# evergreen-ci/evergreen

Measured on NVIDIA H100. Metric: tasks scheduled/sec over N distros; host-allocator decisions/sec at 1/2/4/8 GPU, higher is better.
Workload: dtype int64

## Files before the change

### evergreen_b200/_lib.py

```python
from __future__ import annotations

import ctypes as C
import os

import numpy as np

_HERE = os.path.dirname(os.path.abspath(__file__))
LIB_PATH = os.path.join(_HERE, "libevgsched.so")

EVG_TIME_ZERO = -(2 ** 63)

EVG_OK = 0
EVG_ERR_INVALID, EVG_ERR_CUDA, EVG_ERR_NOMEM, EVG_ERR_STATE = -1, -2, -3, -4
EVG_ALLOC_OK, EVG_ALLOC_ERR_FUTURE_FRACTION, EVG_ALLOC_ERR_POOL_SIZE, EVG_ALLOC_ERR_PARENT_MISSING = 0, 1, 2, 3

EVG_TF_REQ_OTHER, EVG_TF_REQ_PATCH, EVG_TF_REQ_MERGE_QUEUE = 0, 1, 2
EVG_TF_GENERATE, EVG_TF_STEPBACK, EVG_TF_DEPS_MET, EVG_TF_OTHER_DISTRO = 0x4, 0x8, 0x10, 0x20
EVG_HF_RUNNING, EVG_HF_TEARDOWN, EVG_HF_RT_FOUND = 0x1, 0x2, 0x4
EVG_HG_NONE, EVG_HG_UNQUEUED = -1, -2
EVG_PROVIDER_STATIC, EVG_PROVIDER_EPHEMERAL, EVG_PROVIDER_DOCKER = 0, 1, 2
EVG_OPT_BREAKDOWN = 0x1
EVG_BD_N = 13
(EVG_BD_TASK_GROUP_LENGTH, EVG_BD_TOTAL_VALUE, EVG_BD_P_INITIAL, EVG_BD_P_TASK_GROUP, EVG_BD_P_GENERATOR,
 EVG_BD_P_COMMIT_QUEUE, EVG_BD_R_COMMIT_QUEUE, EVG_BD_R_NUM_DEPENDENTS, EVG_BD_R_ESTIMATED_RUNTIME,
# ... 66 lines not shown
class PlanOutStruct(C.Structure):
    _fields_ = [("order", C.c_void_p), ("total_value", C.c_void_p), ("breakdown", C.c_void_p),
                ("info", C.c_void_p), ("group_info", C.c_void_p)]


class HostSoAStruct(C.Structure):
    _fields_ = [("n_hosts", C.c_int64), ("flags", C.c_void_p), ("group_id", C.c_void_p),
                ("expected_ns", C.c_void_p), ("std_ns", C.c_void_p), ("start_ns", C.c_void_p)]


class DepsInStruct(C.Structure):
    _fields_ = [("n_tasks", C.c_int64), ("n_deps", C.c_int64), ("dep_off", C.c_void_p), ("dep_kind", C.c_void_p),
                ("dep_ref", C.c_void_p), ("dep_want", C.c_void_p), ("task_state", C.c_void_p), ("task_pre", C.c_void_p),
                ("ext_state", C.c_void_p), ("n_ext", C.c_int64)]


EVG_DEP_IN_QUEUE, EVG_DEP_EXTERNAL, EVG_DEP_MISSING = 0, 1, 2
EVG_WANT_SUCCESS, EVG_WANT_FAILED, EVG_WANT_ANY, EVG_WANT_OTHER = 0, 1, 2, 3
EVG_TS_BLOCKED = 0x4
EVG_TP_OVERRIDE, EVG_TP_MET_TIME = 0x1, 0x2


class RunnableInStruct(C.Structure):
    _fields_ = [("n_tasks", C.c_int64), ("n_distros", C.c_int32), ("n_projects", C.c_int32), ("task_off", C.c_void_p),
                ("sched", C.c_void_p), ("project", C.c_void_p), ("project_flags", C.c_void_p), ("valid_off", C.c_void_p),
                ("valid_idx", C.c_void_p), ("finder", C.c_void_p), ("deps", C.POINTER(DepsInStruct))]


class AliasInStruct(C.Structure):
    _fields_ = [("tasks", TaskSoAStruct), ("n_groups", C.c_int32), ("n_versions", C.c_int32), ("group_max_hosts", C.c_void_p),
                ("sched", C.c_void_p), ("task_group_max_hosts", C.c_void_p), ("primary", C.c_void_p),
                ("secondary_off", C.c_void_p), ("secondary_idx", C.c_void_p), ("n_names", C.c_int32), ("_reserved", C.c_int32),
                ("dest_off", C.c_void_p), ("dest_idx", C.c_void_p), ("deps", C.POINTER(DepsInStruct)),
                ("dep_finished_ns", C.c_void_p)]


class AliasOutStruct(C.Structure):
    _fields_ = [("task_off", C.c_void_p), ("group_off", C.c_void_p), ("n_versions", C.c_void_p)]


EVG_SQ_ACTIVATED, EVG_SQ_UNDISPATCHED, EVG_SQ_PRIORITY_OK, EVG_SQ_HOST_PLATFORM = 0x01, 0x02, 0x04, 0x08
EVG_SQ_UNATTAINABLE, EVG_SQ_OVERRIDE_DEPS, EVG_SQ_GITHUB_PR, EVG_SQ_PATCH_REQUEST = 0x10, 0x20, 0x40, 0x80
EVG_PF_ENABLED, EVG_PF_HIDDEN, EVG_PF_DISPATCHING_DISABLED, EVG_PF_PATCHING_DISABLED = 0x1, 0x2, 0x4, 0x8
EVG_FINDER_NO_DEPS, EVG_FINDER_LEGACY, EVG_FINDER_ALTERNATE = 0, 1, 2
EVG_FINDER_PIPELINE, EVG_FINDER_PIPELINE_NO_DEPS = 3, 4
EVG_STATUS_SUCCESS, EVG_STATUS_FAILED, EVG_STATUS_ANY = 0, 1, 2
EVG_PR_ENABLED, EVG_PR_DISPATCHING_DISABLED, EVG_PR_PATCHING_FALSE = 0x1, 0x2, 0x4


class PipelineInStruct(C.Structure):
    _fields_ = [("n_status", C.c_int32), ("_reserved", C.c_int32), ("dep_status", C.c_void_p), ("task_status", C.c_void_p),
                ("ext_status", C.c_void_p), ("task_unattainable", C.c_void_p), ("ext_unattainable", C.c_void_p),
                ("project_raw", C.c_void_p)]


class DurationRowsStruct(C.Structure):
    _fields_ = [("n_rows", C.c_int64), ("n_keys", C.c_int32), ("_reserved", C.c_int32), ("key", C.c_void_p),
                ("time_taken_ns", C.c_void_p), ("start_ns", C.c_void_p), ("finish_ns", C.c_void_p), ("flags", C.c_void_p),
                ("window_start_ns", C.c_int64), ("window_end_ns", C.c_int64)]


EVG_DR_COMPLETED, EVG_DR_TIMED_OUT = 0x1, 0x2
DURATION_STAT_DTYPE = np.dtype([("count", np.int64), ("mean_ns", np.float64), ("stddev_ns", np.float64)])
EVG_DK_NONE = -1


def EVG_DK_PAIR(p: int) -> int:
    return -2 - p


EVG_DS_FRESH, EVG_DS_BACKFILL, EVG_DS_HISTORY, EVG_DS_PREVIOUS, EVG_DS_DEFAULT = 0, 1, 2, 3, 4
DURATION_CACHE_COLUMNS = ("value_ns", "std_ns", "ttl_ns", "collected_ns", "expected_ns", "expected_std_ns")


class DurationCacheStruct(C.Structure):
    _fields_ = [("n_rows", C.c_int64), ("rows", C.c_void_p), ("value_ns", C.c_void_p), ("std_ns", C.c_void_p),
                ("ttl_ns", C.c_void_p), ("collected_ns", C.c_void_p), ("expected_ns", C.c_void_p),
                ("expected_std_ns", C.c_void_p), ("key", C.c_void_p)]


class DurationInStruct(C.Structure):
    _fields_ = [("history", C.POINTER(DurationRowsStruct)), ("n_pairs", C.c_int32), ("_reserved", C.c_int32),
                ("pair_key_off", C.c_void_p), ("tasks", C.POINTER(DurationCacheStruct)),
                ("hosts", C.POINTER(DurationCacheStruct))]


DURATION_OUT_FIELDS = ("avg_ns", "std_ns", "value_ns", "pred_std_ns", "collected_ns", "source")


class DurationOutStruct(C.Structure):
    _fields_ = [(f, C.c_void_p) for f in DURATION_OUT_FIELDS]


class LegacySoAStruct(C.Structure):
    _fields_ = [("n_tasks", C.c_int64), ("priority", C.c_void_p), ("ingest_ns", C.c_void_p), ("expected_ns", C.c_void_p),
                ("num_dependents", C.c_void_p), ("revision_order", C.c_void_p), ("project_id", C.c_void_p),
                ("tg_rank", C.c_void_p), ("tg_pair_id", C.c_void_p), ("task_group_order", C.c_void_p),
                ("presort_rank", C.c_void_p), ("flags", C.c_void_p)]


EVG_LF_REQ_SYSTEM, EVG_LF_REQ_PATCH, EVG_LF_REQ_OTHER, EVG_LF_GENERATE, EVG_LF_MERGE_QUEUE_VERSION = 0, 1, 2, 0x4, 0x8
EVG_LEGACY_MODE_INGEST, EVG_LEGACY_MODE_REVISION, EVG_LEGACY_MODE_LITERAL = 0, 1, 2
EVG_LEGACY_OK, EVG_LEGACY_NOT_DECOMPOSABLE = 0, 1


class DagInStruct(C.Structure):
    _fields_ = [("n_items", C.c_int64), ("n_deps", C.c_int64), ("dep_off", C.c_void_p), ("dep_item", C.c_void_p),
                ("group_id", C.c_void_p), ("group_index", C.c_void_p)]


DISPATCH_OUT_FIELDS = ("item_off", "sorted", "n_sorted", "n_cycles", "group_off", "group_slot", "unit_items", "unit_off")


class DispatchOutStruct(C.Structure):
    _fields_ = [(f, C.c_void_p) for f in DISPATCH_OUT_FIELDS]


class AllocOutStruct(C.Structure):
    _fields_ = [("result", C.c_void_p), ("status", C.c_void_p)]


class EvgError(RuntimeError):
    def __init__(self, code: int, msg: str):
        super().__init__(f"libevgsched error {code}: {msg}")
        self.code = code


_P = C.c_void_p
SYMBOLS = {
    "evg_init": (C.c_int, [C.c_int, _P, C.POINTER(_P)]),
    "evg_shutdown": (None, [_P]),
    "evg_last_error": (C.c_char_p, []),
    "evg_abi_version": (C.c_int, []),
    "evg_host_alloc": (_P, [C.c_uint64]),
    "evg_host_free": (None, [_P]),
    "evg_plan_batch": (C.c_int, [_P, _P, _P, C.c_int64, C.c_uint32, _P]),
    "evg_alloc_batch": (C.c_int, [_P, _P, _P, _P, _P, _P, _P, C.c_int32, C.c_int64, _P]),
    "evg_plan_and_alloc_batch": (C.c_int, [_P, _P, _P, _P, _P, _P, C.c_int64, C.c_uint32, _P, _P]),
    "evg_upload": (C.c_int, [_P, _P, _P, _P, _P, _P]),
    "evg_upload_device": (C.c_int, [_P, _P, _P, _P, _P, _P]),
    "evg_update_tasks": (C.c_int, [_P, C.c_int64, _P, _P]),
    "evg_edit_tasks": (C.c_int, [_P, _P, _P, _P, _P, _P]),
    "evg_plan_from_finder": (C.c_int, [_P, _P, _P, _P, _P, _P, _P, _P, C.c_int64, _P, _P]),
    "evg_plan_from_finder_ex": (C.c_int, [_P, _P, _P, _P, _P, _P, _P, _P, _P, C.c_int64, _P, _P]),
    "evg_plan_aliases": (C.c_int, [_P, _P, _P, C.c_int32, C.c_int64, _P]),
    "evg_download_alias_map": (C.c_int, [_P, _P, _P]),
    "evg_intern_columns": (C.c_int, [_P, _P, C.c_int32]),
    "evg_run_resident": (C.c_int, [_P, C.c_int64, C.c_uint32]),
    "evg_download": (C.c_int, [_P, _P, _P]),
    "evg_download_queue": (C.c_int, [_P, C.c_int32, _P, _P, C.c_int64]),
    "evg_device_result_ptr": (_P, [_P]),
    "evg_bind_result_buffer": (C.c_int, [_P, _P, C.c_int64]),
    "evg_last_launch_count": (C.c_int64, [_P]),
    "evg_last_timing_ms": (C.c_int, [_P, C.POINTER(C.c_float), C.POINTER(C.c_float)]),
    "evg_kernel_timing_ms": (C.c_int, [_P, C.POINTER(C.c_float), C.c_int32]),
    "evg_general_timing_ms": (C.c_int, [_P, C.POINTER(C.c_float), C.POINTER(C.c_float)]),
    "evg_deps_met_batch": (C.c_int, [_P, _P, _P]),
    "evg_upload_with_deps": (C.c_int, [_P, _P, _P, _P, _P, _P, _P, _P, C.c_int64]),
    "evg_download_deps": (C.c_int, [_P, _P, _P]),
    "evg_find_runnable_batch": (C.c_int, [_P, _P, _P, _P]),
    "evg_find_runnable_ex": (C.c_int, [_P, _P, _P, _P, _P]),
    "evg_expected_durations_batch": (C.c_int, [_P, _P, _P]),
    "evg_resolve_durations": (C.c_int, [_P, _P, C.c_int64]),
    "evg_download_durations": (C.c_int, [_P, _P, _P]),
    "evg_prioritize_legacy_batch": (C.c_int, [_P, _P, _P, _P, C.c_int32, _P, _P, _P]),
    "evg_dag_rebuild_batch": (C.c_int, [_P, _P, _P, _P, C.c_int32, _P, _P, _P, _P, _P]),
    "evg_rebuild_dispatchers": (C.c_int, [_P, C.c_int32, C.c_int64, C.c_int64, _P]),
    "evg_plan_distro": (C.c_int, [_P, _P, _P, C.c_int32, _P, C.c_int64, C.c_uint32, _P]),
    "evg_alloc_distro": (C.c_int, [_P, _P, _P, _P, _P, C.c_int32, C.c_int64, _P, _P]),
}

_lib = None


def load() -> C.CDLL:
    global _lib
    if _lib is not None:
        return _lib
    if not os.path.exists(LIB_PATH):
        raise ImportError(
            f"{LIB_PATH} is missing: build it with `python -c 'import __graft_entry__ as g; g.build()'` "
            "(nvcc, sm_90a). evergreen_b200 has no CPU fallback.")
    lib = C.CDLL(LIB_PATH)
    for name, (res, args) in SYMBOLS.items():
        fn = getattr(lib, name)
        fn.restype = res
        fn.argtypes = args
    if lib.evg_abi_version() != 1:
        raise ImportError("libevgsched.so ABI version mismatch")
    _lib = lib
    return lib


def last_error() -> str:
    return (load().evg_last_error() or b"").decode("utf-8", "replace")


def check(rc: int) -> None:
    if rc != EVG_OK:
        raise EvgError(rc, last_error())


def ptr(a) -> int:
    if a is None:
        return None
    assert a.flags["C_CONTIGUOUS"], "columns must be C-contiguous"
    return a.ctypes.data
```

### evergreen_b200/csrc/evg_plan_general.cuh

```cuda
#pragma once

#ifndef EVG_OCC_GLINK
#define EVG_OCC_GLINK 4
#endif
#ifndef EVG_OCC_GALLOC
#define EVG_OCC_GALLOC 4
#endif
#ifndef EVG_OCC_GFILL
#define EVG_OCC_GFILL 4
#endif
#ifndef EVG_OCC_GUNIT
#define EVG_OCC_GUNIT 4
#endif
#ifndef EVG_OCC_GBEST
#define EVG_OCC_GBEST 4
#endif
#ifndef EVG_GTASK_OCC
#define EVG_GTASK_OCC 2
#endif
constexpr int kGTile = 2048;

struct DGen {
  int64_t n_tiles;
  int64_t tile0;
  const int32_t* tile_distro;
  const int64_t* tile_start;
  const int64_t* dtile_off;
  unsigned long long* vmm;
  uint32_t* key_lo[2];
  uint32_t* key_hi[2];
  uint32_t* idx[2];
  uint32_t* e;
  uint32_t* tile_sum;
  uint32_t* tile_hist;
  uint4* wl;
  struct URec* pay;
  unsigned int* ccount;
  uint4* tie;
  int32_t* maxpass;
  uint32_t* run;
  uint32_t* pown;
  uint32_t* pver;
  uint32_t* pedge;
  uint32_t* sedge;
  uint32_t* rank;
  unsigned int* rcount;
  uint2* blist;
  unsigned int* bcount;
  uint4* usum;
  uint2* hlist;
  unsigned int* hcount;
  int64_t* tv;
};

__device__ __forceinline__ int gen_bits(const DGen& G, int d) {
  const unsigned long long r = G.vmm[2 * d] - G.vmm[2 * d + 1];
  return r == 0 ? 0 : 64 - __clzll((long long)r);
}
__device__ __forceinline__ int gen_npass(int bits) { return (bits + 7) >> 3; }

struct __align__(16) URec {
  int32_t prio, nd;
  int64_t exp_ns, qb;
  int32_t tgo;
  uint32_t lif;
};
static_assert(sizeof(URec) == 32, "one L2 sector per member");
constexpr uint32_t kRecGrouped = 1u << 22, kRecWaitOver = 1u << 23;
constexpr uint32_t kRunOwn = 1u << 31, kRunEntry = kRunOwn - 1u;
__device__ __forceinline__ uint32_t rec_li(const URec& r) { return r.lif & 0x1FFFFFu; }
__device__ __forceinline__ URec rec_load(const URec* p) {
  const uint4 a = reinterpret_cast<const uint4*>(p)[0], b = reinterpret_cast<const uint4*>(p)[1];
  URec r;
  r.prio = int32_t(a.x); r.nd = int32_t(a.y); r.exp_ns = int64_t((unsigned long long)a.z | ((unsigned long long)a.w << 32));
  r.qb = int64_t((unsigned long long)b.x | ((unsigned long long)b.y << 32)); r.tgo = int32_t(b.z); r.lif = b.w;
  return r;
}
__device__ __forceinline__ void rec_store(URec* p, const URec& r) {
  reinterpret_cast<uint4*>(p)[0] = make_uint4(uint32_t(r.prio), uint32_t(r.nd), uint32_t(uint64_t(r.exp_ns)), uint32_t(uint64_t(r.exp_ns) >> 32));
  reinterpret_cast<uint4*>(p)[1] = make_uint4(uint32_t(uint64_t(r.qb)), uint32_t(uint64_t(r.qb) >> 32), uint32_t(r.tgo), r.lif);
}

__global__ void k_ginit(DGen G, const int32_t* __restrict__ general_list, int n) {
  const int k = blockIdx.x * blockDim.x + threadIdx.x;
  if (k == 0) { *G.ccount = 0u; *G.maxpass = 0; *G.rcount = 0u; *G.hcount = 0u; *G.bcount = 0u; }
  if (k >= n) return;
  const int d = general_list[k];
  G.vmm[2 * d] = 0ull;
  G.vmm[2 * d + 1] = ~0ull;
}

__global__ void __launch_bounds__(256) k_gmark(DTasks T, DDistros D, DWork W, DGen G) {
  if (*W.err) return;
  const int tile = int(blockIdx.x + G.tile0);
  const int d = G.tile_distro[tile];
  const int64_t base = D.task_off[d], end = D.task_off[d + 1];
  const int64_t lo = max(G.tile_start[tile], base), hi = min(G.tile_start[tile] + kGTile, end);
  for (int64_t t = lo + threadIdx.x; t < hi; t += 256)
    for (int64_t e = T.dep_off[t]; e < T.dep_off[t + 1]; e++) W.has_dep[base + T.dep_idx[e]] = 1;
}

struct TileFold {
  unsigned int c[10];
  unsigned long long s[4];
  unsigned long long vmax, vmin;
};

__global__ void __launch_bounds__(256, EVG_GTASK_OCC) k_gtask(DTasks T, DDistros D, DWork W, DGen G, int64_t now, int any_complex) {
  if (*W.err) return;
  __shared__ TileFold F;
  __shared__ evg_distro_cfg s_cfg;
  __shared__ uint32_t s_nd[kNdTable];
  const int tile = int(blockIdx.x + G.tile0);
  const int d = G.tile_distro[tile];
  const int tid = threadIdx.x, lane = tid & 31;
  const unsigned full = 0xffffffffu;
  if (tid == 0) {
    for (int k = 0; k < 10; k++) F.c[k] = 0;
    for (int k = 0; k < 4; k++) F.s[k] = 0;
    F.vmax = 0ull; F.vmin = ~0ull;
    s_cfg = D.cfg[d];
  }
  __syncthreads();
  const evg_distro_cfg& cfg = s_cfg;
  const int64_t base = D.task_off[d], end = D.task_off[d + 1];
  const int64_t ts = G.tile_start[tile];
  const uint32_t ng = uint32_t(D.group_off[d + 1] - D.group_off[d]);
  const uint32_t ub = uint32_t(D.unit_base[d]);
  const bool gv = cfg.group_versions != 0;
  const int64_t threshold = cfg.target_time_ns;
  const PlannerFactors pf = clamp_factors(cfg);
  const Factors32 f32 = factors32(pf, now);
  const bool sane_clock = threshold >= 0 && now >= threshold;
  const int64_t wait_cutoff = wsub(now, threshold);
  const bool fast_clock = now >= 0 && pf.nd_int != 0;
  const bool incl = cfg.includes_dependencies != 0;
  if (tid < kNdTable) {
    const int64_t e = nd_table_entry(pf, tid);
    s_nd[tid] = (e >= 0 && e < int64_t(kNdTermLimit)) ? uint32_t(e) : 0xFFFFFFFFu;
  }
  __syncthreads();
  const bool dcomplex = any_complex && (ng > 0 || gv || (T.n_edges > 0 && T.dep_off[end] > T.dep_off[base]));

  unsigned int c_dm = 0, c_mq = 0, c_over = 0, c_wait = 0, c_sec = 0, c_ung = 0, c_ucnt = 0, c_uover = 0, c_uwait = 0, c_umq = 0;
  int64_t s_exp = 0, s_over = 0, s_uexp = 0, s_uover = 0;
  unsigned long long kmax = 0ull, kmin = ~0ull;

#pragma unroll 1
  for (int u = 0; u < 2; u++) {
    const int64_t t4 = ts + 4 * int64_t(u * 256 + tid);
    const bool live = t4 < end;
    int4 prio4 = make_int4(0, 0, 0, 0), nd4 = prio4, gid4 = make_int4(-1, -1, -1, -1), tgo4 = prio4, vid4 = prio4;
    uint4 fl4 = make_uint4(0, 0, 0, 0);
    uint32_t cmask = 0, womask = 0;
    if (live && dcomplex) {
      tgo4 = *reinterpret_cast<const int4*>(T.tgo + t4);
      if (gv) vid4 = *reinterpret_cast<const int4*>(T.vid + t4);
    }
    longlong2 ex01 = make_longlong2(0, 0), ex23 = ex01, qb01 = ex01, qb23 = ex01, wb01 = ex01, wb23 = ex01;
    if (live) {
      prio4 = *reinterpret_cast<const int4*>(T.priority + t4);
      nd4 = *reinterpret_cast<const int4*>(T.numdep + t4);
      gid4 = *reinterpret_cast<const int4*>(T.gid + t4);
      fl4 = *reinterpret_cast<const uint4*>(T.flags + t4);
      ex01 = *reinterpret_cast<const longlong2*>(T.expected + t4); ex23 = *reinterpret_cast<const longlong2*>(T.expected + t4 + 2);
      qb01 = *reinterpret_cast<const longlong2*>(T.qbasis + t4); qb23 = *reinterpret_cast<const longlong2*>(T.qbasis + t4 + 2);
      wb01 = *reinterpret_cast<const longlong2*>(T.wbasis + t4); wb23 = *reinterpret_cast<const longlong2*>(T.wbasis + t4 + 2);
    }
    int64_t doff[5] = {0, 0, 0, 0, 0};
    uint32_t hd4 = 0;
    if (live && dcomplex) {
      if (T.n_edges > 0) {
        const longlong2 d01 = *reinterpret_cast<const longlong2*>(T.dep_off + t4), d23 = *reinterpret_cast<const longlong2*>(T.dep_off + t4 + 2);
        doff[0] = d01.x; doff[1] = d01.y; doff[2] = d23.x; doff[3] = d23.y; doff[4] = T.dep_off[t4 + 4];
      }
      hd4 = *reinterpret_cast<const uint32_t*>(W.has_dep + t4);
    }
    const int32_t prio_[4] = {prio4.x, prio4.y, prio4.z, prio4.w}, nd_[4] = {nd4.x, nd4.y, nd4.z, nd4.w};
    const int32_t gid_[4] = {gid4.x, gid4.y, gid4.z, gid4.w};
    const uint32_t fl_[4] = {fl4.x, fl4.y, fl4.z, fl4.w};
    const int64_t ex_[4] = {ex01.x, ex01.y, ex23.x, ex23.y}, qb_[4] = {qb01.x, qb01.y, qb23.x, qb23.y};
    const int64_t wb_[4] = {wb01.x, wb01.y, wb23.x, wb23.y};
    int64_t vout[4];
    uint32_t eout[4], nd_term[4];
    bool wr_v[4], solo[4];
    bool dom = true;
#pragma unroll
    for (int m = 0; m < 4; m++) {
      const int64_t t = t4 + m;
      const bool valid = live & (t >= base) & (t < end);
      const int32_t prio = prio_[m], nd = nd_[m], gid = gid_[m];
      const uint32_t fl = fl_[m];
      const int64_t exp_ns = ex_[m], qb = qb_[m], wb = wb_[m];
      const bool dm = valid & ((fl & EVG_TF_DEPS_MET) != 0);
      const bool counted = valid & (!incl | dm);
      const bool over = counted & (exp_ns > threshold);
      const bool waited = sane_clock ? (wb < wait_cutoff) : (since(now, wb) > threshold);
      const bool wait_over = counted & dm & waited;
      const bool mq_dm = dm & ((fl & EVG_TF_REQ_MASK) == EVG_TF_REQ_MERGE_QUEUE);
      const bool ung = valid & (gid < 0);
      c_dm += dm; c_mq += mq_dm; c_over += over; c_wait += wait_over; c_sec += valid & ((fl & EVG_TF_OTHER_DISTRO) != 0);
      s_exp += counted ? exp_ns : 0;
      s_over += over ? exp_ns : 0;
      c_ung += ung; c_ucnt += ung & counted; c_uover += ung & over; c_uwait += ung & wait_over; c_umq += ung & mq_dm;
      s_uexp += (ung & counted) ? exp_ns : 0;
      s_uover += (ung & over) ? exp_ns : 0;
      const bool own_complex = valid & dcomplex & ((gid >= 0) | gv | (((hd4 >> (8 * m)) & 0xFFu) != 0));
      const bool complex_task = own_complex | (valid & dcomplex & (doff[m + 1] > doff[m]));
      const bool scores = valid & !own_complex;
      const uint32_t ndc = uint32_t(nd > 0 ? nd : 0);
      const uint32_t tab = s_nd[ndc < uint32_t(kNdTable) ? ndc : 0u];
      const uint32_t mul = (f32.ok & (ndc < kTask32Limit)) ? f32.nd * ndc : 0xFFFFFFFFu;
      nd_term[m] = ndc < uint32_t(kNdTable) ? tab : mul;
      dom = dom & (!scores | (score32_bad(now, prio, exp_ns, qb, nd_term[m]) == 0u));
      wr_v[m] = scores;
      solo[m] = scores & !complex_task;
      eout[m] = (valid & !complex_task) ? 1u : 0u;
      cmask |= (complex_task ? 1u : 0u) << m;
      womask |= (wait_over ? 1u : 0u) << m;
    }
    if (f32.ok_base && __all_sync(full, dom)) {
#pragma unroll
      for (int m = 0; m < 4; m++) vout[m] = int64_t(single_task_value32_nd(f32, now, prio_[m], ex_[m], qb_[m], nd_term[m], fl_[m]));
    } else {
#pragma unroll
      for (int m = 0; m < 4; m++) vout[m] = int64_t(score_slow(pf, fast_clock, wr_v[m], now, prio_[m], ex_[m], qb_[m], nd_[m], fl_[m]));
    }
#pragma unroll
    for (int m = 0; m < 4; m++) {
      const unsigned long long k = ord_i64(vout[m]);
      kmax = solo[m] ? max(kmax, k) : kmax;
      kmin = solo[m] ? min(kmin, k) : kmin;
    }
    if (!live) {
    } else if (t4 >= base && t4 + 3 < end) {
      *reinterpret_cast<longlong2*>(G.tv + t4) = make_longlong2(vout[0], vout[1]);
      *reinterpret_cast<longlong2*>(G.tv + t4 + 2) = make_longlong2(vout[2], vout[3]);
    } else {
#pragma unroll
      for (int m = 0; m < 4; m++)
        if (wr_v[m]) G.tv[t4 + m] = vout[m];
    }
    if (dcomplex && live) {
      if (t4 >= base && t4 + 3 < end) *reinterpret_cast<uint4*>(G.e + t4) = make_uint4(eout[0], eout[1], eout[2], eout[3]);
      else {
#pragma unroll
        for (int m = 0; m < 4; m++)
          if (t4 + m >= base && t4 + m < end) G.e[t4 + m] = eout[m];
      }
    }
    if (dcomplex) {
      __shared__ uint32_t s_wsum[8];
      __shared__ uint32_t s_lbase;
      const uint32_t mine = __popc(cmask);
      uint32_t inc = mine;
#pragma unroll
      for (int o = 1; o < 32; o <<= 1) { const uint32_t x = __shfl_up_sync(full, inc, o); if (lane >= o) inc += x; }
      if (lane == 31) s_wsum[tid >> 5] = inc;
      __syncthreads();
      uint32_t before = 0, total = 0;
#pragma unroll
      for (int w = 0; w < 8; w++) { const uint32_t x = s_wsum[w]; before += w < (tid >> 5) ? x : 0u; total += x; }
      if (total) {
        if (tid == 0) s_lbase = atomicAdd(G.ccount, total);
        __syncthreads();
        uint32_t pos = s_lbase + before + inc - mine;
        const int32_t vid_[4] = {vid4.x, vid4.y, vid4.z, vid4.w}, tgo_[4] = {tgo4.x, tgo4.y, tgo4.z, tgo4.w};
#pragma unroll
        for (int m = 0; m < 4; m++) {
          if (!((cmask >> m) & 1u)) continue;
          const uint32_t t = uint32_t(t4 + m), li = uint32_t(t4 + m - base);
          const int32_t gid = gid_[m], vid = vid_[m];
          const bool own_complex = (gid >= 0) | gv | (((hd4 >> (8 * m)) & 0xFFu) != 0);
          const uint32_t s_own = own_complex ? ub + own_slot_local(gid, vid, li, ng, gv) : kInactive;
          const uint32_t s_ver = (gid >= 0 && gv) ? ub + ng + uint32_t(vid) : kInactive;
          G.wl[pos] = make_uint4(t, uint32_t(d), s_own, s_ver);
          URec r;
          r.prio = prio_[m]; r.nd = nd_[m]; r.exp_ns = ex_[m]; r.qb = qb_[m]; r.tgo = tgo_[m];
          r.lif = li | (gid >= 0 ? kRecGrouped : 0u) | (((womask >> m) & 1u) ? kRecWaitOver : 0u) | ((fl_[m] & 0x3Fu) << 24);
          rec_store(G.pay + pos, r);
          pos++;
        }
      }
      __syncthreads();
    }
  }
  {
    unsigned int cs[10] = {c_dm, c_mq, c_over, c_wait, c_sec, c_ung, c_ucnt, c_uover, c_uwait, c_umq};
#pragma unroll
    for (int k = 0; k < 10; k++) cs[k] = __reduce_add_sync(full, cs[k]);
    int64_t ss[4] = {s_exp, s_over, s_uexp, s_uover};
#pragma unroll
    for (int k = 0; k < 4; k++) ss[k] = warp_sum64(ss[k]);
#pragma unroll
    for (int o = 16; o > 0; o >>= 1) {
      kmax = max(kmax, __shfl_xor_sync(full, kmax, o));
      kmin = min(kmin, __shfl_xor_sync(full, kmin, o));
    }
    if (lane == 0) {
#pragma unroll
      for (int k = 0; k < 10; k++) if (cs[k]) atomicAdd(&F.c[k], cs[k]);
#pragma unroll
      for (int k = 0; k < 4; k++) if (ss[k]) atomicAdd(&F.s[k], (unsigned long long)ss[k]);
      atomicMax(&F.vmax, kmax); atomicMin(&F.vmin, kmin);
    }
  }
  __syncthreads();
  if (tid < 16) {
    evg_queue_info* q = W.qinfo + d;
    switch (tid) {
      case 0: atomic_add64(&q->length_with_dependencies_met, F.c[0]); break;
      case 1: atomic_add64(&q->count_dep_filled_merge_queue_tasks, F.c[1]); break;
      case 2: atomic_add64(&q->count_duration_over_threshold, F.c[2]); break;
      case 3: atomic_add64(&q->count_wait_over_threshold, F.c[3]); break;
      case 4: atomic_add64(&q->secondary_queue, F.c[4]); break;
      case 5: atomic_add64(&q->has_ungrouped, F.c[5]); break;
      case 6: atomic_add64(&q->ungrouped.count, F.c[6]); break;
      case 7: atomic_add64(&q->ungrouped.count_duration_over_threshold, F.c[7]); break;
      case 8: atomic_add64(&q->ungrouped.count_wait_over_threshold, F.c[8]); break;
      case 9: atomic_add64(&q->ungrouped.count_dep_filled_merge_queue_tasks, F.c[9]); break;
      case 10: atomic_add64(&q->expected_duration, int64_t(F.s[0])); break;
      case 11: atomic_add64(&q->duration_over_threshold, int64_t(F.s[1])); break;
      case 12: atomic_add64(&q->ungrouped.expected_duration, int64_t(F.s[2])); break;
      case 13: atomic_add64(&q->ungrouped.duration_over_threshold, int64_t(F.s[3])); break;
      case 14: if (F.vmax > __ldcg(G.vmm + 2 * d)) atomicMax(G.vmm + 2 * d, F.vmax); break;
      case 15: if (F.vmin < __ldcg(G.vmm + 2 * d + 1)) atomicMin(G.vmm + 2 * d + 1, F.vmin); break;
    }
  }
}


struct WlTask {
  uint32_t t; int d; int64_t base; uint32_t li; bool own_complex; uint32_t s_own, s_ver;
};
__device__ __forceinline__ WlTask wl_task(const DDistros& D, const DGen& G, unsigned int k) {
  const uint4 e = G.wl[k];
  WlTask x;
  x.t = e.x; x.d = int(e.y); x.s_own = e.z; x.s_ver = e.w;
  x.base = D.task_off[x.d];
  x.li = uint32_t(int64_t(x.t) - x.base);
  x.own_complex = x.s_own != kInactive;
  return x;
}
template <typename F>
__device__ __forceinline__ void wl_pairs(const DTasks& T, const DGen& G, const WlTask& x, unsigned int k, F&& f) {
  if (x.own_complex) f(G.pown + k, x.s_own, true);
  if (x.s_ver != kInactive) f(G.pver + k, x.s_ver, false);
  if (T.n_edges > 0)
    for (int64_t e = T.dep_off[x.t]; e < T.dep_off[x.t + 1]; e++) {
      const uint32_t sl = G.sedge[e];
      if (sl != kInactive) f(G.pedge + e, sl, false);
    }
}

__global__ void __launch_bounds__(256, EVG_OCC_GLINK) k_glink(DTasks T, DDistros D, DWork W, DGen G, int64_t now) {
  if (*W.err) return;
  const unsigned int n = *G.ccount;
  for (unsigned int k = blockIdx.x * blockDim.x + threadIdx.x; k < n; k += gridDim.x * blockDim.x) {
    const WlTask x = wl_task(D, G, k);
    const uint32_t t = x.t;
    const int d = x.d;
    const uint32_t ub = uint32_t(D.unit_base[d]), ng = uint32_t(D.group_off[d + 1] - D.group_off[d]);
    if (x.own_complex && x.s_own - ub < ng) {
      const URec me = rec_load(G.pay + k);
      const evg_distro_cfg* cf = D.cfg + d;
      const uint32_t fl = (me.lif >> 24) & 0x3Fu;
      const int64_t exp_ns = me.exp_ns, threshold = cf->target_time_ns;
      const bool dm = (fl & EVG_TF_DEPS_MET) != 0;
      const bool counted = !cf->includes_dependencies || dm;
      const bool over = counted && exp_ns > threshold;
      const bool wait_over = (me.lif & kRecWaitOver) != 0;
      const bool mq_dm = dm && (fl & EVG_TF_REQ_MASK) == EVG_TF_REQ_MERGE_QUEUE;
      evg_group_info* g = W.ginfo + D.group_off[d] + (x.s_own - ub);
      atomic_add64(&g->count, counted);
      atomic_add64(&g->expected_duration, counted ? exp_ns : 0);
      atomic_add64(&g->count_duration_over_threshold, over);
      atomic_add64(&g->duration_over_threshold, over ? exp_ns : 0);
      atomic_add64(&g->count_wait_over_threshold, wait_over);
      atomic_add64(&g->count_dep_filled_merge_queue_tasks, mq_dm);
    }
    if (x.own_complex) G.pown[k] = atomicAdd(W.unit_n + x.s_own, 1u);
    if (x.s_ver != kInactive) G.pver[k] = atomicAdd(W.unit_n + x.s_ver, 1u);
    if (T.n_edges > 0) {
      const bool gv = D.cfg[d].group_versions != 0;
      const int64_t e0 = T.dep_off[t], e1 = T.dep_off[t + 1];
      for (int64_t e = e0; e < e1; e++) {
        const uint32_t dl = uint32_t(T.dep_idx[e]);
        const uint32_t sl = ub + own_slot_local(T.gid[x.base + dl], T.vid[x.base + dl], dl, ng, gv);
        bool dup = (sl == x.s_own) || (sl == x.s_ver);
        for (int64_t f = e0; f < e && !dup; f++) {
          const uint32_t fl2 = uint32_t(T.dep_idx[f]);
          dup = ub + own_slot_local(T.gid[x.base + fl2], T.vid[x.base + fl2], fl2, ng, gv) == sl;
        }
        G.sedge[e] = dup ? kInactive : sl;
        if (!dup) G.pedge[e] = atomicAdd(W.unit_n + sl, 1u);
      }
    }
  }
}

__global__ void __launch_bounds__(256, EVG_OCC_GALLOC) k_galloc(DTasks T, DDistros D, DWork W, DGen G) {
  if (*W.err) return;
  __shared__ uint32_t s_wsum[8], s_wcnt[8];
  __shared__ uint32_t s_base, s_hbase;
  const unsigned int n = *G.ccount;
  const int lane = threadIdx.x & 31, warp = threadIdx.x >> 5;
  for (unsigned int k0 = blockIdx.x * blockDim.x; k0 < n; k0 += gridDim.x * blockDim.x) {
    const unsigned int k = k0 + threadIdx.x;
    WlTask x;
    uint32_t need = 0, heads = 0;
    if (k < n) {
      x = wl_task(D, G, k);
      wl_pairs(T, G, x, k, [&](const uint32_t* place, uint32_t slot, bool) { if (*place == 0u) { need += W.unit_n[slot]; heads++; } });
    }
    uint32_t inc = need, hinc = heads;
#pragma unroll
    for (int o = 1; o < 32; o <<= 1) {
      const uint32_t y = __shfl_up_sync(0xffffffffu, inc, o), z = __shfl_up_sync(0xffffffffu, hinc, o);
      if (lane >= o) { inc += y; hinc += z; }
    }
    if (lane == 31) { s_wsum[warp] = inc; s_wcnt[warp] = hinc; }
    __syncthreads();
    uint32_t before = 0, total = 0, hbefore = 0, htotal = 0;
#pragma unroll
    for (int w = 0; w < 8; w++) {
      const uint32_t y = s_wsum[w], z = s_wcnt[w];
      before += w < warp ? y : 0u; total += y; hbefore += w < warp ? z : 0u; htotal += z;
    }
    if (threadIdx.x == 0 && htotal) { s_base = atomicAdd(G.rcount, total); s_hbase = atomicAdd(G.hcount, htotal); }
    __syncthreads();
    if (heads) {
      uint32_t pos = s_base + before + inc - need, hp = s_hbase + hbefore + hinc - heads;
      wl_pairs(T, G, x, k, [&](const uint32_t* place, uint32_t slot, bool) {
        if (*place == 0u) { W.head[slot] = pos; pos += W.unit_n[slot]; G.hlist[hp++] = make_uint2(slot, uint32_t(x.d)); }
      });
    }
    __syncthreads();
  }
}

__global__ void __launch_bounds__(256, EVG_OCC_GFILL) k_gfill(DTasks T, DDistros D, DWork W, DGen G) {
  if (*W.err) return;
  const unsigned int n = *G.ccount;
  for (unsigned int k = blockIdx.x * blockDim.x + threadIdx.x; k < n; k += gridDim.x * blockDim.x) {
    const WlTask x = wl_task(D, G, k);
    wl_pairs(T, G, x, k, [&](const uint32_t* place, uint32_t slot, bool own) {
      G.run[W.head[slot] + *place] = k | (own ? kRunOwn : 0u);
    });
  }
}

__device__ __forceinline__ void rec_acc(UnitAcc& a, int64_t now, const URec& r) {
  acc_add(a, now, r.prio, r.exp_ns, r.qb, r.nd, (r.lif & kRecGrouped) ? 0 : -1, (r.lif >> 24) & 0x3Fu);
}
__device__ __forceinline__ bool rec_less(const URec& x, const URec& y) {
  return in_unit_less(x.tgo, x.nd, x.prio, x.exp_ns, rec_li(x), y.tgo, y.nd, y.prio, y.exp_ns, rec_li(y));
}
constexpr uint32_t kRankOne = 8;
constexpr int kRankKey = 6;

__global__ void __launch_bounds__(256, EVG_OCC_GUNIT) k_gunit(DDistros D, DWork W, DGen G, int64_t now) {
  if (*W.err) return;
  const unsigned int n = *G.hcount;
  __shared__ uint32_t s_key[kRankOne * kRankKey][256];
  for (unsigned int k = blockIdx.x * blockDim.x + threadIdx.x; k < n; k += gridDim.x * blockDim.x) {
    const uint2 u = G.hlist[k];
    const uint32_t cnt = W.unit_n[u.x], h = W.head[u.x];
    const uint32_t* run = G.run + h;
    UnitAcc a;
    acc_init(a);
    uint32_t anchor = kNoAnchor;
    const bool small = cnt <= kRankOne;
    for (uint32_t i = 0; i < cnt; i++) {
      const uint32_t q = run[i];
      const URec r = rec_load(G.pay + (q & kRunEntry));
      rec_acc(a, now, r);
      if (q & kRunOwn) anchor = min(anchor, rec_li(r));
      if (small) {
        uint32_t* kx = &s_key[i * kRankKey][threadIdx.x];
        kx[0] = uint32_t(r.tgo); kx[256] = uint32_t(r.nd); kx[512] = uint32_t(r.prio);
        kx[768] = uint32_t(uint64_t(r.exp_ns)); kx[1024] = uint32_t(uint64_t(r.exp_ns) >> 32); kx[1280] = rec_li(r);
      }
    }
    const unsigned long long v = (unsigned long long)unit_value(a, D.cfg[u.y], nullptr);
    G.usum[u.x] = make_uint4(uint32_t(v), uint32_t(v >> 32), anchor, cnt);
    W.unit_mask[u.x] = 0ull;
    if (small) {
      auto key = [&](uint32_t i, URec& r) {
        const uint32_t* kx = &s_key[i * kRankKey][threadIdx.x];
        r.tgo = int32_t(kx[0]); r.nd = int32_t(kx[256]); r.prio = int32_t(kx[512]);
        r.exp_ns = int64_t((unsigned long long)kx[768] | ((unsigned long long)kx[1024] << 32)); r.lif = kx[1280];
      };
      for (uint32_t i = 0; i < cnt; i++) {
        URec me, o;
        key(i, me);
        uint32_t rk = 0;
        for (uint32_t j = 0; j < cnt; j++) { key(j, o); rk += rec_less(o, me) ? 1u : 0u; }
        G.rank[h + i] = rk;
      }
    } else {
      const uint32_t nch = (cnt + 31) >> 5;
      const uint32_t b = atomicAdd(G.bcount, nch);
      for (uint32_t c = 0; c < nch; c++) G.blist[b + c] = make_uint2(u.x, c);
    }
  }
}

__global__ void __launch_bounds__(256, EVG_OCC_GUNIT) k_grank(DWork W, DGen G) {
  if (*W.err) return;
  const unsigned int n = *G.bcount;
  const unsigned full = 0xffffffffu;
  const int lane = threadIdx.x & 31;
  const unsigned int nw = gridDim.x * (blockDim.x >> 5);
  for (unsigned int c = blockIdx.x * (blockDim.x >> 5) + (threadIdx.x >> 5); c < n; c += nw) {
    const uint2 ch = G.blist[c];
    const uint32_t cnt = W.unit_n[ch.x], h = W.head[ch.x];
    const uint32_t* run = G.run + h;
    const uint32_t i = ch.y * 32u + uint32_t(lane);
    URec me;
    me.tgo = 0; me.nd = 0; me.prio = 0; me.exp_ns = 0; me.lif = 0;
    if (i < cnt) me = rec_load(G.pay + (run[i] & kRunEntry));
    uint32_t rk = 0;
    for (uint32_t j0 = 0; j0 < cnt; j0 += 32) {
      URec o;
      o.tgo = 0; o.nd = 0; o.prio = 0; o.exp_ns = 0; o.lif = 0;
      if (j0 + lane < cnt) o = rec_load(G.pay + (run[j0 + lane] & kRunEntry));
      const uint32_t m = min(32u, cnt - j0);
      for (uint32_t q = 0; q < m; q++) {
        URec y;
        y.tgo = __shfl_sync(full, o.tgo, q); y.nd = __shfl_sync(full, o.nd, q); y.prio = __shfl_sync(full, o.prio, q);
        y.exp_ns = __shfl_sync(full, o.exp_ns, q); y.lif = __shfl_sync(full, o.lif, q);
        rk += (i < cnt && rec_less(y, me)) ? 1u : 0u;
      }
    }
    if (i < cnt) G.rank[h + i] = rk;
  }
}

__global__ void __launch_bounds__(256, EVG_OCC_GBEST) k_gbest(DTasks T, DDistros D, DWork W, DGen G, int want_best_pair) {
  if (*W.err) return;
  const unsigned int n = *G.ccount;
  const unsigned full = 0xffffffffu;
  const int lane = threadIdx.x & 31;
  for (unsigned int kw = blockIdx.x * blockDim.x + (threadIdx.x & ~31u); kw < n; kw += gridDim.x * blockDim.x) {
    const unsigned int k = kw + lane;
    int d = -1;
    unsigned long long kk = 0ull;
    if (k < n) {
      const WlTask x = wl_task(D, G, k);
      const uint32_t t = x.t, li = x.li;
      d = x.d;
      bool have = false;
      int64_t bv = 0;
      uint32_t ba = 0, brk = 0, bslot = kInactive, bn = 1, bkx = 0;
      if (!x.own_complex) { have = true; bv = G.tv[t]; ba = li; }
      wl_pairs(T, G, x, k, [&](const uint32_t* place, uint32_t slot, bool) {
        const uint4 u = G.usum[slot];
        const uint32_t kx = *place;
        const uint32_t a = u.z;
        if (a == kNoAnchor) return;
        const int64_t v = int64_t((unsigned long long)u.x | ((unsigned long long)u.y << 32));
        if (!have || v > bv || (v == bv && a < ba)) { have = true; bv = v; ba = a; bslot = slot; bn = u.w; bkx = kx; }
      });
      if (bslot != kInactive) {
        brk = G.rank[W.head[bslot] + bkx];
        if (bn <= 64) atomicOr(&W.unit_mask[bslot], 1ull << brk);
      }
      G.tv[t] = bv;
      G.tie[k] = make_uint4(ba, brk, bslot, 0u);
      if (want_best_pair) W.best_pair[t] = bslot;
      const bool displaced = !(ba == li && brk == 0);
      if (displaced) W.has_dep[t] |= 2;
      atomicAdd(G.e + x.base + ba, 1u);
      kk = ord_i64(bv);
    }
    const int d0 = __shfl_sync(full, d, 0);
    if (__all_sync(full, d < 0 || d == d0)) {
      unsigned long long hi = d < 0 ? 0ull : kk, lo = d < 0 ? ~0ull : kk;
#pragma unroll
      for (int o = 16; o > 0; o >>= 1) {
        hi = max(hi, __shfl_xor_sync(full, hi, o));
        lo = min(lo, __shfl_xor_sync(full, lo, o));
      }
      if (lane == 0) {
        if (hi > __ldcg(G.vmm + 2 * d0)) atomicMax(G.vmm + 2 * d0, hi);
        if (lo < __ldcg(G.vmm + 2 * d0 + 1)) atomicMin(G.vmm + 2 * d0 + 1, lo);
      }
    } else if (d >= 0) {
      if (kk > __ldcg(G.vmm + 2 * d)) atomicMax(G.vmm + 2 * d, kk);
      if (kk < __ldcg(G.vmm + 2 * d + 1)) atomicMin(G.vmm + 2 * d + 1, kk);
    }
  }
}

__global__ void k_gsched(DGen G, const int32_t* __restrict__ general_list, int n) {
  const int k = blockIdx.x * blockDim.x + threadIdx.x;
  if (k >= n) return;
  const int np = gen_npass(gen_bits(G, general_list[k]));
  if (np > 0) atomicMax(G.maxpass, np);
}

__global__ void __launch_bounds__(256) k_gsum(DDistros D, DGen G) {
  const int tile = int(blockIdx.x + G.tile0);
  const int d = G.tile_distro[tile];
  const int64_t base = D.task_off[d], end = D.task_off[d + 1];
  const int64_t lo = max(G.tile_start[tile], base), hi = min(G.tile_start[tile] + kGTile, end);
  uint32_t sum = 0;
  for (int64_t t = lo + threadIdx.x; t < hi; t += 256) sum += G.e[t];
  sum = __reduce_add_sync(0xffffffffu, sum);
  __shared__ uint32_t sw[8];
  if ((threadIdx.x & 31) == 0) sw[threadIdx.x >> 5] = sum;
  __syncthreads();
  if (threadIdx.x == 0) G.tile_sum[tile] = sw[0] + sw[1] + sw[2] + sw[3] + sw[4] + sw[5] + sw[6] + sw[7];
}

__global__ void __launch_bounds__(1024) k_gscan(DGen G, const int32_t* __restrict__ general_list) {
  const int d = general_list[blockIdx.x];
  const int64_t t0 = G.dtile_off[d], nt = G.dtile_off[d + 1] - t0;
  __shared__ uint32_t sw[32];
  __shared__ uint32_t carry;
  const int lane = threadIdx.x & 31, warp = threadIdx.x >> 5;
  if (threadIdx.x == 0) carry = 0;
  __syncthreads();
  for (int64_t c0 = 0; c0 < nt; c0 += 1024) {
    const int64_t i = c0 + threadIdx.x;
    const uint32_t v = i < nt ? G.tile_sum[t0 + i] : 0u;
    uint32_t inc = v;
#pragma unroll
    for (int o = 1; o < 32; o <<= 1) { const uint32_t x = __shfl_up_sync(0xffffffffu, inc, o); if (lane >= o) inc += x; }
    if (lane == 31) sw[warp] = inc;
    __syncthreads();
    if (warp == 0) {
      const uint32_t w = sw[lane];
      uint32_t winc = w;
#pragma unroll
      for (int o = 1; o < 32; o <<= 1) { const uint32_t x = __shfl_up_sync(0xffffffffu, winc, o); if (lane >= o) winc += x; }
      sw[lane] = winc - w;
    }
    __syncthreads();
    const uint32_t ex = carry + sw[warp] + inc - v;
    if (i < nt) G.tile_sum[t0 + i] = ex;
    __syncthreads();
    if (threadIdx.x == 1023) carry = ex + v;
    __syncthreads();
  }
}

__device__ __forceinline__ void gen_put(const DGen& G, int64_t base, uint32_t pos, unsigned long long vmax_ord, bool wide,
                                        int64_t v, uint32_t li) {
  const unsigned long long key = vmax_ord - ord_i64(v);
  G.key_lo[0][base + pos] = uint32_t(key);
  if (wide) G.key_hi[0][base + pos] = uint32_t(key >> 32);
  G.idx[0][base + pos] = li;
}

__global__ void __launch_bounds__(256) k_gplace(DDistros D, DWork W, DGen G, int use_e) {
  const int tile = int(blockIdx.x + G.tile0);
  const int d = G.tile_distro[tile];
  const int64_t base = D.task_off[d], end = D.task_off[d + 1];
  const int64_t ts = G.tile_start[tile];
  const unsigned long long vmax_ord = G.vmm[2 * d];
  const bool wide = gen_bits(G, d) > 32;
  const int tid = threadIdx.x, lane = tid & 31, warp = tid >> 5;
  const int64_t t8 = ts + 8 * int64_t(tid);
  const bool interior = t8 >= base && t8 + 7 < end;
  uint32_t ev[8];
  uint32_t sum = 0;
  if (use_e) {
    if (interior) {
      const uint4 a = *reinterpret_cast<const uint4*>(G.e + t8), b = *reinterpret_cast<const uint4*>(G.e + t8 + 4);
      ev[0] = a.x; ev[1] = a.y; ev[2] = a.z; ev[3] = a.w; ev[4] = b.x; ev[5] = b.y; ev[6] = b.z; ev[7] = b.w;
    } else {
#pragma unroll
      for (int m = 0; m < 8; m++) { const int64_t t = t8 + m; ev[m] = (t >= base && t < end) ? G.e[t] : 0u; }
    }
#pragma unroll
    for (int m = 0; m < 8; m++) sum += ev[m];
  }
  uint32_t run = 0;
  if (use_e) {
    __shared__ uint32_t sw[8];
    uint32_t inc = sum;
#pragma unroll
    for (int o = 1; o < 32; o <<= 1) { const uint32_t x = __shfl_up_sync(0xffffffffu, inc, o); if (lane >= o) inc += x; }
    if (lane == 31) sw[warp] = inc;
    __syncthreads();
    uint32_t before = 0;
#pragma unroll
    for (int w = 0; w < 8; w++) if (w < warp) before += sw[w];
    run = G.tile_sum[tile] + before + inc - sum;
  }
  int64_t vv[8];
  uint32_t dsp = 0;
  if (interior) {
#pragma unroll
    for (int m = 0; m < 8; m += 2) {
      const longlong2 x = *reinterpret_cast<const longlong2*>(G.tv + t8 + m);
      vv[m] = x.x; vv[m + 1] = x.y;
    }
    if (use_e) {
      const uint32_t h0 = *reinterpret_cast<const uint32_t*>(W.has_dep + t8), h1 = *reinterpret_cast<const uint32_t*>(W.has_dep + t8 + 4);
#pragma unroll
      for (int m = 0; m < 4; m++) dsp |= (((h0 >> (8 * m + 1)) & 1u) << m) | (((h1 >> (8 * m + 1)) & 1u) << (m + 4));
    }
  } else {
#pragma unroll
    for (int m = 0; m < 8; m++) {
      const int64_t t = t8 + m;
      const bool in = t >= base && t < end;
      vv[m] = in ? G.tv[t] : 0;
      if (use_e && in && (W.has_dep[t] & 2)) dsp |= 1u << m;
    }
  }
  if (use_e) {
    constexpr int kStage = 3072;
    __shared__ uint32_t st_lo[kStage], st_ix[kStage], st_hi[kStage];
    __shared__ uint32_t s_total;
    const uint32_t p_tile = G.tile_sum[tile];
    if (tid == 255) s_total = run + sum - p_tile;
    uint32_t ps[8];
#pragma unroll
    for (int m = 0; m < 8; m++) { ps[m] = run; run += ev[m]; }
    if (interior) {
      *reinterpret_cast<uint4*>(G.e + t8) = make_uint4(ps[0], ps[1], ps[2], ps[3]);
      *reinterpret_cast<uint4*>(G.e + t8 + 4) = make_uint4(ps[4], ps[5], ps[6], ps[7]);
    } else {
#pragma unroll
      for (int m = 0; m < 8; m++) { const int64_t t = t8 + m; if (t >= base && t < end) G.e[t] = ps[m]; }
    }
    __syncthreads();
    const uint32_t total = s_total;
    const bool staged = total <= uint32_t(kStage);
#pragma unroll
    for (int m = 0; m < 8; m++) {
      const int64_t t = t8 + m;
      if (t >= base && t < end && !((dsp >> m) & 1u)) {
        if (staged) {
          const unsigned long long key = vmax_ord - ord_i64(vv[m]);
          const uint32_t q = ps[m] - p_tile;
          st_lo[q] = uint32_t(key); st_ix[q] = uint32_t(t - base);
          if (wide) st_hi[q] = uint32_t(key >> 32);
        } else {
          gen_put(G, base, ps[m], vmax_ord, wide, vv[m], uint32_t(t - base));
        }
      }
    }
    if (staged) {
      __syncthreads();
      uint32_t* dlo = G.key_lo[0] + base + p_tile;
      uint32_t* dix = G.idx[0] + base + p_tile;
      uint32_t* dhi = G.key_hi[0] + base + p_tile;
      for (uint32_t q = tid; q < total; q += 256) {
        dlo[q] = st_lo[q]; dix[q] = st_ix[q];
        if (wide) dhi[q] = st_hi[q];
      }
    }
  } else if (interior) {
    uint32_t kl[8], kh[8];
#pragma unroll
    for (int m = 0; m < 8; m++) {
      const unsigned long long key = vmax_ord - ord_i64(vv[m]);
      kl[m] = uint32_t(key); kh[m] = uint32_t(key >> 32);
    }
    const uint32_t p0 = uint32_t(t8 - base);
    *reinterpret_cast<uint4*>(G.key_lo[0] + t8) = make_uint4(kl[0], kl[1], kl[2], kl[3]);
    *reinterpret_cast<uint4*>(G.key_lo[0] + t8 + 4) = make_uint4(kl[4], kl[5], kl[6], kl[7]);
    *reinterpret_cast<uint4*>(G.idx[0] + t8) = make_uint4(p0, p0 + 1, p0 + 2, p0 + 3);
    *reinterpret_cast<uint4*>(G.idx[0] + t8 + 4) = make_uint4(p0 + 4, p0 + 5, p0 + 6, p0 + 7);
    if (wide) {
      *reinterpret_cast<uint4*>(G.key_hi[0] + t8) = make_uint4(kh[0], kh[1], kh[2], kh[3]);
      *reinterpret_cast<uint4*>(G.key_hi[0] + t8 + 4) = make_uint4(kh[4], kh[5], kh[6], kh[7]);
    }
  } else {
#pragma unroll
    for (int m = 0; m < 8; m++) {
      const int64_t t = t8 + m;
      if (t >= base && t < end) gen_put(G, base, uint32_t(t - base), vmax_ord, wide, vv[m], uint32_t(t - base));
    }
  }
}

__global__ void __launch_bounds__(256) k_gplace_disp(DTasks T, DDistros D, DWork W, DGen G) {
  const unsigned int n = *G.ccount;
  for (unsigned int k = blockIdx.x * blockDim.x + threadIdx.x; k < n; k += gridDim.x * blockDim.x) {
  const uint4 ent = G.wl[k];
  const uint32_t t = ent.x;
  if (!(W.has_dep[t] & 2)) continue;
  const int d = int(ent.y);
  const int64_t base = D.task_off[d];
  const uint4 tie = G.tie[k];
  const uint32_t a = tie.x, myrk = tie.y, slot = tie.z;
  uint32_t pos = G.e[base + a];
  const uint32_t cnt = W.unit_n[slot];
  if (cnt <= 64) {
    pos += __popcll(W.unit_mask[slot] & ((1ull << myrk) - 1ull));
  } else {
    const uint32_t* run = G.run + W.head[slot];
    for (uint32_t i = 0; i < cnt; i++) {
      const uint4 tq = G.tie[run[i] & kRunEntry];
      if (tq.z == slot && tq.y < myrk) pos++;
    }
  }
  gen_put(G, base, pos, G.vmm[2 * d], gen_bits(G, d) > 32, G.tv[t], uint32_t(int64_t(t) - base));
  }
}

__device__ __forceinline__ bool gen_tile(const DDistros& D, const DGen& G, int tile, int j, int* d_out, int64_t* seg, int64_t* lo,
                                         int* cnt, bool* wide) {
  const int d = G.tile_distro[tile];
  const int bits = gen_bits(G, d);
  if (j >= gen_npass(bits)) return false;
  const int64_t base = D.task_off[d], end = D.task_off[d + 1];
  const int64_t a = max(G.tile_start[tile], base), b = min(G.tile_start[tile] + kGTile, end);
  *d_out = d; *seg = base; *lo = a; *cnt = int(b - a); *wide = bits > 32;
  return true;
}

__global__ void __launch_bounds__(256) k_ghist(int j, DDistros D, DGen G) {
  if (j >= *G.maxpass) return;
  int d, cnt; int64_t seg, lo; bool wide;
  const int tile = int(blockIdx.x + G.tile0);
  if (!gen_tile(D, G, tile, j, &d, &seg, &lo, &cnt, &wide)) return;
  const uint32_t* src = (j < 4 ? G.key_lo[j & 1] : G.key_hi[j & 1]) + lo;
  const int shift = 8 * (j & 3);
  __shared__ uint32_t h[256];
  h[threadIdx.x] = 0;
  __syncthreads();
  for (int i = threadIdx.x; i < cnt; i += 256) atomicAdd(&h[(src[i] >> shift) & 255u], 1u);
  __syncthreads();
  G.tile_hist[int64_t(tile) * 256 + threadIdx.x] = h[threadIdx.x];
}

__global__ void __launch_bounds__(1024) k_gdscan(int j, const int32_t* __restrict__ general_list, DGen G) {
  if (j >= *G.maxpass) return;
  const int d = general_list[blockIdx.x];
  if (j >= gen_npass(gen_bits(G, d))) return;
  const int dg = threadIdx.x & 255, grp = threadIdx.x >> 8;
  const int64_t t0 = G.dtile_off[d], nt = G.dtile_off[d + 1] - t0;
  const int64_t per = (nt + 3) / 4;
  const int64_t a = t0 + (grp * per < nt ? grp * per : nt), b = t0 + ((grp + 1) * per < nt ? (grp + 1) * per : nt);
  uint32_t* h = G.tile_hist + dg;
  uint32_t sum = 0;
  int64_t tile = a;
  for (; tile + 8 <= b; tile += 8) {
    uint32_t x[8];
#pragma unroll
    for (int k = 0; k < 8; k++) x[k] = h[(tile + k) * 256];
#pragma unroll
    for (int k = 0; k < 8; k++) sum += x[k];
  }
  for (; tile < b; tile++) sum += h[tile * 256];
  __shared__ uint32_t part[4][256];
  __shared__ uint32_t s[256];
  part[grp][dg] = sum;
  __syncthreads();
  const uint32_t total = part[0][dg] + part[1][dg] + part[2][dg] + part[3][dg];
  if (grp == 0) s[dg] = total;
  __syncthreads();
  for (int o = 1; o < 256; o <<= 1) {
    uint32_t v = 0;
    if (grp == 0 && dg >= o) v = s[dg - o];
    __syncthreads();
    if (grp == 0) s[dg] += v;
    __syncthreads();
  }
  uint32_t run = s[dg] - total;
  for (int g = 0; g < grp; g++) run += part[g][dg];
  tile = a;
  for (; tile + 8 <= b; tile += 8) {
    uint32_t x[8];
#pragma unroll
    for (int k = 0; k < 8; k++) x[k] = h[(tile + k) * 256];
#pragma unroll
    for (int k = 0; k < 8; k++) { h[(tile + k) * 256] = run; run += x[k]; }
  }
  for (; tile < b; tile++) { const uint32_t x = h[tile * 256]; h[tile * 256] = run; run += x; }
}

template <bool WIDE>
__device__ __forceinline__ void gscatter_tile(int j, const DGen& G, int tile, int64_t seg, int64_t lo, int cnt, uint32_t (*wcnt)[256],
                                              uint32_t* s_lo, uint32_t* s_ix, uint32_t* s_hi, int32_t* s_delta, uint32_t* s_wsum) {
  constexpr bool wide = WIDE;
  const int sb = j & 1, db = sb ^ 1;
  const int tid = threadIdx.x, warp = tid >> 5, lane = tid & 31;
#pragma unroll
  for (int w = 0; w < 8; w++) wcnt[w][tid] = 0u;
  __syncthreads();
  const unsigned lt = (1u << lane) - 1u;
  const int shift = 8 * (j & 3);
  const bool use_hi = j >= 4;
  const uint32_t* src_lo = G.key_lo[sb] + lo;
  const uint32_t* src_hi = G.key_hi[sb] + lo;
  const uint32_t* src_ix = G.idx[sb] + lo;
  uint32_t kl[8], kh[8], ix[8], dg[8], rk[8];
#pragma unroll
  for (int k = 0; k < 8; k++) {
    const int i = (warp * 8 + k) * 32 + lane;
    const bool ok = i < cnt;
    kl[k] = ok ? src_lo[i] : 0u;
    kh[k] = (ok && wide) ? src_hi[i] : 0u;
    ix[k] = ok ? src_ix[i] : 0u;
  }
  unsigned peers[8];
#pragma unroll
  for (int k = 0; k < 8; k++) {
    const int i = (warp * 8 + k) * 32 + lane;
    dg[k] = i < cnt ? (((use_hi ? kh[k] : kl[k]) >> shift) & 255u) : 256u;
    peers[k] = __match_any_sync(0xffffffffu, dg[k]);
  }
#pragma unroll
  for (int k = 0; k < 8; k++) {
    rk[k] = 0;
    if (dg[k] < 256u && (peers[k] & lt) == 0u) rk[k] = atomicAdd(&wcnt[warp][dg[k]], uint32_t(__popc(peers[k])));
  }
#pragma unroll
  for (int k = 0; k < 8; k++) rk[k] = __shfl_sync(0xffffffffu, rk[k], __ffs(peers[k]) - 1) + uint32_t(__popc(peers[k] & lt));
  __syncthreads();
  {
    uint32_t x[8], tot = 0;
#pragma unroll
    for (int w = 0; w < 8; w++) { x[w] = wcnt[w][tid]; tot += x[w]; }
    uint32_t inc = tot;
#pragma unroll
    for (int o = 1; o < 32; o <<= 1) { const uint32_t y = __shfl_up_sync(0xffffffffu, inc, o); if (lane >= o) inc += y; }
    if (lane == 31) s_wsum[warp] = inc;
    __syncthreads();
    uint32_t before = 0;
#pragma unroll
    for (int w = 0; w < 8; w++) before += w < warp ? s_wsum[w] : 0u;
    const uint32_t lbase = before + inc - tot;
    s_delta[tid] = int32_t(G.tile_hist[int64_t(tile) * 256 + tid]) - int32_t(lbase);
    uint32_t run = lbase;
#pragma unroll
    for (int w = 0; w < 8; w++) { wcnt[w][tid] = run; run += x[w]; }
  }
  __syncthreads();
#pragma unroll
  for (int k = 0; k < 8; k++) {
    if (dg[k] < 256u) {
      const uint32_t lp = wcnt[warp][dg[k]] + rk[k];
// ... 49 lines not shown
```

### evergreen_b200/csrc/evg_sched.cu

```cuda
#include <cuda_runtime.h>
#include <stdarg.h>
#include <stdint.h>
#include <stdio.h>
#include <string.h>

#include <algorithm>
#include <type_traits>
#include <cstdlib>
#include <future>
#include <mutex>
#include <string>
#include <vector>

#include "evg_score.cuh"
#include "evg_intern.h"

using namespace evg;

namespace {

thread_local std::string g_err;

int fail(int code, const char* fmt, ...) {
  char buf[512];
// ... 962 lines not shown
  }
  int32_t st = EVG_ALLOC_OK;
  int64_t n_new = 0, n_free_out = n_free_all;
  if (c.provider != EVG_PROVIDER_DOCKER && n_existing >= c.maximum_hosts) {
    n_new = 0;
  } else if (c.disabled) {
    n_new = int64_t(c.minimum_hosts) - n_existing;
    if (n_new < 0) n_new = 0;
  } else {
    int64_t required = 0, free_approx = 0;
    if (qi.has_ungrouped || u_hosts > 0) {
      int64_t n, f;
      st = eval_group(c, qi.ungrouped, threshold, c.maximum_hosts, u_hosts, u_free, u_soon, &n, &f);
      required += n;
      free_approx += f;
    }
    if (st == EVG_ALLOC_OK) {
      if (required + n_free_all > qi.length_with_dependencies_met) required = qi.length_with_dependencies_met - n_free_all;
      if (required < 0) required = 0;
      int64_t topup = 0;
      if (n_existing + required < c.minimum_hosts) topup = c.minimum_hosts - (n_existing + required);
      n_new = required + topup;
      n_free_out = free_approx;
    } else {
      n_new = 0;
      n_free_out = n_free_all;
    }
  }
  int64_t deficit = wsub(qi.expected_duration, wmul(n_free_out, threshold));
  if (deficit < 0) deficit = 0;
  result[d].new_hosts = int32_t(n_new);
  result[d].free_hosts = int32_t(n_free_out);
  result[d].deficit_ns = deficit;
  status[d] = st;
}

struct TaskCols {
  DevBuf prio, nd, tgo, gid, vid, flags, exp, qb, wb;
  int stage(const evg_task_soa* t, int64_t n, cudaStream_t s) {
    UP(s, prio, t->priority, n, int32_t);
    UP(s, nd, t->num_dependents, n, int32_t);
    UP(s, tgo, t->task_group_order, n, int32_t);
    UP(s, gid, t->group_id, n, int32_t);
    UP(s, vid, t->version_id, n, int32_t);
    UP(s, flags, t->flags, n, uint32_t);
    UP(s, exp, t->expected_ns, n, int64_t);
    UP(s, qb, t->queue_basis_ns, n, int64_t);
    UP(s, wb, t->wait_basis_ns, n, int64_t);
    return EVG_OK;
  }
  DTasks view(int64_t n) const {
    DTasks v;
    memset(&v, 0, sizeof(v));
    v.n = n;
    v.priority = prio.as<int32_t>(); v.expected = exp.as<int64_t>(); v.qbasis = qb.as<int64_t>(); v.wbasis = wb.as<int64_t>();
    v.numdep = nd.as<int32_t>(); v.tgo = tgo.as<int32_t>(); v.gid = gid.as<int32_t>(); v.vid = vid.as<int32_t>();
    v.flags = flags.as<uint32_t>();
    return v;
  }
  void swap(TaskCols& o) {
    prio.swap(o.prio); nd.swap(o.nd); tgo.swap(o.tgo); gid.swap(o.gid); vid.swap(o.vid);
    flags.swap(o.flags); exp.swap(o.exp); qb.swap(o.qb); wb.swap(o.wb);
  }
};

enum class Tick : uint8_t { kNone, kFixed, kBorrowed, kOwn };

struct evg_ctx {
  int device = 0;
  int num_sms = 0;
  cudaStream_t stream = nullptr;
  bool own_stream = false;
  std::recursive_mutex mu;
  cudaEvent_t ev_begin = nullptr, ev_sort0 = nullptr, ev_sort1 = nullptr, ev_end = nullptr, ev_gt0 = nullptr, ev_gt1 = nullptr;
  bool general_timed = false;
  static constexpr int kRing = 128;
  cudaEvent_t ring0[kRing] = {}, ring1[kRing] = {};
  int64_t runs = 0;
  int64_t max_groups = 0;
  int sort_slot = -1;
  static constexpr int kAux = 6;
  cudaStream_t s_aux[kAux] = {};
  cudaEvent_t ev_fork = nullptr, ev_join[kAux] = {};
  struct { Tick kind = Tick::kNone; bool hosts = false, deps = false, aliases = false, durations = false; } tick;
  int64_t T = 0, E = 0, G = 0, H = 0, U = 0, NT = 0, t_pad = 0;
  int32_t Dn = 0;
  int any_complex = 0;
  int64_t launches = 0;
  bool timed = false;
  TaskCols tasks;
  DevBuf b_depoff, b_depidx;
  DevBuf b_taskoff, b_groupoff, b_cfg, b_gmax, b_unitbase;
  DevBuf b_hasdep, b_head, b_next, b_pslot, b_etask, b_elive, b_bestpair;
  DevBuf b_rn0, b_rn1, b_rn2, b_rn3, b_rn4, b_rn5, b_rn6, b_rn7;
  struct {
    DevBuf off, kind, ref, want, state, pre, ext;
    DevBuf met, fin, stamp;
  } deps;
  struct {
    DevBuf task_off, sched, project, project_flags, valid_off, valid_idx, finder;
    DevBuf kept, count;
    TaskCols cand;
    DevBuf dep_off, dep_idx;
  } pf;
  struct {
    DevBuf dep_status, task_status, ext_status, task_unatt, ext_unatt, project_raw;
    DevBuf edge_cnt, dep_off, dep_idx, scan_sum;
  } pl;
  struct {
    TaskCols out;
    DevBuf dep_off, dep_idx;
    TaskCols ins;
    DevBuf ins_dep_off, ins_dep_idx, rm, add_task, add_dep, gremap, vremap;
    DevBuf new_off, old_off, old_goff, ins_off, old_vbase, edge_at;
    DevBuf keep, pos, src, scan_sum, edge_cnt, err;
  } ed;
  struct {
    TaskCols src;
    DevBuf dep_off, dep_idx, gmax, sched, tgmax, primary, soff, sidx, doff, didx;
    DevBuf cnt, poff, keys[2], hist, hoff;
    DevBuf hk, hv, gslot, vslot, fg, fv, pg, pv;
    DevBuf qoff, samp, gout, srow, gsrc, err;
  } al;
  struct {
    DevBuf key, taken, start, finish, flags, acc, stat, pair_off, single;
    DevBuf rows, in, out, src, err;
    int64_t n_t = 0, n_h = 0;
  } dur;
  struct {
    DevBuf item_off, rank_of, row, first, gslot_of, gindex, cnt, dep_off, dep_item, pos, group_off, group_slot, group_id, scan_sum;
    DevBuf succ_off, succ, index, low, stack, cs_node, cs_pos, emit, on_stack, sorted, stats, buf[2], unit_off;
  } dp;
  DevBuf b_err;
  DevBuf b_route, b_unitv, b_unita, b_unitn, b_unitmask;
  DevBuf b_punt, b_puntcnt;
  struct RouteList {
    std::vector<int32_t> h;
    DevBuf b, lpt;
    int32_t n() const { return int32_t(h.size()); }
  };
  RouteList routes[kRoutes];
  int64_t max_cta_tasks = 0;
  int32_t nNA_big = 0;
  DevBuf b_alist;
  int64_t n_alist = 0;
  bool alist_valid = false;
  std::vector<int64_t> h_taskoff, h_groupoff, h_unitbase, h_edgeoff, h_dtileoff;
  std::vector<int32_t> h_nver;
  cudaStream_t s_h2d = nullptr, s_d2h = nullptr;
  static constexpr int kMaxChunks = 16;
  cudaEvent_t ev_h[kMaxChunks] = {}, ev_c[kMaxChunks] = {};
  int general_complex = 0;
  int64_t Tgc = 0;
  DevBuf b_kv, b_vmm, b_klo[2], b_khi[2], b_ix[2], b_e, b_tilesum, b_gmisc;
  DevBuf b_tiledistro, b_tilestart, b_dtileoff, b_tilehist, b_wl, b_pay, b_place, b_eplace, b_run, b_rank, b_blist, b_tie, b_hlist, b_usum, b_upd;
  DevBuf b_qinfo, b_ginfo, b_order, b_tv, b_bd;
  DevBuf b_hflags, b_hgid, b_hexp, b_hstd, b_hstart, b_hostoff, b_acfg, b_gs, b_result, b_status;
  bool bd_valid = false;
  evg_alloc_result* ext_result = nullptr;
  int64_t ext_capacity = 0;
  evg_alloc_result* result_ptr() const { return ext_result ? ext_result : b_result.as<evg_alloc_result>(); }
};

namespace {

DTasks dtasks(const evg_ctx* c);
DDistros ddistros(const evg_ctx* c);
DWork dwork(const evg_ctx* c);
DGen dgen(const evg_ctx* c);
inline unsigned grid_for(int64_t n, int block) { return unsigned((n + block - 1) / block); }

constexpr int64_t kColPad = 8;

void drop_tick(evg_ctx* c) { c->tick = {}; }

enum class Need { kTick, kOwnColumns, kEditable, kHosts, kVerdicts, kAliasMap, kDurations };
int need_tick(const evg_ctx* c, const char* who, Need what) {
  const auto& t = c->tick;
  const bool own = what == Need::kOwnColumns || what == Need::kEditable;
  const char* unmet = t.kind == Tick::kNone                               ? "no resident tick"
                      : own && t.kind == Tick::kBorrowed                  ? "the resident columns are borrowed (evg_upload_device)"
                      : what == Need::kEditable && t.kind == Tick::kFixed ? "the resident tick is what a one-shot call left"
                      : what == Need::kHosts && !t.hosts                  ? "the resident tick has no hosts"
                      : what == Need::kVerdicts && !t.deps                ? "the resident tick was not uploaded with evg_upload_with_deps"
                      : what == Need::kAliasMap && !t.aliases             ? "the resident tick was not built by evg_plan_aliases"
                      : what == Need::kDurations && !t.durations          ? "no evg_resolve_durations on the resident tick's rows" : nullptr;
  return unmet ? fail(EVG_ERR_STATE, "%s: %s", who, unmet) : EVG_OK;
}

enum class Cols {
  kCopy,
  kChunked,
  kAdopt,
  kResident,
};

int upload_tasks(evg_ctx* c, const char* who, const evg_task_soa* t, const evg_distro_table* dt, Cols cols = Cols::kCopy,
                 const int64_t* edge_off = nullptr) {
  const bool copy_columns = cols == Cols::kCopy, adopt = cols == Cols::kAdopt;
  if (!t || !dt) return fail(EVG_ERR_INVALID, "null task table / distro table");
  const int64_t T = t->n_tasks, E = t->n_edges;
  const int32_t D = dt->n_distros;
  if (T < 0 || E < 0 || D < 0) return fail(EVG_ERR_INVALID, "negative sizes");
  if (T >= (int64_t(1) << 31) - 2) return fail(EVG_ERR_INVALID, "n_tasks %lld exceeds 2^31-2 per call", (long long)T);
  if (2 * T + E >= int64_t(0xFFFFFFF0u)) return fail(EVG_ERR_INVALID, "2*n_tasks+n_edges exceeds the 32-bit pair id space");
  if (D > 0 && (!dt->task_off || !dt->group_off || !dt->cfg)) return fail(EVG_ERR_INVALID, "null distro arrays");
  if (T > 0 && task_cols_missing(t)) return fail(EVG_ERR_INVALID, "null task column");
  if (E > 0 && (!t->dep_off || !t->dep_idx)) return fail(EVG_ERR_INVALID, "n_edges > 0 but dep_off/dep_idx null");
  if (D == 0 && T != 0) return fail(EVG_ERR_INVALID, "tasks without distros");
  int rc = D > 0 ? check_offsets(dt->task_off, D, T, who, "task_off") : EVG_OK;
  if (rc == EVG_OK && D > 0) rc = check_offsets(dt->group_off, D, -1, who, "group_off");
  if (rc != EVG_OK) return rc;
  std::vector<int64_t> unit_base(size_t(D) + 1, 0), dtile_off(size_t(D) + 1, 0);
  std::vector<int32_t> tile_distro, list[kRoutes];
  std::vector<int64_t> tile_start;
  std::vector<uint8_t> route(size_t(D) + 1, 0);
  int general_complex = 0;
  int any_complex = E > 0 ? 1 : 0;
  int64_t Tgc = 0, Prec = 0;
  constexpr int kGA = PlanCta<kNT_A, kNCapA>::kGroupCap, kGB = PlanCta<kNT_B, kNCapB>::kGroupCap, kGC = PlanCta<kNT_C, kNCapC>::kGroupCap;
  constexpr int kBigUnits = kRoutes;
  auto size_class = [&](int32_t d) -> int {
    const int64_t a = dt->task_off[d], b = dt->task_off[d + 1];
    const int64_t n = b - a, g = dt->group_off[d + 1] - dt->group_off[d];
    const evg_distro_cfg& cf = dt->cfg[d];
    const int64_t de = (E > 0) ? (edge_off ? edge_off[d + 1] - edge_off[d] : t->dep_off[b] - t->dep_off[a]) : 0;
    const bool narrow = !cf.group_versions && de == 0;
    if (n <= kCapW) return kWarp;
    if (narrow && n <= kNCapA && g <= kGA) return kCtaA;
    if (narrow && n <= kNCapB && g <= kGB) return kCtaB;
    if (narrow && n <= kNCapC && g <= kGC) return kCtaC;
    if (n <= kCapA) return (cf.group_versions && n > kBigUnitTasks) ? kBigUnits : kSmemA;
    if (n <= kCapB) return kSmemB;
    if (n <= kCapC) return kSmemC;
    return kGeneral;
  };
  int64_t n_class[kBigUnits + 1] = {};
  for (int32_t d = 0; d < D; d++) n_class[size_class(d)]++;
  const char* sparse_env = getenv("EVG_SPARSE_CLASS");
  const int64_t sparse = sparse_env ? atoll(sparse_env) : kSparseClass;
  auto route_of = [&](int32_t d) -> int {
    const int k = size_class(d);
    if ((k == kSmemB || k == kSmemC || k == kBigUnits) && n_class[k] < sparse) return kGeneral;
    return k == kBigUnits ? kSmemA : k;
  };
  for (int32_t d = 0; d < D; d++) {
    const int64_t a = dt->task_off[d], b = dt->task_off[d + 1];
    const int64_t ga = dt->group_off[d], gb = dt->group_off[d + 1];
    if (b - a > kMaxTasksPerDistro) return fail(EVG_ERR_INVALID, "distro %d holds %lld tasks (max %lld)", d, (long long)(b - a), (long long)kMaxTasksPerDistro);
    const evg_distro_cfg& cf = dt->cfg[d];
    if (cf.n_versions < 0) return fail(EVG_ERR_INVALID, "distro %d: negative n_versions", d);
    if (gb > ga || cf.group_versions) any_complex = 1;
    unit_base[d + 1] = unit_base[d] + (gb - ga) + (cf.group_versions ? int64_t(cf.n_versions) : (b - a));
    const int64_t n = b - a;
    const int64_t de = (E > 0) ? (edge_off ? edge_off[d + 1] - edge_off[d] : t->dep_off[b] - t->dep_off[a]) : 0;
    const int r = route_of(d);
    list[r].push_back(d);
    route[d] = r != kGeneral;
    if (r == kGeneral) {
      if (gb > ga || cf.group_versions || de > 0) {
        general_complex = 1;
        Tgc += n;
        Prec += n + ((cf.group_versions && gb > ga) ? n : 0) + de;
      }
      const int64_t a0 = a & ~int64_t(3);
      for (int64_t s = a0; s < b; s += kGTile) { tile_distro.push_back(d); tile_start.push_back(s); }
    }
    dtile_off[d + 1] = int64_t(tile_distro.size());
  }
  const int64_t G = D > 0 ? dt->group_off[D] : 0;
  if (G > 0 && !dt->group_max_hosts) return fail(EVG_ERR_INVALID, "null group_max_hosts");
  const int64_t U = unit_base[D];
  if (U >= int64_t(0xFFFFFFF0u)) return fail(EVG_ERR_INVALID, "unit slot space exceeds 32 bits");
  if (Prec >= int64_t(0xFFFFFFF0u)) return fail(EVG_ERR_INVALID, "unit table exceeds 32 bits");
  if (Tgc >= int64_t(kRunOwn)) return fail(EVG_ERR_INVALID, "work list exceeds 31 bits (a run position is entry id | own bit)");
  const int64_t NT = int64_t(tile_distro.size());
  const int64_t P = 2 * T + E;
  cudaStream_t s = c->stream;
  drop_tick(c);
#define UPC(buf, ptr, count, type)                                                                    \
  do {                                                                                                \
    if (cols == Cols::kResident) break;                                                               \
    if (adopt) {                                                                                      \
      if ((reinterpret_cast<uintptr_t>(ptr) & 15u) != 0) return fail(EVG_ERR_INVALID, "device column %s is not 16-byte aligned", #ptr); \
      (buf).adopt(const_cast<void*>(static_cast<const void*>(ptr)));                                  \
    } else {                                                                                          \
      CK((buf).ensure(sizeof(type) * size_t((count) + kColPad)));                                     \
      if (copy_columns && (count) > 0) CK(cudaMemcpyAsync((buf).p, (ptr), sizeof(type) * size_t(count), cudaMemcpyHostToDevice, s)); \
    }                                                                                                 \
  } while (0)
  UPC(c->tasks.prio, t->priority, T, int32_t);
  UPC(c->tasks.exp, t->expected_ns, T, int64_t);
  UPC(c->tasks.qb, t->queue_basis_ns, T, int64_t);
  UPC(c->tasks.wb, t->wait_basis_ns, T, int64_t);
  UPC(c->tasks.nd, t->num_dependents, T, int32_t);
  UPC(c->tasks.tgo, t->task_group_order, T, int32_t);
  UPC(c->tasks.gid, t->group_id, T, int32_t);
  UPC(c->tasks.vid, t->version_id, T, int32_t);
  UPC(c->tasks.flags, t->flags, T, uint32_t);
  if (E > 0) {
    UPC(c->b_depoff, t->dep_off, T + 1, int64_t);
    UPC(c->b_depidx, t->dep_idx, E, int32_t);
  }
#undef UPC
  UP(s, c->b_taskoff, dt->task_off, D + 1, int64_t);
  UP(s, c->b_groupoff, dt->group_off, D + 1, int64_t);
  UP(s, c->b_cfg, dt->cfg, D, evg_distro_cfg);
  UP(s, c->b_gmax, dt->group_max_hosts, G, int32_t);
  UP(s, c->b_unitbase, unit_base.data(), D + 1, int64_t);
  UP(s, c->b_tiledistro, tile_distro.data(), NT, int32_t);
  UP(s, c->b_tilestart, tile_start.data(), NT, int64_t);
  UP(s, c->b_dtileoff, dtile_off.data(), D + 1, int64_t);
  UP(s, c->b_route, route.data(), D + 1, uint8_t);
  for (int r = 0; r < kRoutes; r++) UP(s, c->routes[r].b, list[r].data(), int64_t(list[r].size()), int32_t);
  std::vector<int32_t> lpt[kRoutes];
  for (int r = 0; r < kRoutes; r++) {
    if (!largest_first(r)) continue;
    lpt[r] = list[r];
    std::stable_sort(lpt[r].begin(), lpt[r].end(), [&](int32_t x, int32_t y) {
      return dt->task_off[x + 1] - dt->task_off[x] > dt->task_off[y + 1] - dt->task_off[y];
    });
  }
  constexpr int kGS = PlanCta<kNT_S, kNCapS>::kGroupCap;
  auto fits_s = [&](int32_t x) { return dt->task_off[x + 1] - dt->task_off[x] <= kNCapS && dt->group_off[x + 1] - dt->group_off[x] <= kGS; };
  std::vector<int32_t>& lpt_a = lpt[kCtaA];
  std::stable_partition(lpt_a.begin(), lpt_a.end(), [&](int32_t x) { return !fits_s(x); });
  c->nNA_big = int32_t(std::count_if(lpt_a.begin(), lpt_a.end(), [&](int32_t x) { return !fits_s(x); }));
  c->max_cta_tasks = 0;
  for (int r = 0; r < kRoutes; r++)
    if (is_cta(r))
      for (int32_t x : list[r]) c->max_cta_tasks = std::max<int64_t>(c->max_cta_tasks, dt->task_off[x + 1] - dt->task_off[x]);
  for (int r = 0; r < kRoutes; r++)
    if (largest_first(r)) UP(s, c->routes[r].lpt, lpt[r].data(), int64_t(lpt[r].size()), int32_t);
  CK(cudaStreamSynchronize(s));
  const bool on_chip = list[kGeneral].size() < size_t(D);
  if (any_complex) {
    CK(c->b_hasdep.ensure(size_t(T) + 16));
    CK(c->b_head.ensure(sizeof(uint32_t) * size_t(U + 1)));
    if (on_chip) {
      CK(c->b_next.ensure(sizeof(uint32_t) * size_t(P + 1)));
      CK(c->b_pslot.ensure(sizeof(uint32_t) * size_t(P + 1)));
    }
    CK(c->b_etask.ensure(sizeof(uint32_t) * size_t(E + 1)));
    CK(c->b_elive.ensure(size_t(E) + 1));
    CK(c->b_unitv.ensure(sizeof(int64_t) * size_t(U + 1)));
    CK(c->b_unita.ensure(sizeof(uint32_t) * size_t(U + 1)));
    CK(c->b_unitn.ensure(sizeof(uint32_t) * size_t(U + 1)));
    CK(c->b_unitmask.ensure(sizeof(uint64_t) * size_t(U + 1)));
    CK(c->b_bestpair.ensure(sizeof(uint32_t) * size_t(T + 1)));
  }
  if (on_chip) CK(c->b_kv.ensure(sizeof(uint64_t) * size_t(T + 1)));
  if (!list[kGeneral].empty()) {
    for (int k = 0; k < 2; k++) {
      CK(c->b_klo[k].ensure(sizeof(uint32_t) * size_t(T + 1)));
      CK(c->b_khi[k].ensure(sizeof(uint32_t) * size_t(T + 1)));
      CK(c->b_ix[k].ensure(sizeof(uint32_t) * size_t(T + 1)));
    }
    CK(c->b_vmm.ensure(sizeof(uint64_t) * 2 * size_t(D + 1)));
    CK(c->b_gmisc.ensure(64));
    CK(c->b_tilesum.ensure(sizeof(uint32_t) * size_t(NT + 1)));
    CK(c->b_tilehist.ensure(sizeof(uint32_t) * 256 * size_t(NT + 1)));
    if (general_complex) {
      CK(c->b_e.ensure(sizeof(uint32_t) * size_t(T + kColPad)));
      CK(c->b_wl.ensure(sizeof(uint4) * size_t(Tgc + 1)));
      CK(c->b_pay.ensure(sizeof(URec) * size_t(Tgc + 1)));
      CK(c->b_tie.ensure(sizeof(uint4) * size_t(Tgc + 1)));
      CK(c->b_place.ensure(sizeof(uint32_t) * 2 * size_t(Tgc + 1)));
      CK(c->b_eplace.ensure(sizeof(uint32_t) * 2 * size_t(E + 1)));
      CK(c->b_run.ensure(sizeof(uint32_t) * size_t(Prec + 1)));
      CK(c->b_rank.ensure(sizeof(uint32_t) * size_t(Prec + 1)));
      CK(c->b_blist.ensure(sizeof(uint2) * size_t(Prec / kRankOne + 1)));
      CK(c->b_hlist.ensure(sizeof(uint2) * size_t(Prec + 1)));
      CK(c->b_usum.ensure(sizeof(uint4) * size_t(U + 1)));
    }
  }
  CK(c->b_punt.ensure(sizeof(int32_t) * size_t(D + 1)));
  CK(c->b_puntcnt.ensure(sizeof(int32_t) * (evg_ctx::kMaxChunks + 2)));
  CK(c->b_qinfo.ensure(sizeof(evg_queue_info) * size_t(D + 1)));
  CK(c->b_ginfo.ensure(sizeof(evg_group_info) * size_t(G + 1)));
  CK(c->b_order.ensure(sizeof(int32_t) * size_t(T + 1)));
  CK(c->b_tv.ensure(sizeof(int64_t) * size_t(T + kColPad)));
  c->T = T; c->E = E; c->G = G; c->U = U; c->NT = NT; c->Dn = D;
  c->t_pad = (T + 3) & ~int64_t(3);
  c->Tgc = Tgc;
  c->max_groups = 0;
  for (int32_t d = 0; d < D; d++) c->max_groups = std::max(c->max_groups, dt->group_off[d + 1] - dt->group_off[d]);
  c->any_complex = any_complex;
  c->general_complex = general_complex;
  CK(c->b_err.ensure(sizeof(int) * 4));
  CK(cudaMemsetAsync(c->b_err.p, 0, sizeof(int) * 4, s));
  for (int r = 0; r < kRoutes; r++) c->routes[r].h.swap(list[r]);
  c->h_taskoff.assign(dt->task_off, dt->task_off + D + 1);
  c->h_groupoff.assign(dt->group_off, dt->group_off + D + 1);
  c->h_edgeoff.assign(size_t(D) + 1, 0);
  if (E > 0)
    for (int32_t d = 0; d <= D; d++) c->h_edgeoff[size_t(d)] = edge_off ? edge_off[d] : t->dep_off[dt->task_off[d]];
  c->h_nver.resize(size_t(D));
  for (int32_t d = 0; d < D; d++) c->h_nver[size_t(d)] = dt->cfg[d].n_versions;
  c->h_unitbase.swap(unit_base);
  c->h_dtileoff.swap(dtile_off);
  c->tick.kind = adopt ? Tick::kBorrowed : Tick::kFixed;
  c->alist_valid = false;
  if (cols != Cols::kChunked && T > 0) {
    DTasks dtv = dtasks(c);
    DDistros ddv = ddistros(c);
    DWork wv = dwork(c);
    k_validate<<<grid_for(T, 256), 256, 0, s>>>(dtv, ddv, wv, 0, T);
    int bad = 0;
    CK(cudaMemcpyAsync(&bad, c->b_err.p, sizeof(int), cudaMemcpyDeviceToHost, s));
    CK(cudaStreamSynchronize(s));
    if (bad) { drop_tick(c); return fail(EVG_ERR_INVALID, "a group_id / version_id / dep_idx is out of range for its distro"); }
  }
  return EVG_OK;
}

int upload_hosts(evg_ctx* c, const char* who, const evg_host_soa* h, const int64_t* host_off, const evg_alloc_cfg* acfg, int32_t D) {
  if (!h || (D > 0 && !acfg)) return fail(EVG_ERR_INVALID, "null host table / allocator config");
  const int64_t H = h->n_hosts;
  if (H < 0) return fail(EVG_ERR_INVALID, "negative n_hosts");
  if (D > 0 && !host_off) return fail(EVG_ERR_INVALID, "null host_off");
  if (D == 0 && H != 0) return fail(EVG_ERR_INVALID, "hosts without distros");
  const int rc = D > 0 ? check_offsets(host_off, D, H, who, "host_off") : EVG_OK;
  if (rc != EVG_OK) return rc;
  if (H > 0 && (!h->flags || !h->group_id || !h->expected_ns || !h->std_ns || !h->start_ns)) return fail(EVG_ERR_INVALID, "null host column");
  cudaStream_t s = c->stream;
  UP(s, c->b_hflags, h->flags, H, uint32_t);
  UP(s, c->b_hgid, h->group_id, H, int32_t);
  UP(s, c->b_hexp, h->expected_ns, H, int64_t);
  UP(s, c->b_hstd, h->std_ns, H, int64_t);
  UP(s, c->b_hstart, h->start_ns, H, int64_t);
  if (D > 0) UP(s, c->b_hostoff, host_off, D + 1, int64_t);
  UP(s, c->b_acfg, acfg, D, evg_alloc_cfg);
  c->alist_valid = false;
  std::vector<int32_t> alist;
  if (c->tick.kind != Tick::kNone && c->Dn == D && int64_t(c->h_groupoff.size()) == int64_t(D) + 1) {
    for (int32_t d = 0; d < D; d++)
      if (c->h_groupoff[d + 1] != c->h_groupoff[d] || host_off[d + 1] - host_off[d] > kGrouplessHosts) alist.push_back(d);
    UP(s, c->b_alist, alist.data(), int64_t(alist.size()), int32_t);
    CK(cudaStreamSynchronize(s));
    c->n_alist = int64_t(alist.size());
    c->alist_valid = true;
  }
  CK(c->b_result.ensure(sizeof(evg_alloc_result) * size_t(D + 1)));
  CK(c->b_status.ensure(sizeof(int32_t) * size_t(D + 1)));
  c->H = H;
  c->tick.hosts = true;
  return EVG_OK;
}

DTasks dtasks(const evg_ctx* c) {
  DTasks t = c->tasks.view(c->T);
  t.n_edges = c->E;
  t.dep_off = c->b_depoff.as<int64_t>(); t.dep_idx = c->b_depidx.as<int32_t>();
  return t;
}
DDistros ddistros(const evg_ctx* c) {
  DDistros d;
  d.n = c->Dn; d.task_off = c->b_taskoff.as<int64_t>(); d.group_off = c->b_groupoff.as<int64_t>();
  d.cfg = c->b_cfg.as<evg_distro_cfg>(); d.gmax = c->b_gmax.as<int32_t>(); d.unit_base = c->b_unitbase.as<int64_t>();
  return d;
}
DWork dwork(const evg_ctx* c) {
  DWork w;
  w.has_dep = c->b_hasdep.as<uint8_t>(); w.head = c->b_head.as<uint32_t>(); w.next = c->b_next.as<uint32_t>();
  w.pair_slot = c->b_pslot.as<uint32_t>(); w.edge_task = c->b_etask.as<uint32_t>();
  w.edge_live = c->b_elive.as<uint8_t>(); w.route = c->b_route.as<uint8_t>();
  w.err = c->b_err.as<int>();
  w.unit_v = c->b_unitv.as<int64_t>(); w.unit_a = c->b_unita.as<uint32_t>(); w.unit_n = c->b_unitn.as<uint32_t>();
  w.unit_mask = c->b_unitmask.as<unsigned long long>();
  w.best_pair = c->b_bestpair.as<uint32_t>();
  w.buf[0].key_v = c->b_kv.as<uint64_t>();
  w.qinfo = c->b_qinfo.as<evg_queue_info>(); w.ginfo = c->b_ginfo.as<evg_group_info>();
  return w;
}
DGen dgen(const evg_ctx* c) {
  DGen g;
  g.n_tiles = c->NT;
  g.tile0 = 0;
  g.tile_distro = c->b_tiledistro.as<int32_t>(); g.tile_start = c->b_tilestart.as<int64_t>();
  g.dtile_off = c->b_dtileoff.as<int64_t>();
  g.vmm = c->b_vmm.as<unsigned long long>();
  for (int k = 0; k < 2; k++) {
    g.key_lo[k] = c->b_klo[k].as<uint32_t>(); g.key_hi[k] = c->b_khi[k].as<uint32_t>(); g.idx[k] = c->b_ix[k].as<uint32_t>();
  }
  g.e = c->b_e.as<uint32_t>(); g.tile_sum = c->b_tilesum.as<uint32_t>(); g.tile_hist = c->b_tilehist.as<uint32_t>();
  g.wl = c->b_wl.as<uint4>();
  g.pay = c->b_pay.as<URec>();
  g.pown = c->b_place.as<uint32_t>();
  g.pver = c->b_place.as<uint32_t>() + (c->Tgc + 1);
  g.pedge = c->b_eplace.as<uint32_t>();
  g.sedge = c->b_eplace.as<uint32_t>() + (c->E + 1);
  g.ccount = c->b_gmisc.as<unsigned int>();
  g.maxpass = c->b_gmisc.as<int32_t>() + 1;
  g.rcount = c->b_gmisc.as<unsigned int>() + 2;
  g.hcount = c->b_gmisc.as<unsigned int>() + 3;
  g.bcount = c->b_gmisc.as<unsigned int>() + 4;
  g.blist = c->b_blist.as<uint2>();
  g.rank = c->b_rank.as<uint32_t>();
  g.hlist = c->b_hlist.as<uint2>();
  g.usum = c->b_usum.as<uint4>();
  g.run = c->b_run.as<uint32_t>();
  g.tie = c->b_tie.as<uint4>();
  g.tv = c->b_tv.as<int64_t>();
  return g;
}

#define LOCK(c) std::lock_guard<std::recursive_mutex> lock_((c)->mu)
#define LAUNCH_ON(c, st, kernel, grid, block, ...)                           \
  do {                                                                       \
    if ((grid) > 0) {                                                        \
      kernel<<<(grid), (block), 0, (st)>>>(__VA_ARGS__);                     \
      (c)->launches++;                                                       \
    }                                                                        \
  } while (0)
#define LAUNCH(c, kernel, grid, block, ...) LAUNCH_ON(c, (c)->stream, kernel, grid, block, __VA_ARGS__)

int run_alloc_range(evg_ctx* c, int64_t now, int32_t d0, int32_t d1) {
  DHosts h;
  h.n = c->H; h.flags = c->b_hflags.as<uint32_t>(); h.gid = c->b_hgid.as<int32_t>();
  h.expected = c->b_hexp.as<int64_t>(); h.stddev = c->b_hstd.as<int64_t>(); h.start = c->b_hstart.as<int64_t>();
  h.host_off = c->b_hostoff.as<int64_t>(); h.cfg = c->b_acfg.as<evg_alloc_cfg>();
  if (c->ext_result && c->ext_capacity < c->Dn) return fail(EVG_ERR_INVALID, "bound result buffer holds %lld rows, need %d", (long long)c->ext_capacity, c->Dn);
  CK(c->b_gs.ensure(sizeof(GroupScratch) * size_t(c->G + 1)));
  const int split = (d1 - d0) >= 4096 ? 1 : 0;
  const bool listed = split && c->alist_valid && d0 == 0 && d1 == c->Dn;
  const int32_t* al = listed ? c->b_alist.as<int32_t>() : nullptr;
  const int64_t teams = listed ? c->n_alist : int64_t(d1 - d0);
  if (c->max_groups > kWideAllocGroups)
    LAUNCH(c, k_alloc<128>, unsigned(teams), 128, h, d0, d1, c->b_groupoff.as<int64_t>(), c->b_qinfo.as<evg_queue_info>(),
           c->b_ginfo.as<evg_group_info>(), c->b_gs.as<GroupScratch>(), now, c->result_ptr(), c->b_status.as<int32_t>(), split, al, int32_t(c->n_alist));
  else
    LAUNCH(c, k_alloc<32>, grid_for(teams, 4), 128, h, d0, d1, c->b_groupoff.as<int64_t>(), c->b_qinfo.as<evg_queue_info>(),
           c->b_ginfo.as<evg_group_info>(), c->b_gs.as<GroupScratch>(), now, c->result_ptr(), c->b_status.as<int32_t>(), split, al, int32_t(c->n_alist));
  if (split)
    LAUNCH(c, k_alloc_groupless, grid_for(d1 - d0, 128), 128, h, d0, d1, c->b_groupoff.as<int64_t>(), c->b_qinfo.as<evg_queue_info>(), now,
           c->result_ptr(), c->b_status.as<int32_t>());
  CK(cudaGetLastError());
  return EVG_OK;
}
int run_alloc(evg_ctx* c, int64_t now) { return run_alloc_range(c, now, 0, c->Dn); }

template <int THREADS, int ITEMS, int MIN_CTAS>
int launch_smem(evg_ctx* c, cudaStream_t st, const DTasks& dt, const DDistros& dd, const DWork& w, const int32_t* list, int32_t n,
                int64_t now, int lists_needed = 0, const int32_t* list_count = nullptr) {
  if (n <= 0) return EVG_OK;
  const size_t bytes = PlanSmem<THREADS, ITEMS>::kBytes;
  CK(cudaFuncSetAttribute(k_plan_smem<THREADS, ITEMS, MIN_CTAS>, cudaFuncAttributeMaxDynamicSharedMemorySize, int(bytes)));
  k_plan_smem<THREADS, ITEMS, MIN_CTAS><<<unsigned(n), THREADS, bytes, st>>>(dt, dd, w, list, list_count, now, lists_needed,
                                                                          c->b_order.as<int32_t>(), c->b_tv.as<int64_t>());
  c->launches++;
  return EVG_OK;
}

template <int THREADS, int CAP, int OCC>
int launch_cta(evg_ctx* c, cudaStream_t st, const DTasks& dt, const DDistros& dd, const DWork& w, const int32_t* list, int32_t n,
               int64_t now, int32_t* punt_list, int32_t* punt_count) {
  if (n <= 0) return EVG_OK;
  const size_t bytes = PlanCta<THREADS, CAP>::kBytes;
  CK(cudaFuncSetAttribute(k_plan_cta<THREADS, CAP, OCC>, cudaFuncAttributeMaxDynamicSharedMemorySize, int(bytes)));
  k_plan_cta<THREADS, CAP, OCC><<<unsigned(n), THREADS, bytes, st>>>(dt, dd, w, list, now, c->t_pad, c->b_order.as<int32_t>(),
                                                                  c->b_tv.as<int64_t>(), punt_list, punt_count);
  c->launches++;
  return EVG_OK;
}

int launch_tiny(evg_ctx* c, cudaStream_t st, const DTasks& dt, const DDistros& dd, const DWork& w, const int32_t* list, int32_t n,
                int64_t now, int lists_needed) {
  if (n <= 0) return EVG_OK;
  if (lists_needed) return launch_smem<128, 8, 8>(c, st, dt, dd, w, list, n, now, 1);
  k_plan_warp<<<grid_for(int64_t(n) * 32, 256), 256, 0, st>>>(dt, dd, w, list, n, now, c->b_order.as<int32_t>(), c->b_tv.as<int64_t>());
  c->launches++;
  return EVG_OK;
}

int prepare_general(evg_ctx* c, cudaStream_t s, int32_t d0, int32_t d1) {
  const int64_t t0 = c->h_taskoff[d0], t1 = c->h_taskoff[d1], u0 = c->h_unitbase[d0], u1 = c->h_unitbase[d1];
  const int64_t g0 = c->h_groupoff[d0], g1 = c->h_groupoff[d1], e0 = c->h_edgeoff[d0], e1 = c->h_edgeoff[d1];
  CK(cudaMemsetAsync(c->b_qinfo.as<evg_queue_info>() + d0, 0, sizeof(evg_queue_info) * size_t(d1 - d0), s));
  if (g1 > g0) CK(cudaMemsetAsync(c->b_ginfo.as<evg_group_info>() + g0, 0, sizeof(evg_group_info) * size_t(g1 - g0), s));
  if (c->general_complex) {
    const size_t nt = size_t(t1 - t0);
    CK(cudaMemsetAsync(c->b_hasdep.as<uint8_t>() + t0, 0, nt, s));
    CK(cudaMemsetAsync(c->b_unitn.as<uint32_t>() + u0, 0, sizeof(uint32_t) * size_t(u1 - u0), s));
  }
  return EVG_OK;
}

int run_general(evg_ctx* c, cudaStream_t st, const DTasks& dt, const DDistros& dd, const DWork& w, int64_t now, int32_t gfirst,
                int32_t gcount) {
  if (gcount <= 0) return EVG_OK;
  DGen g = dgen(c);
  const int gc = c->general_complex;
  const std::vector<int32_t>& gh = c->routes[kGeneral].h;
  const int32_t d_first = gh[size_t(gfirst)], d_last = gh[size_t(gfirst + gcount - 1)];
  g.tile0 = c->h_dtileoff[size_t(d_first)];
  const unsigned nt = unsigned(c->h_dtileoff[size_t(d_last) + 1] - g.tile0);
  const int32_t* gl = c->routes[kGeneral].b.as<int32_t>() + gfirst;
  LAUNCH_ON(c, st, k_ginit, grid_for(gcount, 256), 256, g, gl, gcount);
  if (gc && c->E > 0) LAUNCH_ON(c, st, k_gmark, nt, 256, dt, dd, w, g);
  if (c->timed) CK(cudaEventRecord(c->ev_gt0, st));
  LAUNCH_ON(c, st, k_gtask, nt, 256, dt, dd, w, g, now, gc);
  if (c->timed) { CK(cudaEventRecord(c->ev_gt1, st)); c->general_timed = true; }
  const unsigned wl_grid = unsigned(std::min<int64_t>(std::max<int64_t>(1, (c->Tgc + 255) / 256), int64_t(c->num_sms) * 16));
  if (gc) {
    LAUNCH_ON(c, st, k_glink, wl_grid, 256, dt, dd, w, g, now);
    LAUNCH_ON(c, st, k_galloc, wl_grid, 256, dt, dd, w, g);
    LAUNCH_ON(c, st, k_gfill, wl_grid, 256, dt, dd, w, g);
    LAUNCH_ON(c, st, k_gunit, wl_grid, 256, dd, w, g, now);
    LAUNCH_ON(c, st, k_grank, wl_grid, 256, w, g);
    LAUNCH_ON(c, st, k_gbest, wl_grid, 256, dt, dd, w, g, c->bd_valid ? 1 : 0);
  }
  LAUNCH_ON(c, st, k_gsched, grid_for(gcount, 128), 128, g, gl, gcount);
  if (gc) {
    LAUNCH_ON(c, st, k_gsum, nt, 256, dd, g);
    LAUNCH_ON(c, st, k_gscan, unsigned(gcount), 1024, g, gl);
  }
  LAUNCH_ON(c, st, k_gplace, nt, 256, dd, w, g, gc);
  if (gc) LAUNCH_ON(c, st, k_gplace_disp, wl_grid, 256, dt, dd, w, g);
  if (c->timed) CK(cudaEventRecord(c->ev_sort0, st));
  for (int j = 0; j < 8; j++) {
    LAUNCH_ON(c, st, k_ghist, nt, 256, j, dd, g);
    LAUNCH_ON(c, st, k_gdscan, unsigned(gcount), 1024, j, gl, g);
    LAUNCH_ON(c, st, k_gscatter, nt, 256, j, dd, g);
  }
  if (c->timed) CK(cudaEventRecord(c->ev_sort1, st));
  LAUNCH_ON(c, st, k_gemit, nt, 256, dd, g, c->b_order.as<int32_t>(), c->b_tv.as<int64_t>());
  const int64_t g0 = c->h_groupoff[size_t(d_first)], g1 = c->h_groupoff[size_t(d_last) + 1];
  LAUNCH_ON(c, st, k_finalize_info, grid_for(std::max<int64_t>(d_last + 1 - d_first, g1 - g0), 256), 256, dd, w, d_first, d_last + 1, g0, g1);
  return EVG_OK;
}

int ensure_aux_streams(evg_ctx* c) {
  if (c->ev_fork) return EVG_OK;
  for (int k = 0; k < evg_ctx::kAux; k++) {
    CK(cudaStreamCreateWithFlags(&c->s_aux[k], cudaStreamNonBlocking));
    CK(cudaEventCreateWithFlags(&c->ev_join[k], cudaEventDisableTiming));
  }
  CK(cudaEventCreateWithFlags(&c->ev_fork, cudaEventDisableTiming));
  return EVG_OK;
}

enum class Mode { kResident, kBreakdown, kPipelined };

int plan_route(evg_ctx* c, int r, Mode mode, cudaStream_t st, const DTasks& dt, const DDistros& dd, const DWork& w, int64_t now,
               int32_t first, int32_t n, int32_t* punt, int32_t* punt_count) {
  if (n <= 0) return EVG_OK;
  const int bd = mode == Mode::kBreakdown ? 1 : 0;
  const int32_t* list = punt;
  if (r != kPunted) list = (mode != Mode::kPipelined && largest_first(r) ? c->routes[r].lpt : c->routes[r].b).as<int32_t>() + first;
  if (bd && is_cta(r)) return launch_smem<EVG_C_THREADS, EVG_C_ITEMS, 1>(c, st, dt, dd, w, list, n, now, 1);
  int rc;
  switch (r) {
    case kCtaC: return launch_cta<kNT_C, kNCapC, kNOccC>(c, st, dt, dd, w, list, n, now, punt, punt_count);
    case kCtaB: return launch_cta<kNT_B, kNCapB, kNOccB>(c, st, dt, dd, w, list, n, now, punt, punt_count);
    case kCtaA:
      if (mode == Mode::kResident) {
        if ((rc = launch_cta<kNT_A, kNCapA, kNOccA>(c, st, dt, dd, w, list, c->nNA_big, now, punt, punt_count)) != EVG_OK) return rc;
        return launch_cta<kNT_S, kNCapS, kNOccS>(c, st, dt, dd, w, list + c->nNA_big, n - c->nNA_big, now, punt, punt_count);
      }
      return launch_cta<kNT_A, kNCapA, kNOccA>(c, st, dt, dd, w, list, n, now, punt, punt_count);
    case kPunted:
      if (mode == Mode::kResident && c->max_cta_tasks <= kCapA) return launch_smem<128, 8, 8>(c, st, dt, dd, w, list, n, now, 0, punt_count);
      if (mode == Mode::kResident && c->max_cta_tasks <= kCapB) return launch_smem<256, 16, 3>(c, st, dt, dd, w, list, n, now, 0, punt_count);
      return launch_smem<EVG_C_THREADS, EVG_C_ITEMS, 1>(c, st, dt, dd, w, list, n, now, 0, punt_count);
    case kSmemC: return launch_smem<EVG_C_THREADS, EVG_C_ITEMS, 1>(c, st, dt, dd, w, list, n, now, bd);
    case kSmemB: return launch_smem<256, 16, 3>(c, st, dt, dd, w, list, n, now, bd);
    case kSmemA: return launch_smem<128, 8, 8>(c, st, dt, dd, w, list, n, now, bd);
    case kWarp: return launch_tiny(c, st, dt, dd, w, list, n, now, bd);
    default: {
      const std::vector<int32_t>& gh = c->routes[kGeneral].h;
      if (mode == Mode::kPipelined && (rc = prepare_general(c, st, gh[size_t(first)], gh[size_t(first + n - 1)] + 1)) != EVG_OK) return rc;
      return run_general(c, st, dt, dd, w, now, first, n);
    }
  }
}

int run_plan(evg_ctx* c, int64_t now, uint32_t opts) {
  const int64_t T = c->T;
  const int32_t D = c->Dn;
  cudaStream_t s = c->stream;
  DTasks dt = dtasks(c);
  DDistros dd = ddistros(c);
  DWork w = dwork(c);
  int64_t* bd = nullptr;
  c->bd_valid = false;
  if (opts & EVG_OPT_BREAKDOWN) {
    CK(c->b_bd.ensure(sizeof(int64_t) * EVG_BD_N * size_t(T + 1)));
    bd = c->b_bd.as<int64_t>();
    c->bd_valid = true;
  }
  c->sort_slot = -1;
  if (D == 0) {
    if (c->timed) { CK(cudaEventRecord(c->ev_sort0, s)); CK(cudaEventRecord(c->ev_sort1, s)); }
    return EVG_OK;
  }
  const std::vector<int32_t>& gh = c->routes[kGeneral].h;
  const bool general = !gh.empty();
  if (bd && c->any_complex) CK(cudaMemsetAsync(c->b_bestpair.p, 0xFF, sizeof(uint32_t) * size_t(T + 1), s));
  const int32_t n_new = bd ? 0 : c->routes[kCtaA].n() + c->routes[kCtaB].n() + c->routes[kCtaC].n();
  if (n_new > 0) CK(cudaMemsetAsync(c->b_puntcnt.p, 0, sizeof(int32_t), s));
  if (general) { int rcg = prepare_general(c, s, gh.front(), gh.back() + 1); if (rcg != EVG_OK) return rcg; }
  bool busy[evg_ctx::kAux] = {};
  for (int r = 0; r < kRoutes; r++) busy[kRouteStream[r]] |= c->routes[r].n() > 0;
  const bool fork = std::count(busy, busy + evg_ctx::kAux, true) > 1;
  if (fork) {
    int rc0 = ensure_aux_streams(c);
    if (rc0 != EVG_OK) return rc0;
    CK(cudaEventRecord(c->ev_fork, s));
    for (int k = 0; k < evg_ctx::kAux; k++) CK(cudaStreamWaitEvent(c->s_aux[k], c->ev_fork, 0));
  }
  int rc;
  const int slot = int(c->runs % evg_ctx::kRing);
  const Mode mode = bd ? Mode::kBreakdown : Mode::kResident;
  for (int r : {kCtaC, kCtaB, kCtaA, kPunted, kSmemC, kSmemB, kSmemA, kWarp, kGeneral}) {
    const int32_t n = r == kPunted ? n_new : c->routes[r].n();
    cudaStream_t sr = fork ? c->s_aux[kRouteStream[r]] : s;
    const bool time_it = c->timed && !general && c->sort_slot < 0 && n > 0 && (r == kSmemC || (r == kCtaC && !bd));
    if (time_it) CK(cudaEventRecord(c->ring0[slot], sr));
    if ((rc = plan_route(c, r, mode, sr, dt, dd, w, now, 0, n, c->b_punt.as<int32_t>(), c->b_puntcnt.as<int32_t>())) != EVG_OK) return rc;
    if (time_it) { CK(cudaEventRecord(c->ring1[slot], sr)); c->runs++; c->sort_slot = slot; }
  }
  if (fork) {
    for (int k = 0; k < evg_ctx::kAux; k++) {
      CK(cudaEventRecord(c->ev_join[k], c->s_aux[k]));
      CK(cudaStreamWaitEvent(s, c->ev_join[k], 0));
    }
  }
  if (bd) LAUNCH(c, k_breakdown, grid_for(T, 256), 256, dt, dd, w, c->b_run.as<uint32_t>(), c->b_pay.as<URec>(), now, c->any_complex, c->b_order.as<int32_t>(), bd);
  CK(cudaGetLastError());
  return EVG_OK;
}

}

extern "C" {

const char* evg_last_error(void) { return g_err.c_str(); }
int evg_abi_version(void) { return EVG_ABI_VERSION; }

int evg_init(int device, void* stream, evg_ctx** out) {
  if (!out) return fail(EVG_ERR_INVALID, "evg_init: out is null");
  *out = nullptr;
  int n = 0;
  cudaError_t e = cudaGetDeviceCount(&n);
  if (e != cudaSuccess || n == 0) return fail(EVG_ERR_CUDA, "no CUDA device: %s (libevgsched has no CPU fallback)", cudaGetErrorString(e));
  if (device < 0 || device >= n) return fail(EVG_ERR_INVALID, "device %d out of range (%d devices)", device, n);
  CK(cudaSetDevice(device));
  cudaDeviceProp prop;
  CK(cudaGetDeviceProperties(&prop, device));
  if (prop.major != 9 || prop.minor != 0)
    return fail(EVG_ERR_CUDA, "device %d is sm_%d%d; this library is built for sm_90a only", device, prop.major, prop.minor);
  evg_ctx* c = new evg_ctx();
  c->device = device;
  c->num_sms = prop.multiProcessorCount;
  if (stream) { c->stream = reinterpret_cast<cudaStream_t>(stream); c->own_stream = false; }
  else { CK(cudaStreamCreateWithFlags(&c->stream, cudaStreamNonBlocking)); c->own_stream = true; }
  CK(cudaEventCreate(&c->ev_begin)); CK(cudaEventCreate(&c->ev_sort0));
  CK(cudaEventCreate(&c->ev_sort1)); CK(cudaEventCreate(&c->ev_end));
  CK(cudaEventCreate(&c->ev_gt0)); CK(cudaEventCreate(&c->ev_gt1));
  for (int k = 0; k < evg_ctx::kRing; k++) { CK(cudaEventCreate(&c->ring0[k])); CK(cudaEventCreate(&c->ring1[k])); }
  *out = c;
  return EVG_OK;
}

void evg_shutdown(evg_ctx* c) {
  if (!c) return;
  cudaSetDevice(c->device);
  cudaStreamSynchronize(c->stream);
  for (int k = 0; k < evg_ctx::kRing; k++) { if (c->ring0[k]) cudaEventDestroy(c->ring0[k]); if (c->ring1[k]) cudaEventDestroy(c->ring1[k]); }
  cudaEventDestroy(c->ev_begin); cudaEventDestroy(c->ev_sort0); cudaEventDestroy(c->ev_sort1); cudaEventDestroy(c->ev_end);
  cudaEventDestroy(c->ev_gt0); cudaEventDestroy(c->ev_gt1);
  for (int k = 0; k < evg_ctx::kMaxChunks; k++) { if (c->ev_h[k]) cudaEventDestroy(c->ev_h[k]); if (c->ev_c[k]) cudaEventDestroy(c->ev_c[k]); }
  if (c->s_h2d) cudaStreamDestroy(c->s_h2d);
  if (c->s_d2h) cudaStreamDestroy(c->s_d2h);
  for (int k = 0; k < evg_ctx::kAux; k++) { if (c->s_aux[k]) cudaStreamDestroy(c->s_aux[k]); if (c->ev_join[k]) cudaEventDestroy(c->ev_join[k]); }
  if (c->ev_fork) cudaEventDestroy(c->ev_fork);
  if (c->own_stream) cudaStreamDestroy(c->stream);
  delete c;
}

static int upload(evg_ctx* c, const char* who, const evg_task_soa* tasks, const evg_distro_table* distros, const evg_host_soa* hosts,
                  const int64_t* host_off, const evg_alloc_cfg* acfg, Tick kind, Cols cols = Cols::kCopy,
                  const int64_t* edge_off = nullptr) {
  CK(cudaSetDevice(c->device));
  int rc = upload_tasks(c, who, tasks, distros, cols, edge_off);
  if (rc != EVG_OK) return rc;
  if (hosts) {
    rc = upload_hosts(c, who, hosts, host_off, acfg, distros->n_distros);
    if (rc != EVG_OK) return rc;
    CK(cudaStreamSynchronize(c->stream));
  }
  c->tick.kind = kind;
  return EVG_OK;
}
int evg_upload(evg_ctx* c, const evg_task_soa* tasks, const evg_distro_table* distros, const evg_host_soa* hosts,
               const int64_t* host_off, const evg_alloc_cfg* acfg) {
  if (!c) return fail(EVG_ERR_INVALID, "null context");
  LOCK(c);
  return upload(c, "evg_upload", tasks, distros, hosts, host_off, acfg, Tick::kOwn);
}

__global__ void k_gather_i64(const int64_t* __restrict__ src, const int64_t* __restrict__ at, int64_t* __restrict__ out, int n) {
  const int i = blockIdx.x * blockDim.x + threadIdx.x;
  if (i < n) out[i] = src[at[i]];
}

__global__ void __launch_bounds__(256) k_update_rows(int64_t n, const int64_t* __restrict__ rows, int64_t T, int32_t* priority, int32_t* numdep,
                                                     int32_t* tgo, uint32_t* flags, int64_t* expected, int64_t* qbasis, int64_t* wbasis,
                                                     const int32_t* v_priority, const int32_t* v_numdep, const int32_t* v_tgo,
                                                     const uint32_t* v_flags, const int64_t* v_expected, const int64_t* v_qbasis,
                                                     const int64_t* v_wbasis, int* bad) {
  const int64_t i = int64_t(blockIdx.x) * blockDim.x + threadIdx.x;
  if (i >= n) return;
  const int64_t r = rows[i];
  if (r < 0 || r >= T) { *bad = 1; return; }
  priority[r] = v_priority[i]; numdep[r] = v_numdep[i]; tgo[r] = v_tgo[i]; flags[r] = v_flags[i];
  expected[r] = v_expected[i]; qbasis[r] = v_qbasis[i]; wbasis[r] = v_wbasis[i];
}

int evg_update_tasks(evg_ctx* c, int64_t n_rows, const int64_t* rows, const evg_task_soa* v) {
  if (!c) return fail(EVG_ERR_INVALID, "null context");
  LOCK(c);
  if (const int rc = need_tick(c, "evg_update_tasks", Need::kOwnColumns); rc != EVG_OK) return rc;
  if (n_rows < 0) return fail(EVG_ERR_INVALID, "negative row count");
  if (n_rows == 0) return EVG_OK;
  if (!rows || !v || v->n_tasks != n_rows || !v->priority || !v->num_dependents || !v->task_group_order || !v->flags || !v->expected_ns ||
      !v->queue_basis_ns || !v->wait_basis_ns)
    return fail(EVG_ERR_INVALID, "evg_update_tasks: rows and a %lld-row value table (priority, num_dependents, task_group_order, flags, "
                                 "expected_ns, queue_basis_ns, wait_basis_ns) are required", (long long)n_rows);
  CK(cudaSetDevice(c->device));
  cudaStream_t s = c->stream;
  const size_t n = size_t(n_rows);
  CK(c->b_upd.ensure(n * 48 + 64));
  unsigned char* base = c->b_upd.as<unsigned char>();
  int64_t* d_rows = reinterpret_cast<int64_t*>(base);
  int64_t* d_exp = d_rows + n; int64_t* d_qb = d_exp + n; int64_t* d_wb = d_qb + n;
  int32_t* d_prio = reinterpret_cast<int32_t*>(d_wb + n); int32_t* d_nd = d_prio + n; int32_t* d_tgo = d_nd + n;
  uint32_t* d_fl = reinterpret_cast<uint32_t*>(d_tgo + n);
  CK(cudaMemcpyAsync(d_rows, rows, n * 8, cudaMemcpyHostToDevice, s));
  CK(cudaMemcpyAsync(d_exp, v->expected_ns, n * 8, cudaMemcpyHostToDevice, s));
  CK(cudaMemcpyAsync(d_qb, v->queue_basis_ns, n * 8, cudaMemcpyHostToDevice, s));
  CK(cudaMemcpyAsync(d_wb, v->wait_basis_ns, n * 8, cudaMemcpyHostToDevice, s));
  CK(cudaMemcpyAsync(d_prio, v->priority, n * 4, cudaMemcpyHostToDevice, s));
  CK(cudaMemcpyAsync(d_nd, v->num_dependents, n * 4, cudaMemcpyHostToDevice, s));
  CK(cudaMemcpyAsync(d_tgo, v->task_group_order, n * 4, cudaMemcpyHostToDevice, s));
  CK(cudaMemcpyAsync(d_fl, v->flags, n * 4, cudaMemcpyHostToDevice, s));
  int* bad = reinterpret_cast<int*>(base + n * 48);
  CK(cudaMemsetAsync(bad, 0, sizeof(int), s));
  k_update_rows<<<grid_for(n_rows, 256), 256, 0, s>>>(n_rows, d_rows, c->T, c->tasks.prio.as<int32_t>(), c->tasks.nd.as<int32_t>(), c->tasks.tgo.as<int32_t>(),
                                                      c->tasks.flags.as<uint32_t>(), c->tasks.exp.as<int64_t>(), c->tasks.qb.as<int64_t>(), c->tasks.wb.as<int64_t>(),
                                                      d_prio, d_nd, d_tgo, d_fl, d_exp, d_qb, d_wb, bad);
  CK(cudaGetLastError());
  int h_bad = 0;
  CK(cudaMemcpyAsync(&h_bad, bad, sizeof(int), cudaMemcpyDeviceToHost, s));
  CK(cudaStreamSynchronize(s));
  if (h_bad) return fail(EVG_ERR_INVALID, "evg_update_tasks: a row index is outside [0, n_tasks)");
  c->tick.deps = false;
  return EVG_OK;
}

int evg_upload_device(evg_ctx* c, const evg_task_soa* tasks, const evg_distro_table* distros, const evg_host_soa* hosts,
                      const int64_t* host_off, const evg_alloc_cfg* acfg) {
  if (!c) return fail(EVG_ERR_INVALID, "null context");
  LOCK(c);
  if (!tasks || !distros) return fail(EVG_ERR_INVALID, "null task table / distro table");
  CK(cudaSetDevice(c->device));
  std::vector<int64_t> edge_off;
  const int32_t D = distros->n_distros;
  if (tasks->n_edges > 0 && D > 0) {
    if (!tasks->dep_off || !distros->task_off) return fail(EVG_ERR_INVALID, "null dep_off / task_off");
    edge_off.resize(size_t(D) + 1);
    CK(c->b_rn0.ensure(sizeof(int64_t) * size_t(D + 1)));
    CK(c->b_rn1.ensure(sizeof(int64_t) * size_t(D + 1)));
    CK(cudaMemcpyAsync(c->b_rn0.p, distros->task_off, sizeof(int64_t) * size_t(D + 1), cudaMemcpyHostToDevice, c->stream));
    k_gather_i64<<<grid_for(D + 1, 256), 256, 0, c->stream>>>(tasks->dep_off, c->b_rn0.as<int64_t>(), c->b_rn1.as<int64_t>(), D + 1);
    CK(cudaMemcpyAsync(edge_off.data(), c->b_rn1.p, sizeof(int64_t) * size_t(D + 1), cudaMemcpyDeviceToHost, c->stream));
    CK(cudaStreamSynchronize(c->stream));
  }
  return upload(c, "evg_upload_device", tasks, distros, hosts, host_off, acfg, Tick::kBorrowed, Cols::kAdopt,
                edge_off.empty() ? nullptr : edge_off.data());
}

int evg_run_resident(evg_ctx* c, int64_t now_ns, uint32_t opts) {
  if (!c) return fail(EVG_ERR_INVALID, "null context");
  LOCK(c);
  if (const int rc = need_tick(c, "evg_run_resident", Need::kTick); rc != EVG_OK) return rc;
  CK(cudaSetDevice(c->device));
  c->launches = 0;
  c->timed = true;
  c->general_timed = false;
  CK(cudaEventRecord(c->ev_begin, c->stream));
  int rc = run_plan(c, now_ns, opts);
  if (rc != EVG_OK) return rc;
  if (c->tick.hosts) {
    rc = run_alloc(c, now_ns);
    if (rc != EVG_OK) return rc;
  }
  CK(cudaEventRecord(c->ev_end, c->stream));
  return EVG_OK;
}

int evg_download(evg_ctx* c, evg_plan_out* po, evg_alloc_out* ao) {
  if (!c) return fail(EVG_ERR_INVALID, "null context");
  LOCK(c);
  if (const int rc = need_tick(c, "evg_download", Need::kTick); rc != EVG_OK) return rc;
  CK(cudaSetDevice(c->device));
  cudaStream_t s = c->stream;
  if (po) {
    if (po->order && c->T) CK(cudaMemcpyAsync(po->order, c->b_order.p, sizeof(int32_t) * size_t(c->T), cudaMemcpyDeviceToHost, s));
    if (po->total_value && c->T) CK(cudaMemcpyAsync(po->total_value, c->b_tv.p, sizeof(int64_t) * size_t(c->T), cudaMemcpyDeviceToHost, s));
    if (po->breakdown && c->T) {
      if (!c->bd_valid) return fail(EVG_ERR_STATE, "breakdown requested but the run did not set EVG_OPT_BREAKDOWN");
      CK(cudaMemcpyAsync(po->breakdown, c->b_bd.p, sizeof(int64_t) * EVG_BD_N * size_t(c->T), cudaMemcpyDeviceToHost, s));
    }
    if (po->info && c->Dn) CK(cudaMemcpyAsync(po->info, c->b_qinfo.p, sizeof(evg_queue_info) * size_t(c->Dn), cudaMemcpyDeviceToHost, s));
    if (po->group_info && c->G) CK(cudaMemcpyAsync(po->group_info, c->b_ginfo.p, sizeof(evg_group_info) * size_t(c->G), cudaMemcpyDeviceToHost, s));
  }
  if (ao) {
    if (const int rc = need_tick(c, "evg_download", Need::kHosts); rc != EVG_OK) return rc;
    if (ao->result && c->Dn) CK(cudaMemcpyAsync(ao->result, c->result_ptr(), sizeof(evg_alloc_result) * size_t(c->Dn), cudaMemcpyDeviceToHost, s));
    if (ao->status && c->Dn) CK(cudaMemcpyAsync(ao->status, c->b_status.p, sizeof(int32_t) * size_t(c->Dn), cudaMemcpyDeviceToHost, s));
  }
  CK(cudaStreamSynchronize(s));
  return EVG_OK;
}

__global__ void __launch_bounds__(256) k_project_queue(DTasks T, DDistros D, const int64_t* __restrict__ item_off, int64_t n_items,
                                                       const int32_t* __restrict__ order, const int64_t* __restrict__ total_value,
                                                       evg_queue_item* __restrict__ items) {
  const int64_t j = int64_t(blockIdx.x) * blockDim.x + threadIdx.x;
  if (j >= n_items) return;
  const int d = find_distro(item_off, 0, D.n - 1, j);
  const int64_t base = D.task_off[d];
  const int64_t r = j - item_off[d];
  const int32_t i = order[base + r];
  const int64_t t = base + i;
  const int32_t gid = T.gid[t];
  evg_queue_item q;
  q.task = i;
  q.group_index = T.tgo[t];
  q.group_max_hosts = gid >= 0 ? D.gmax[D.group_off[d] + gid] : 0;
  q.flags = (T.flags[t] & EVG_TF_DEPS_MET) ? EVG_QI_DEPS_MET : 0u;
  q.priority = T.priority[t];
  q.expected_ns = T.expected[t];
  q.total_value = total_value[base + r];
  items[j] = q;
}

int evg_download_queue(evg_ctx* c, int32_t cap, int64_t* item_off, evg_queue_item* items, int64_t items_capacity) {
  if (!c) return fail(EVG_ERR_INVALID, "null context");
  LOCK(c);
  if (const int rc = need_tick(c, "evg_download_queue", Need::kTick); rc != EVG_OK) return rc;
  if (cap < 0 || !item_off) return fail(EVG_ERR_INVALID, "evg_download_queue: bad argument");
  if (cap == 0) cap = EVG_PERSISTED_QUEUE_CAP;
  const int32_t D = c->Dn;
  item_off[0] = 0;
  for (int32_t d = 0; d < D; d++) item_off[d + 1] = item_off[d] + std::min<int64_t>(c->h_taskoff[d + 1] - c->h_taskoff[d], cap);
  const int64_t n = item_off[D];
  if (n > items_capacity || (n > 0 && !items)) return fail(EVG_ERR_INVALID, "evg_download_queue: %lld rows needed, %lld available", (long long)n, (long long)items_capacity);
  if (n == 0) return EVG_OK;
  CK(cudaSetDevice(c->device));
  cudaStream_t s = c->stream;
  CK(c->b_rn0.ensure(sizeof(int64_t) * size_t(D + 1)));
  CK(c->b_rn1.ensure(sizeof(evg_queue_item) * size_t(n)));
  CK(cudaMemcpyAsync(c->b_rn0.p, item_off, sizeof(int64_t) * size_t(D + 1), cudaMemcpyHostToDevice, s));
  k_project_queue<<<grid_for(n, 256), 256, 0, s>>>(dtasks(c), ddistros(c), c->b_rn0.as<int64_t>(), n, c->b_order.as<int32_t>(),
                                                 c->b_tv.as<int64_t>(), c->b_rn1.as<evg_queue_item>());
  CK(cudaGetLastError());
  CK(cudaMemcpyAsync(items, c->b_rn1.p, sizeof(evg_queue_item) * size_t(n), cudaMemcpyDeviceToHost, s));
  CK(cudaStreamSynchronize(s));
  return EVG_OK;
}

void* evg_device_result_ptr(evg_ctx* c) { return c ? (void*)c->result_ptr() : nullptr; }
int evg_bind_result_buffer(evg_ctx* c, void* device_ptr, int64_t capacity) {
  if (!c) return fail(EVG_ERR_INVALID, "null context");
  LOCK(c);
  if (device_ptr && capacity < 0) return fail(EVG_ERR_INVALID, "negative capacity");
  c->ext_result = reinterpret_cast<evg_alloc_result*>(device_ptr);
  c->ext_capacity = device_ptr ? capacity : 0;
  return EVG_OK;
}
int64_t evg_last_launch_count(evg_ctx* c) { return c ? c->launches : 0; }

int evg_last_timing_ms(evg_ctx* c, float* total_ms, float* sort_ms) {
  if (!c || !c->timed) return fail(EVG_ERR_STATE, "no timed run");
  LOCK(c);
  CK(cudaSetDevice(c->device));
  CK(cudaEventSynchronize(c->ev_end));
  if (total_ms) CK(cudaEventElapsedTime(total_ms, c->ev_begin, c->ev_end));
  if (sort_ms) {
    if (c->sort_slot >= 0) CK(cudaEventElapsedTime(sort_ms, c->ring0[c->sort_slot], c->ring1[c->sort_slot]));
    else if (c->general_timed) CK(cudaEventElapsedTime(sort_ms, c->ev_sort0, c->ev_sort1));
    else *sort_ms = 0.0f;
  }
  return EVG_OK;
}

int evg_general_timing_ms(evg_ctx* c, float* task_pass_ms, float* sort_ms) {
  if (!c) return fail(EVG_ERR_INVALID, "null context");
  LOCK(c);
  if (!c->timed || !c->general_timed) return fail(EVG_ERR_STATE, "the last timed run had no general-path distro");
  CK(cudaSetDevice(c->device));
  CK(cudaEventSynchronize(c->ev_end));
  if (task_pass_ms) CK(cudaEventElapsedTime(task_pass_ms, c->ev_gt0, c->ev_gt1));
  if (sort_ms) CK(cudaEventElapsedTime(sort_ms, c->ev_sort0, c->ev_sort1));
  return EVG_OK;
}

int evg_kernel_timing_ms(evg_ctx* c, float* out_ms, int32_t n) {
  if (!c || !out_ms || n < 0) return fail(EVG_ERR_INVALID, "evg_kernel_timing_ms: bad argument");
  LOCK(c);
  if (n > evg_ctx::kRing || n > c->runs) return fail(EVG_ERR_STATE, "only %lld timed runs recorded (ring of %d)", (long long)c->runs, evg_ctx::kRing);
  CK(cudaSetDevice(c->device));
  for (int32_t k = 0; k < n; k++) {
    const int slot = int((c->runs - n + k) % evg_ctx::kRing);
    CK(cudaEventSynchronize(c->ring1[slot]));
    CK(cudaEventElapsedTime(out_ms + k, c->ring0[slot], c->ring1[slot]));
  }
  return EVG_OK;
}

int evg_plan_batch(evg_ctx* c, const evg_task_soa* tasks, const evg_distro_table* distros, int64_t now_ns, uint32_t opts,
                   evg_plan_out* out) {
  if (!c) return fail(EVG_ERR_INVALID, "null context");
  LOCK(c);
  int rc = upload(c, "evg_plan_batch", tasks, distros, nullptr, nullptr, nullptr, Tick::kFixed);
  if (rc != EVG_OK) return rc;
  rc = evg_run_resident(c, now_ns, opts);
  if (rc != EVG_OK) return rc;
  return evg_download(c, out, nullptr);
}

static int plan_and_alloc_pipelined(evg_ctx* c, const evg_task_soa* t, const evg_distro_table* dt, const evg_host_soa* hosts,
                                    const int64_t* host_off, const evg_alloc_cfg* acfg, int64_t now, evg_plan_out* po,
                                    evg_alloc_out* ao) {
  const int64_t T = c->T, E = c->E;
  const int32_t D = c->Dn;
  if (!c->s_h2d) {
    CK(cudaStreamCreateWithFlags(&c->s_h2d, cudaStreamNonBlocking));
    CK(cudaStreamCreateWithFlags(&c->s_d2h, cudaStreamNonBlocking));
    for (int k = 0; k < evg_ctx::kMaxChunks; k++) {
      CK(cudaEventCreateWithFlags(&c->ev_h[k], cudaEventDisableTiming));
      CK(cudaEventCreateWithFlags(&c->ev_c[k], cudaEventDisableTiming));
    }
  }
  cudaStream_t s = c->stream;
  DTasks dtk = dtasks(c);
  DDistros dd = ddistros(c);
  DWork w = dwork(c);
  if (c->ext_result && c->ext_capacity < D) return fail(EVG_ERR_INVALID, "bound result buffer too small");
  CK(c->b_gs.ensure(sizeof(GroupScratch) * size_t(c->G + 1)));
  c->launches = 0;
  c->timed = false;
  c->bd_valid = false;
  CK(cudaMemsetAsync(c->b_puntcnt.p, 0, sizeof(int32_t) * (evg_ctx::kMaxChunks + 2), s));
  const int n_chunks = int(std::min<int64_t>(evg_ctx::kMaxChunks, std::max<int64_t>(1, T / (1 << 20))));
  std::vector<int32_t> cut(size_t(n_chunks) + 1, D);
  cut[0] = 0;
  {
    int32_t d = 0;
    for (int k = 1; k < n_chunks; k++) {
      const int64_t want = T * k / n_chunks;
      while (d < D && c->h_taskoff[d] < want) d++;
      cut[k] = d;
    }
  }
  auto sub = [](const std::vector<int32_t>& v, int32_t d0, int32_t d1, int32_t* first) {
    auto a = std::lower_bound(v.begin(), v.end(), d0), b = std::lower_bound(v.begin(), v.end(), d1);
    *first = int32_t(a - v.begin());
    return int32_t(b - a);
  };
#define H2D(buf, ptr, off, count, type)                                                                  \
  if ((count) > 0) CK(cudaMemcpyAsync((buf).as<type>() + (off), (ptr) + (off), sizeof(type) * size_t(count), cudaMemcpyHostToDevice, c->s_h2d))
#define D2H(dst, src, off, count, type)                                                                  \
  if ((dst) && (count) > 0) CK(cudaMemcpyAsync((dst) + (off), (src) + (off), sizeof(type) * size_t(count), cudaMemcpyDeviceToHost, c->s_d2h))
  int rc;
  for (int k = 0; k < n_chunks; k++) {
    const int32_t d0 = cut[k], d1 = cut[k + 1];
    if (d1 <= d0) continue;
    const int64_t t0 = c->h_taskoff[d0], n = c->h_taskoff[d1] - t0;
    const int64_t g0 = c->h_groupoff[d0], ng = c->h_groupoff[d1] - g0;
    H2D(c->tasks.prio, t->priority, t0, n, int32_t);
    H2D(c->tasks.exp, t->expected_ns, t0, n, int64_t);
    H2D(c->tasks.qb, t->queue_basis_ns, t0, n, int64_t);
    H2D(c->tasks.wb, t->wait_basis_ns, t0, n, int64_t);
    H2D(c->tasks.nd, t->num_dependents, t0, n, int32_t);
    H2D(c->tasks.tgo, t->task_group_order, t0, n, int32_t);
    H2D(c->tasks.gid, t->group_id, t0, n, int32_t);
    H2D(c->tasks.vid, t->version_id, t0, n, int32_t);
    H2D(c->tasks.flags, t->flags, t0, n, uint32_t);
    if (E > 0) {
      const int64_t e0 = t->dep_off[t0], ne = t->dep_off[t0 + n] - e0;
      H2D(c->b_depoff, t->dep_off, t0, n + 1, int64_t);
      H2D(c->b_depidx, t->dep_idx, e0, ne, int32_t);
    }
    CK(cudaEventRecord(c->ev_h[k], c->s_h2d));
    CK(cudaStreamWaitEvent(s, c->ev_h[k], 0));
    k_validate<<<grid_for(n, 256), 256, 0, s>>>(dtk, dd, w, t0, t0 + n);
    int32_t* pl = c->b_punt.as<int32_t>() + d0;
    int32_t* pc = c->b_puntcnt.as<int32_t>() + 1 + k;
    int32_t n_cta = 0;
    for (int r : {kCtaC, kCtaB, kCtaA, kPunted, kGeneral, kSmemC, kSmemB, kSmemA, kWarp}) {
      int32_t first = 0, cnt = n_cta;
      if (r != kPunted) cnt = sub(c->routes[r].h, d0, d1, &first);
      if (is_cta(r)) n_cta += cnt;
      if ((rc = plan_route(c, r, Mode::kPipelined, s, dtk, dd, w, now, first, cnt, pl, pc)) != EVG_OK) return rc;
    }
    if ((rc = run_alloc_range(c, now, d0, d1)) != EVG_OK) return rc;
    CK(cudaEventRecord(c->ev_c[k], s));
    CK(cudaStreamWaitEvent(c->s_d2h, c->ev_c[k], 0));
    if (po) {
      D2H(po->order, c->b_order.as<int32_t>(), t0, n, int32_t);
      D2H(po->total_value, c->b_tv.as<int64_t>(), t0, n, int64_t);
      D2H(po->info, c->b_qinfo.as<evg_queue_info>(), d0, d1 - d0, evg_queue_info);
      D2H(po->group_info, c->b_ginfo.as<evg_group_info>(), g0, ng, evg_group_info);
    }
    if (ao) {
      D2H(ao->result, c->result_ptr(), d0, d1 - d0, evg_alloc_result);
      D2H(ao->status, c->b_status.as<int32_t>(), d0, d1 - d0, int32_t);
    }
  }
#undef H2D
#undef D2H
  CK(cudaGetLastError());
  int bad = 0;
  CK(cudaMemcpyAsync(&bad, c->b_err.p, sizeof(int), cudaMemcpyDeviceToHost, s));
  CK(cudaStreamSynchronize(c->s_d2h));
  CK(cudaStreamSynchronize(s));
  if (bad) { drop_tick(c); return fail(EVG_ERR_INVALID, "a group_id / version_id / dep_idx is out of range for its distro"); }
  return EVG_OK;
}

int evg_plan_and_alloc_batch(evg_ctx* c, const evg_task_soa* tasks, const evg_distro_table* distros,
                             const evg_host_soa* hosts, const int64_t* host_off, const evg_alloc_cfg* acfg, int64_t now_ns,
                             uint32_t opts, evg_plan_out* plan_out, evg_alloc_out* alloc_out) {
// ... 1774 lines not shown
```

### evergreen_b200/scheduler.py

```python
from __future__ import annotations

import ctypes as C
from dataclasses import dataclass
from typing import Callable, Dict, List, Optional, Sequence, Tuple

import numpy as np

from . import _lib as L
from . import model as M
from . import soa as S

RUNNER_NAME = "scheduler"
PLANNER_VERSION_GPU_TUNABLE = "gpu-tunable"
HOST_ALLOCATOR_GPU_UTILIZATION = "gpu-utilization"


class AllocatorError(Exception):
    MESSAGES = {
        L.EVG_ALLOC_ERR_FUTURE_FRACTION: "future host factor cannot be greater than 1",
        L.EVG_ALLOC_ERR_POOL_SIZE: "unable to plan hosts for distro due to pool size",
        L.EVG_ALLOC_ERR_PARENT_MISSING: "error finding parent distros",
    }

    def __init__(self, status: int, distro_id: str = ""):
# ... 4 lines not shown
class Engine:

    def __init__(self, device: int = 0, stream: Optional[int] = None):
        self.lib = L.load()
        h = C.c_void_p()
        L.check(self.lib.evg_init(int(device), C.c_void_p(stream) if stream else None, C.byref(h)))
        self.ctx = h
        self._n_tasks = self._n_distros = self._n_groups = 0
        self._has_hosts = False
        self._n_dur = (0, 0)
        self._pinned = {}

    def close(self) -> None:
        if getattr(self, "ctx", None):
            for addr, _ in self._pinned.values():
                self.lib.evg_host_free(C.c_void_p(addr))
            self._pinned = {}
            self.lib.evg_shutdown(self.ctx)
            self.ctx = None

    def _out(self, name: str, shape, dtype) -> np.ndarray:
        dtype = np.dtype(dtype)
        n = int(np.prod(shape)) if np.ndim(shape) else int(shape)
        nbytes = max(n * dtype.itemsize, 1)
        addr, cap = self._pinned.get(name, (0, 0))
        if cap < nbytes:
            if addr:
                self.lib.evg_host_free(C.c_void_p(addr))
            cap = nbytes + nbytes // 8
            addr = self.lib.evg_host_alloc(cap)
            if not addr:
                raise L.EvgError(L.EVG_ERR_NOMEM, L.last_error())
            self._pinned[name] = (addr, cap)
        buf = (C.c_uint8 * nbytes).from_address(addr)
        return np.frombuffer(buf, dtype=dtype, count=n).reshape(shape)

    def _plan_output(self, T: int, D: int, G: int, breakdown: bool) -> S.PlanOutput:
        info = self._out("info", D, L.QUEUE_INFO_DTYPE)
        ginfo = self._out("group_info", G, L.GROUP_INFO_DTYPE)
        return S.PlanOutput(self._out("order", T, np.int32), self._out("total_value", T, np.int64), info, ginfo,
                            self._out("breakdown", (T, L.EVG_BD_N), np.int64) if breakdown else None)

    def _alloc_output(self, D: int) -> S.AllocOutput:
        return S.AllocOutput(self._out("result", D, L.ALLOC_RESULT_DTYPE), self._out("status", D, np.int32))

    def __del__(self):
        try:
            self.close()
        except Exception:
            pass

    def upload(self, tasks: S.TaskSoA, distros: S.DistroTable, hosts: Optional[S.HostSoA] = None) -> None:
        ts, ds = tasks.struct(), distros.struct()
        if hosts is not None:
            hs = hosts.struct()
            L.check(self.lib.evg_upload(self.ctx, C.byref(ts), C.byref(ds), C.byref(hs), L.ptr(hosts.host_off),
                                        L.ptr(hosts.cfg) if hosts.cfg.shape[0] else None))
        else:
            L.check(self.lib.evg_upload(self.ctx, C.byref(ts), C.byref(ds), None, None, None))
        self._n_tasks, self._n_distros, self._n_groups = tasks.n_tasks, distros.n_distros, distros.n_groups
        self._has_hosts = hosts is not None

    def upload_with_deps(self, tasks: S.TaskSoA, distros: S.DistroTable, hosts: Optional[S.HostSoA], deps: "S.DepsTable",
                         dep_finished: Optional[np.ndarray], now: int) -> None:
        ts, ds, dp = tasks.struct(), distros.struct(), deps.struct()
        fin = None
        if dep_finished is not None and dep_finished.shape[0]:
            fin = np.ascontiguousarray(dep_finished, dtype=np.int64)
        if hosts is not None:
            hs = hosts.struct()
            L.check(self.lib.evg_upload_with_deps(self.ctx, C.byref(ts), C.byref(ds), C.byref(hs), L.ptr(hosts.host_off),
                                                  L.ptr(hosts.cfg) if hosts.cfg.shape[0] else None, C.byref(dp), L.ptr(fin), int(now)))
        else:
            L.check(self.lib.evg_upload_with_deps(self.ctx, C.byref(ts), C.byref(ds), None, None, None, C.byref(dp), L.ptr(fin), int(now)))
        self._n_tasks, self._n_distros, self._n_groups = tasks.n_tasks, distros.n_distros, distros.n_groups
        self._has_hosts = hosts is not None

    def download_deps(self):
        met = self._out("deps_met", self._n_tasks, np.uint8)
        stamp = self._out("deps_stamp", self._n_tasks, np.int64)
        L.check(self.lib.evg_download_deps(self.ctx, L.ptr(met) if self._n_tasks else None, L.ptr(stamp) if self._n_tasks else None))
        return met, stamp

    def upload_device(self, cols: dict, n_tasks: int, distros: S.DistroTable, hosts: Optional[S.HostSoA] = None,
                      n_edges: int = 0) -> None:
        ts = L.TaskSoAStruct(int(n_tasks), int(n_edges), *[cols.get(name) for name, _ in S.TaskSoA.COLUMNS],
                             cols.get("dep_off"), cols.get("dep_idx"))
        ds = distros.struct()
        if hosts is not None:
            hs = hosts.struct()
            L.check(self.lib.evg_upload_device(self.ctx, C.byref(ts), C.byref(ds), C.byref(hs), L.ptr(hosts.host_off),
                                               L.ptr(hosts.cfg) if hosts.cfg.shape[0] else None))
        else:
            L.check(self.lib.evg_upload_device(self.ctx, C.byref(ts), C.byref(ds), None, None, None))
        self._n_tasks, self._n_distros, self._n_groups = int(n_tasks), distros.n_distros, distros.n_groups
        self._has_hosts = hosts is not None

    def update_tasks(self, rows: np.ndarray, values: S.TaskSoA) -> None:
        rows = np.ascontiguousarray(rows, dtype=np.int64)
        values = values.normalize()
        if values.n_tasks != rows.shape[0]:
            raise ValueError("one value row per updated task slot")
        vs = values.struct()
        L.check(self.lib.evg_update_tasks(self.ctx, int(rows.shape[0]), L.ptr(rows), C.byref(vs)))

    def edit_tasks(self, edit: S.TaskEdit, distros: S.DistroTable, hosts: Optional[S.HostSoA] = None) -> None:
        es, keep = edit.normalize().struct()
        ds = distros.struct()
        hargs = (None, None, None)
        if hosts is not None:
            hs = hosts.struct()
            hargs = (C.byref(hs), L.ptr(hosts.host_off), L.ptr(hosts.cfg) if hosts.cfg.shape[0] else None)
        L.check(self.lib.evg_edit_tasks(self.ctx, C.byref(es), C.byref(ds), *hargs))
        del keep
        self._n_tasks, self._n_distros, self._n_groups = int(distros.task_off[-1]), distros.n_distros, distros.n_groups
        self._has_hosts = hosts is not None

    def run(self, now: int, opts: int = 0) -> None:
        L.check(self.lib.evg_run_resident(self.ctx, int(now), int(opts)))

    def download(self, want_breakdown: bool = False, want_alloc: Optional[bool] = None):
        T, D, G = self._n_tasks, self._n_distros, self._n_groups
        po = self._plan_output(T, D, G, want_breakdown)
        ps = L.PlanOutStruct(L.ptr(po.order), L.ptr(po.total_value),
                             L.ptr(po.breakdown) if want_breakdown else None, L.ptr(po.info), L.ptr(po.group_info))
        ao = None
        if want_alloc is None:
            want_alloc = self._has_hosts
        if want_alloc:
            ao = self._alloc_output(D)
            as_ = L.AllocOutStruct(L.ptr(ao.result), L.ptr(ao.status))
            L.check(self.lib.evg_download(self.ctx, C.byref(ps), C.byref(as_)))
        else:
            L.check(self.lib.evg_download(self.ctx, C.byref(ps), None))
        return po, ao

    def download_queue(self, cap: int = 0, task_off=None):
        D = self._n_distros
        item_off = self._out("queue_item_off", D + 1, np.int64)
        cap_eff = cap or L.EVG_PERSISTED_QUEUE_CAP
        n = self._n_tasks if task_off is None else int(np.minimum(np.diff(task_off), cap_eff).sum())
        items = self._out("queue_items", max(n, 1), L.QUEUE_ITEM_DTYPE)
        L.check(self.lib.evg_download_queue(self.ctx, int(cap), L.ptr(item_off), L.ptr(items), int(max(n, 1))))
        return item_off, items[: int(item_off[D])]

    def bind_result_buffer(self, device_ptr: int, capacity_rows: int) -> None:
        L.check(self.lib.evg_bind_result_buffer(self.ctx, C.c_void_p(device_ptr) if device_ptr else None, int(capacity_rows)))

    def device_result_ptr(self) -> int:
        return int(self.lib.evg_device_result_ptr(self.ctx) or 0)

    def last_launch_count(self) -> int:
        return int(self.lib.evg_last_launch_count(self.ctx))

    def last_timing_ms(self) -> Tuple[float, float]:
        a, b = C.c_float(), C.c_float()
        L.check(self.lib.evg_last_timing_ms(self.ctx, C.byref(a), C.byref(b)))
        return a.value, b.value

    def general_timing_ms(self) -> Tuple[float, float]:
        a, b = C.c_float(), C.c_float()
        L.check(self.lib.evg_general_timing_ms(self.ctx, C.byref(a), C.byref(b)))
        return float(a.value), float(b.value)

    def kernel_timing_ms(self, n: int):
        buf = (C.c_float * max(n, 1))()
        L.check(self.lib.evg_kernel_timing_ms(self.ctx, buf, int(n)))
        return [buf[k] for k in range(n)]

    def plan_batch(self, tasks: S.TaskSoA, distros: S.DistroTable, now: int, breakdown: bool = False) -> S.PlanOutput:
        T, D, G = tasks.n_tasks, distros.n_distros, distros.n_groups
        po = self._plan_output(T, D, G, breakdown)
        ps = L.PlanOutStruct(L.ptr(po.order), L.ptr(po.total_value), L.ptr(po.breakdown) if breakdown else None,
                             L.ptr(po.info), L.ptr(po.group_info))
        ts, ds = tasks.struct(), distros.struct()
        L.check(self.lib.evg_plan_batch(self.ctx, C.byref(ts), C.byref(ds), int(now),
                                        L.EVG_OPT_BREAKDOWN if breakdown else 0, C.byref(ps)))
        self._n_tasks, self._n_distros, self._n_groups, self._has_hosts = T, D, G, False
        return po

    def plan_and_alloc_batch(self, tasks: S.TaskSoA, distros: S.DistroTable, hosts: S.HostSoA, now: int,
                             breakdown: bool = False):
        T, D, G = tasks.n_tasks, distros.n_distros, distros.n_groups
        po = self._plan_output(T, D, G, breakdown)
        ao = self._alloc_output(D)
        ps = L.PlanOutStruct(L.ptr(po.order), L.ptr(po.total_value), L.ptr(po.breakdown) if breakdown else None,
                             L.ptr(po.info), L.ptr(po.group_info))
        as_ = L.AllocOutStruct(L.ptr(ao.result), L.ptr(ao.status))
        ts, ds, hs = tasks.struct(), distros.struct(), hosts.struct()
        L.check(self.lib.evg_plan_and_alloc_batch(self.ctx, C.byref(ts), C.byref(ds), C.byref(hs), L.ptr(hosts.host_off),
                                                  L.ptr(hosts.cfg) if hosts.cfg.shape[0] else None, int(now),
                                                  L.EVG_OPT_BREAKDOWN if breakdown else 0, C.byref(ps), C.byref(as_)))
        self._n_tasks, self._n_distros, self._n_groups, self._has_hosts = T, D, G, True
        return po, ao

    def deps_met_batch(self, deps: "S.DepsTable") -> np.ndarray:
        met = self._out("deps_met", deps.n_tasks, np.uint8)
        st = deps.struct()
        L.check(self.lib.evg_deps_met_batch(self.ctx, C.byref(st), L.ptr(met) if deps.n_tasks else None))
        return met

    def find_runnable_batch(self, table: "S.RunnableTable"):
        runnable = self._out("runnable", table.n_tasks, np.int32)
        count = self._out("runnable_count", table.n_distros, np.int64)
        st, keep = table.struct()
        outs = (L.ptr(runnable) if table.n_tasks else None, L.ptr(count) if table.n_distros else None)
        if table.pipe is None:
            L.check(self.lib.evg_find_runnable_batch(self.ctx, C.byref(st), *outs))
        else:
            ps = table.pipe.struct()
            L.check(self.lib.evg_find_runnable_ex(self.ctx, C.byref(st), C.byref(ps), *outs))
        del keep
        return runnable, count

    def plan_from_finder(self, table: "S.RunnableTable", candidates: S.TaskSoA, distros: S.DistroTable,
                         hosts: Optional[S.HostSoA], dep_finished: Optional[np.ndarray], now: int):
        if table.deps is None:
            raise ValueError("plan_from_finder needs the candidates' dependency table")
        runnable = self._out("runnable", table.n_tasks, np.int32)
        count = self._out("runnable_count", table.n_distros, np.int64)
        st, keep = table.struct()
        ts, ds = candidates.normalize().struct(), distros.struct()
        fin = None if dep_finished is None else np.ascontiguousarray(dep_finished, dtype=np.int64)
        hargs = (None, None, None)
        if hosts is not None:
            hs = hosts.struct()
            hargs = (C.byref(hs), L.ptr(hosts.host_off), L.ptr(hosts.cfg) if hosts.cfg.shape[0] else None)
        rest = (*hargs, L.ptr(fin) if fin is not None and fin.shape[0] else None, int(now),
                L.ptr(runnable) if table.n_tasks else None, L.ptr(count) if table.n_distros else None)
        if table.pipe is None:
            L.check(self.lib.evg_plan_from_finder(self.ctx, C.byref(st), C.byref(ts), C.byref(ds), *rest))
        else:
            ps = table.pipe.struct()
            L.check(self.lib.evg_plan_from_finder_ex(self.ctx, C.byref(st), C.byref(ps), C.byref(ts), C.byref(ds), *rest))
        del keep
        self._n_tasks, self._n_distros, self._n_groups = int(count.sum()), distros.n_distros, distros.n_groups
        self._has_hosts = hosts is not None
        return runnable, count

    def plan_aliases(self, table: "S.AliasTable", cfg: np.ndarray, now: int):
        D = int(cfg.shape[0])
        cfg = np.ascontiguousarray(cfg, dtype=L.DISTRO_CFG_DTYPE)
        task_off, group_off = np.zeros(D + 1, np.int64), np.zeros(D + 1, np.int64)
        n_versions = np.zeros(max(D, 1), np.int32)
        st, keep = table.normalize().struct()
        out = L.AliasOutStruct(L.ptr(task_off), L.ptr(group_off), L.ptr(n_versions))
        L.check(self.lib.evg_plan_aliases(self.ctx, C.byref(st), L.ptr(cfg) if D else None, D, int(now), C.byref(out)))
        del keep
        self._n_tasks, self._n_distros, self._n_groups = int(task_off[D]), D, int(group_off[D])
        self._has_hosts = False
        return task_off, group_off, n_versions[:D]

    def download_alias_map(self):
        src = self._out("alias_source_row", self._n_tasks, np.int32)
        gsrc = self._out("alias_group_source", self._n_groups, np.int32)
        L.check(self.lib.evg_download_alias_map(self.ctx, L.ptr(src) if self._n_tasks else None,
                                                L.ptr(gsrc) if self._n_groups else None))
        return src, gsrc

    def expected_durations_batch(self, rows: "S.DurationRows") -> np.ndarray:
        out = self._out("duration_stats", rows.n_keys, L.DURATION_STAT_DTYPE)
        st = rows.struct()
        L.check(self.lib.evg_expected_durations_batch(self.ctx, C.byref(st), L.ptr(out) if rows.n_keys else None))
        return out

    def resolve_durations(self, history: Optional["S.DurationHistory"], now: int, tasks: Optional["S.DurationCache"] = None,
                          hosts: Optional["S.DurationCache"] = None) -> None:
        keep = []
        din = L.DurationInStruct()
        if history is not None:
            hs = history.rows.struct()
            keep.append(hs)
            din.history = C.pointer(hs)
            din.n_pairs = history.n_pairs
            off = np.ascontiguousarray(history.pair_key_off, dtype=np.int64)
            keep.append(off)
            din.pair_key_off = L.ptr(off)
        for name, cache in (("tasks", tasks), ("hosts", hosts)):
            if cache is not None:
                cs = cache.normalize().struct()
                keep.append(cs)
                setattr(din, name, C.pointer(cs))
        L.check(self.lib.evg_resolve_durations(self.ctx, C.byref(din), int(now)))
        self._n_dur = (tasks.n_rows if tasks is not None else 0, hosts.n_rows if hosts is not None else 0)
        del keep

    def download_durations(self):
        res = []
        for side, n in zip(("tasks", "hosts"), self._n_dur):
            res.append({f: self._out(f"dur_{side}_{f}", n, np.uint8 if f == "source" else np.int64) for f in L.DURATION_OUT_FIELDS})
        outs = [L.DurationOutStruct(*[L.ptr(d[f]) if d[f].shape[0] else None for f in L.DURATION_OUT_FIELDS]) for d in res]
        L.check(self.lib.evg_download_durations(self.ctx, C.byref(outs[0]), C.byref(outs[1])))
        return res[0], res[1]

    def prioritize_legacy_batch(self, table: "S.LegacyTable"):
        T, D = table.n_tasks, table.n_distros
        order = self._out("legacy_order", T, np.int32)
        count = self._out("legacy_count", D, np.int64)
        status = self._out("legacy_status", D, np.int32)
        ts = table.struct()
        L.check(self.lib.evg_prioritize_legacy_batch(self.ctx, C.byref(ts), L.ptr(table.task_off), L.ptr(table.list_mode), D,
                                                     L.ptr(order) if T else None, L.ptr(count), L.ptr(status)))
        return order, count, status

    def dag_rebuild_batch(self, item_off, group_off, dep_off, dep_item, group_id, group_index):
        D = int(item_off.shape[0]) - 1
# ... 643 lines not shown
```

### include/evg_sched.h

```cpp
#ifndef EVG_SCHED_H
#define EVG_SCHED_H
#include <stdint.h>

#ifdef __cplusplus
extern "C" {
#endif

#define EVG_ABI_VERSION 1

#define EVG_TIME_ZERO INT64_MIN

enum {
  EVG_OK = 0,
  EVG_ERR_INVALID = -1,
  EVG_ERR_CUDA = -2,
  EVG_ERR_NOMEM = -3,
  EVG_ERR_STATE = -4
};

enum {
  EVG_ALLOC_OK = 0,
  EVG_ALLOC_ERR_FUTURE_FRACTION = 1,
  EVG_ALLOC_ERR_POOL_SIZE = 2,
  EVG_ALLOC_ERR_PARENT_MISSING = 3
// ... 54 lines not shown
  int64_t count_free;
  int64_t count_required;
  int64_t max_hosts;
  int64_t expected_duration;
  int64_t count_duration_over_threshold;
  int64_t count_wait_over_threshold;
  int64_t count_dep_filled_merge_queue_tasks;
  int64_t duration_over_threshold;
} evg_group_info;

typedef struct {
  int64_t length;
  int64_t length_with_dependencies_met;
  int64_t count_dep_filled_merge_queue_tasks;
  int64_t expected_duration;
  int64_t max_duration_threshold;
  int64_t count_duration_over_threshold;
  int64_t duration_over_threshold;
  int64_t count_wait_over_threshold;
  int64_t secondary_queue;
  int64_t has_ungrouped;
  evg_group_info ungrouped;
} evg_queue_info;

enum {
  EVG_BD_TASK_GROUP_LENGTH = 0, EVG_BD_TOTAL_VALUE,
  EVG_BD_P_INITIAL, EVG_BD_P_TASK_GROUP, EVG_BD_P_GENERATOR, EVG_BD_P_COMMIT_QUEUE,
  EVG_BD_R_COMMIT_QUEUE, EVG_BD_R_NUM_DEPENDENTS, EVG_BD_R_ESTIMATED_RUNTIME,
  EVG_BD_R_MAINLINE_WAIT, EVG_BD_R_STEPBACK, EVG_BD_R_PATCH, EVG_BD_R_PATCH_WAIT,
  EVG_BD_N
};

typedef struct {
  int32_t* order;
  int64_t* total_value;
  int64_t* breakdown;
  evg_queue_info* info;
  evg_group_info* group_info;
} evg_plan_out;

#define EVG_HF_RUNNING 0x1u
#define EVG_HF_TEARDOWN 0x2u
#define EVG_HF_RT_FOUND 0x4u

#define EVG_HG_NONE (-1)
#define EVG_HG_UNQUEUED (-2)

typedef struct {
  int64_t n_hosts;
  const uint32_t* flags;
  const int32_t* group_id;
  const int64_t* expected_ns;
  const int64_t* std_ns;
  const int64_t* start_ns;
} evg_host_soa;

enum { EVG_PROVIDER_STATIC = 0,
       EVG_PROVIDER_EPHEMERAL = 1,
       EVG_PROVIDER_DOCKER = 2 };

typedef struct {
  double future_host_fraction;
  int32_t provider;
  int32_t disabled;
  int32_t minimum_hosts;
  int32_t maximum_hosts;
  int32_t round_up;
  int32_t waits_over_thresh_feedback;
  int32_t has_pool;
  int32_t pool_max_containers;
  int32_t parent_found;
  int32_t parent_maximum_hosts;
} evg_alloc_cfg;

typedef struct {
  int32_t new_hosts;
  int32_t free_hosts;
  int64_t deficit_ns;
} evg_alloc_result;

typedef struct {
  evg_alloc_result* result;
  int32_t* status;
} evg_alloc_out;

#define EVG_OPT_BREAKDOWN 0x1u

typedef struct evg_ctx evg_ctx;


int evg_init(int device, void* stream, evg_ctx** out);
void evg_shutdown(evg_ctx* ctx);
const char* evg_last_error(void);
int evg_abi_version(void);

void* evg_host_alloc(uint64_t bytes);
void evg_host_free(void* p);


int evg_plan_batch(evg_ctx* ctx, const evg_task_soa* tasks, const evg_distro_table* distros,
                   int64_t now_ns, uint32_t opts, evg_plan_out* out);

int evg_alloc_batch(evg_ctx* ctx, const evg_host_soa* hosts, const int64_t* host_off,
                    const evg_alloc_cfg* cfg, const evg_queue_info* info, evg_group_info* groups,
                    const int64_t* group_off, int32_t n_distros, int64_t now_ns, evg_alloc_out* out);

int evg_plan_and_alloc_batch(evg_ctx* ctx, const evg_task_soa* tasks, const evg_distro_table* distros,
                             const evg_host_soa* hosts, const int64_t* host_off,
                             const evg_alloc_cfg* acfg, int64_t now_ns, uint32_t opts,
                             evg_plan_out* plan_out, evg_alloc_out* alloc_out);


int evg_upload(evg_ctx* ctx, const evg_task_soa* tasks, const evg_distro_table* distros,
               const evg_host_soa* hosts, const int64_t* host_off, const evg_alloc_cfg* acfg);
int evg_update_tasks(evg_ctx* ctx, int64_t n_rows, const int64_t* rows, const evg_task_soa* values);

typedef struct {
  int64_t n_remove;
  const int64_t* remove_rows;
  const evg_task_soa* insert;
  const int64_t* insert_off;
  int64_t n_add_edges;
  const int64_t* add_edge_task;
  const int32_t* add_edge_dep;
  const int32_t* group_remap;
  const int32_t* version_remap;
} evg_task_edit;

int evg_edit_tasks(evg_ctx* ctx, const evg_task_edit* edit, const evg_distro_table* distros,
                   const evg_host_soa* hosts, const int64_t* host_off, const evg_alloc_cfg* acfg);

int evg_upload_device(evg_ctx* ctx, const evg_task_soa* device_tasks, const evg_distro_table* distros,
                      const evg_host_soa* hosts, const int64_t* host_off, const evg_alloc_cfg* acfg);
int evg_run_resident(evg_ctx* ctx, int64_t now_ns, uint32_t opts);
int evg_download(evg_ctx* ctx, evg_plan_out* plan_out, evg_alloc_out* alloc_out);

#define EVG_QI_DEPS_MET 0x1u
typedef struct {
  int32_t task;
  int32_t group_index;
  int32_t group_max_hosts;
  uint32_t flags;
  int64_t priority;
  int64_t expected_ns;
  int64_t total_value;
} evg_queue_item;
#define EVG_PERSISTED_QUEUE_CAP 10000

int evg_download_queue(evg_ctx* ctx, int32_t cap, int64_t* item_off, evg_queue_item* items, int64_t items_capacity);

void* evg_device_result_ptr(evg_ctx* ctx);
int evg_bind_result_buffer(evg_ctx* ctx, void* device_ptr, int64_t capacity);
int64_t evg_last_launch_count(evg_ctx* ctx);
int evg_last_timing_ms(evg_ctx* ctx, float* total_ms, float* sort_ms);

int evg_kernel_timing_ms(evg_ctx* ctx, float* out_ms, int32_t n);

int evg_general_timing_ms(evg_ctx* ctx, float* task_pass_ms, float* sort_ms);


#define EVG_DEP_IN_QUEUE 0
#define EVG_DEP_EXTERNAL 1
#define EVG_DEP_MISSING 2
#define EVG_WANT_SUCCESS 0
#define EVG_WANT_FAILED 1
#define EVG_WANT_ANY 2
#define EVG_WANT_OTHER 3
#define EVG_TS_STATUS_MASK 0x3u
#define EVG_TS_BLOCKED 0x4u
#define EVG_TP_OVERRIDE 0x1u
#define EVG_TP_MET_TIME 0x2u

typedef struct {
  int64_t n_tasks;
  int64_t n_deps;
  const int64_t* dep_off;
  const uint8_t* dep_kind;
  const int32_t* dep_ref;
  const uint8_t* dep_want;
  const uint8_t* task_state;
  const uint8_t* task_pre;
  const uint8_t* ext_state;
  int64_t n_ext;
} evg_deps_in;

int evg_deps_met_batch(evg_ctx* ctx, const evg_deps_in* in, uint8_t* met);

int evg_upload_with_deps(evg_ctx* ctx, const evg_task_soa* tasks, const evg_distro_table* distros,
                         const evg_host_soa* hosts, const int64_t* host_off, const evg_alloc_cfg* acfg,
                         const evg_deps_in* deps, const int64_t* dep_finished_ns, int64_t now_ns);
int evg_download_deps(evg_ctx* ctx, uint8_t* met, int64_t* met_time_ns);


#define EVG_SQ_ACTIVATED 0x01u
#define EVG_SQ_UNDISPATCHED 0x02u
#define EVG_SQ_PRIORITY_OK 0x04u
#define EVG_SQ_HOST_PLATFORM 0x08u
#define EVG_SQ_UNATTAINABLE 0x10u
#define EVG_SQ_OVERRIDE_DEPS 0x20u
#define EVG_SQ_GITHUB_PR 0x40u
#define EVG_SQ_PATCH_REQUEST 0x80u
#define EVG_PF_ENABLED 0x1u
#define EVG_PF_HIDDEN 0x2u
#define EVG_PF_DISPATCHING_DISABLED 0x4u
#define EVG_PF_PATCHING_DISABLED 0x8u
#define EVG_FINDER_NO_DEPS 0
#define EVG_FINDER_LEGACY 1
#define EVG_FINDER_ALTERNATE 2
#define EVG_FINDER_PIPELINE 3
#define EVG_FINDER_PIPELINE_NO_DEPS 4

typedef struct {
  int64_t n_tasks;
  int32_t n_distros;
  int32_t n_projects;
  const int64_t* task_off;
  const uint8_t* sched;
  const int32_t* project;
  const uint8_t* project_flags;
  const int64_t* valid_off;
  const int32_t* valid_idx;
  const uint8_t* finder;
  const evg_deps_in* deps;
} evg_runnable_in;

int evg_find_runnable_batch(evg_ctx* ctx, const evg_runnable_in* in, int32_t* runnable, int64_t* count);

int evg_plan_from_finder(evg_ctx* ctx, const evg_runnable_in* in, const evg_task_soa* candidates, const evg_distro_table* distros,
                         const evg_host_soa* hosts, const int64_t* host_off, const evg_alloc_cfg* acfg,
                         const int64_t* dep_finished_ns, int64_t now_ns, int32_t* runnable, int64_t* count);


#define EVG_STATUS_SUCCESS 0
#define EVG_STATUS_FAILED 1
#define EVG_STATUS_ANY 2
#define EVG_PR_ENABLED 0x1u
#define EVG_PR_DISPATCHING_DISABLED 0x2u
#define EVG_PR_PATCHING_FALSE 0x4u

typedef struct {
  int32_t n_status;
  int32_t _reserved;
  const int32_t* dep_status;
  const int32_t* task_status;
  const int32_t* ext_status;
  const uint8_t* task_unattainable;
  const uint8_t* ext_unattainable;
  const uint8_t* project_raw;
} evg_pipeline_in;

int evg_find_runnable_ex(evg_ctx* ctx, const evg_runnable_in* in, const evg_pipeline_in* pipe, int32_t* runnable,
                         int64_t* count);

int evg_plan_from_finder_ex(evg_ctx* ctx, const evg_runnable_in* in, const evg_pipeline_in* pipe, const evg_task_soa* candidates,
                            const evg_distro_table* distros, const evg_host_soa* hosts, const int64_t* host_off,
                            const evg_alloc_cfg* acfg, const int64_t* dep_finished_ns, int64_t now_ns, int32_t* runnable,
                            int64_t* count);


typedef struct {
  evg_task_soa tasks;
  int32_t n_groups;
  int32_t n_versions;
  const int32_t* group_max_hosts;
  const uint8_t* sched;
  const int32_t* task_group_max_hosts;
  const int32_t* primary;
  const int64_t* secondary_off;
  const int32_t* secondary_idx;
  int32_t n_names;
  int32_t _reserved;
  const int64_t* dest_off;
  const int32_t* dest_idx;
  const evg_deps_in* deps;
  const int64_t* dep_finished_ns;
} evg_alias_in;

typedef struct {
  int64_t* task_off;
  int64_t* group_off;
  int32_t* n_versions;
} evg_alias_out;

int evg_plan_aliases(evg_ctx* ctx, const evg_alias_in* in, const evg_distro_cfg* cfg, int32_t n_distros, int64_t now_ns,
                     evg_alias_out* out);
int evg_download_alias_map(evg_ctx* ctx, int32_t* source_row, int32_t* group_source);


typedef struct {
  const char* bytes;
  const int64_t* off;
} evg_str_col;

typedef struct {
  int64_t n_tasks;
  int32_t n_distros;
  const int64_t* task_off;
  evg_str_col id;
  evg_str_col version;
  evg_str_col group_key;
  const int32_t* group_max_hosts;
  const int64_t* dep_off;
  evg_str_col dep_id;
} evg_string_cols;

typedef struct {
// ... 149 lines not shown
```

Baseline: 4.543 billion.

## Add per-distro shared-memory units kernel with punt fallback for general path

Adds k_gunits, a one-block-per-distro kernel that runs the link/alloc/fill/unit-accumulate steps for a general distro entirely in shared memory (bitmap slot compaction, local scans, local atomics). Distros that exceed its capacity limits are handed back through a punt list, and the existing grid-wide kernels only process punted entries, found by binary search. The worklist becomes segmented per distro, and displaced tasks are compacted into a list so k_gplace_disp no longer scans everything. It runs by default only when there are at least as many general distros as SMs (or when an env var forces it), and it adds a large dynamic shared-memory footprint.

```diff
diff --git a/evergreen_b200/_lib.py b/evergreen_b200/_lib.py
--- a/evergreen_b200/_lib.py
+++ b/evergreen_b200/_lib.py
@@ -242,6 +242,7 @@
     "evg_device_result_ptr": (_P, [_P]),
     "evg_bind_result_buffer": (C.c_int, [_P, _P, C.c_int64]),
     "evg_last_launch_count": (C.c_int64, [_P]),
+    "evg_general_units": (C.c_int, [_P, C.POINTER(C.c_int64), C.POINTER(C.c_int64)]),
     "evg_last_timing_ms": (C.c_int, [_P, C.POINTER(C.c_float), C.POINTER(C.c_float)]),
     "evg_kernel_timing_ms": (C.c_int, [_P, C.POINTER(C.c_float), C.c_int32]),
     "evg_general_timing_ms": (C.c_int, [_P, C.POINTER(C.c_float), C.POINTER(C.c_float)]),
diff --git a/evergreen_b200/csrc/evg_plan_general.cuh b/evergreen_b200/csrc/evg_plan_general.cuh
--- a/evergreen_b200/csrc/evg_plan_general.cuh
+++ b/evergreen_b200/csrc/evg_plan_general.cuh
@@ -35,7 +35,13 @@
   uint32_t* tile_hist;
   uint4* wl;
   struct URec* pay;
-  unsigned int* ccount;
+  const uint32_t* wl_off;
+  unsigned int* dcount;
+  unsigned long long* punts;
+  uint2* prec;
+  uint32_t* disp;
+  unsigned int* dcnt;
+  unsigned int* ustats;
   uint4* tie;
   int32_t* maxpass;
   uint32_t* run;
@@ -83,9 +89,10 @@
 
 __global__ void k_ginit(DGen G, const int32_t* __restrict__ general_list, int n) {
   const int k = blockIdx.x * blockDim.x + threadIdx.x;
-  if (k == 0) { *G.ccount = 0u; *G.maxpass = 0; *G.rcount = 0u; *G.hcount = 0u; *G.bcount = 0u; }
+  if (k == 0) { *G.maxpass = 0; *G.rcount = 0u; *G.hcount = 0u; *G.bcount = 0u; *G.punts = 0ull; *G.dcnt = 0u; }
   if (k >= n) return;
   const int d = general_list[k];
+  G.dcount[d] = 0u;
   G.vmm[2 * d] = 0ull;
   G.vmm[2 * d + 1] = ~0ull;
 }
@@ -262,7 +269,7 @@
 #pragma unroll
       for (int w = 0; w < 8; w++) { const uint32_t x = s_wsum[w]; before += w < (tid >> 5) ? x : 0u; total += x; }
       if (total) {
-        if (tid == 0) s_lbase = atomicAdd(G.ccount, total);
+        if (tid == 0) s_lbase = G.wl_off[d] + atomicAdd(G.dcount + d, total);
         __syncthreads();
         uint32_t pos = s_lbase + before + inc - mine;
         const int32_t vid_[4] = {vid4.x, vid4.y, vid4.z, vid4.w}, tgo_[4] = {tgo4.x, tgo4.y, tgo4.z, tgo4.w};
@@ -330,6 +337,16 @@
 }
 
 
+__device__ __forceinline__ uint32_t punted_entry(const DGen& G, int np, unsigned int k) {
+  int lo = 0, hi = np - 1;
+  while (lo < hi) {
+    const int mid = (lo + hi + 1) >> 1;
+    if (G.prec[mid].y <= k) lo = mid; else hi = mid - 1;
+  }
+  const uint2 r = G.prec[lo];
+  return r.x + (k - r.y);
+}
+
 struct WlTask {
   uint32_t t; int d; int64_t base; uint32_t li; bool own_complex; uint32_t s_own, s_ver;
 };
@@ -343,20 +360,33 @@
   return x;
 }
 template <typename F>
-__device__ __forceinline__ void wl_pairs(const DTasks& T, const DGen& G, const WlTask& x, unsigned int k, F&& f) {
+__device__ __forceinline__ void wl_pairs(const DTasks& T, const DGen& G, const WlTask& x, unsigned int k, F&& f, bool edges = true) {
   if (x.own_complex) f(G.pown + k, x.s_own, true);
   if (x.s_ver != kInactive) f(G.pver + k, x.s_ver, false);
-  if (T.n_edges > 0)
+  if (edges && T.n_edges > 0)
     for (int64_t e = T.dep_off[x.t]; e < T.dep_off[x.t + 1]; e++) {
       const uint32_t sl = G.sedge[e];
       if (sl != kInactive) f(G.pedge + e, sl, false);
     }
 }
 
+__device__ __forceinline__ uint32_t edge_slot(const DTasks& T, const WlTask& x, int64_t e0, int64_t e, uint32_t ub, uint32_t ng, bool gv) {
+  const uint32_t dl = uint32_t(T.dep_idx[e]);
+  const uint32_t sl = ub + own_slot_local(T.gid[x.base + dl], T.vid[x.base + dl], dl, ng, gv);
+  bool dup = (sl == x.s_own) || (sl == x.s_ver);
+  for (int64_t f = e0; f < e && !dup; f++) {
+    const uint32_t fl2 = uint32_t(T.dep_idx[f]);
+    dup = ub + own_slot_local(T.gid[x.base + fl2], T.vid[x.base + fl2], fl2, ng, gv) == sl;
+  }
+  return dup ? kInactive : sl;
+}
+
 __global__ void __launch_bounds__(256, EVG_OCC_GLINK) k_glink(DTasks T, DDistros D, DWork W, DGen G, int64_t now) {
   if (*W.err) return;
-  const unsigned int n = *G.ccount;
-  for (unsigned int k = blockIdx.x * blockDim.x + threadIdx.x; k < n; k += gridDim.x * blockDim.x) {
+  const unsigned long long pn = *G.punts;
+  const unsigned int n = uint32_t(pn);
+  for (unsigned int j = blockIdx.x * blockDim.x + threadIdx.x; j < n; j += gridDim.x * blockDim.x) {
+    const uint32_t k = punted_entry(G, int(pn >> 32), j);
     const WlTask x = wl_task(D, G, k);
     const uint32_t t = x.t;
     const int d = x.d;
@@ -385,15 +415,9 @@
       const bool gv = D.cfg[d].group_versions != 0;
       const int64_t e0 = T.dep_off[t], e1 = T.dep_off[t + 1];
       for (int64_t e = e0; e < e1; e++) {
-        const uint32_t dl = uint32_t(T.dep_idx[e]);
-        const uint32_t sl = ub + own_slot_local(T.gid[x.base + dl], T.vid[x.base + dl], dl, ng, gv);
-        bool dup = (sl == x.s_own) || (sl == x.s_ver);
-        for (int64_t f = e0; f < e && !dup; f++) {
-          const uint32_t fl2 = uint32_t(T.dep_idx[f]);
-          dup = ub + own_slot_local(T.gid[x.base + fl2], T.vid[x.base + fl2], fl2, ng, gv) == sl;
-        }
-        G.sedge[e] = dup ? kInactive : sl;
-        if (!dup) G.pedge[e] = atomicAdd(W.unit_n + sl, 1u);
+        const uint32_t sl = edge_slot(T, x, e0, e, ub, ng, gv);
+        G.sedge[e] = sl;
+        if (sl != kInactive) G.pedge[e] = atomicAdd(W.unit_n + sl, 1u);
       }
     }
   }
@@ -403,13 +427,15 @@
   if (*W.err) return;
   __shared__ uint32_t s_wsum[8], s_wcnt[8];
   __shared__ uint32_t s_base, s_hbase;
-  const unsigned int n = *G.ccount;
+  const unsigned long long pn = *G.punts;
+  const unsigned int n = uint32_t(pn);
   const int lane = threadIdx.x & 31, warp = threadIdx.x >> 5;
   for (unsigned int k0 = blockIdx.x * blockDim.x; k0 < n; k0 += gridDim.x * blockDim.x) {
-    const unsigned int k = k0 + threadIdx.x;
     WlTask x;
+    uint32_t k = 0;
     uint32_t need = 0, heads = 0;
-    if (k < n) {
+    if (k0 + threadIdx.x < n) {
+      k = punted_entry(G, int(pn >> 32), k0 + threadIdx.x);
       x = wl_task(D, G, k);
       wl_pairs(T, G, x, k, [&](const uint32_t* place, uint32_t slot, bool) { if (*place == 0u) { need += W.unit_n[slot]; heads++; } });
     }
@@ -441,8 +467,10 @@
 
 __global__ void __launch_bounds__(256, EVG_OCC_GFILL) k_gfill(DTasks T, DDistros D, DWork W, DGen G) {
   if (*W.err) return;
-  const unsigned int n = *G.ccount;
-  for (unsigned int k = blockIdx.x * blockDim.x + threadIdx.x; k < n; k += gridDim.x * blockDim.x) {
+  const unsigned long long pn = *G.punts;
+  const unsigned int n = uint32_t(pn);
+  for (unsigned int j = blockIdx.x * blockDim.x + threadIdx.x; j < n; j += gridDim.x * blockDim.x) {
+    const uint32_t k = punted_entry(G, int(pn >> 32), j);
     const WlTask x = wl_task(D, G, k);
     wl_pairs(T, G, x, k, [&](const uint32_t* place, uint32_t slot, bool own) {
       G.run[W.head[slot] + *place] = k | (own ? kRunOwn : 0u);
@@ -539,14 +567,21 @@
 
 __global__ void __launch_bounds__(256, EVG_OCC_GBEST) k_gbest(DTasks T, DDistros D, DWork W, DGen G, int want_best_pair) {
   if (*W.err) return;
-  const unsigned int n = *G.ccount;
+  const unsigned long long pn = *G.punts;
+  const unsigned int n = uint32_t(pn);
   const unsigned full = 0xffffffffu;
   const int lane = threadIdx.x & 31;
-  for (unsigned int kw = blockIdx.x * blockDim.x + (threadIdx.x & ~31u); kw < n; kw += gridDim.x * blockDim.x) {
-    const unsigned int k = kw + lane;
+  __shared__ uint32_t s_dn, s_at;
+  if (threadIdx.x == 0) s_dn = 0u;
+  __syncthreads();
+  for (unsigned int k0 = blockIdx.x * blockDim.x; k0 < n; k0 += gridDim.x * blockDim.x) {
+    const unsigned int kw = k0 + (threadIdx.x & ~31u);
     int d = -1;
     unsigned long long kk = 0ull;
-    if (k < n) {
+    uint32_t k = 0;
+    bool displaced = false;
+    if (kw + lane < n) {
+      k = punted_entry(G, int(pn >> 32), kw + lane);
       const WlTask x = wl_task(D, G, k);
       const uint32_t t = x.t, li = x.li;
       d = x.d;
@@ -569,13 +604,24 @@
       G.tv[t] = bv;
       G.tie[k] = make_uint4(ba, brk, bslot, 0u);
       if (want_best_pair) W.best_pair[t] = bslot;
-      const bool displaced = !(ba == li && brk == 0);
+      displaced = !(ba == li && brk == 0);
       if (displaced) W.has_dep[t] |= 2;
       atomicAdd(G.e + x.base + ba, 1u);
       kk = ord_i64(bv);
     }
+    {
+      const unsigned b = __ballot_sync(full, displaced);
+      uint32_t at = 0;
+      if (lane == 0 && b) at = atomicAdd(&s_dn, uint32_t(__popc(b)));
+      __syncthreads();
+      if (threadIdx.x == 0) { s_at = s_dn ? atomicAdd(G.dcnt, s_dn) : 0u; s_dn = 0u; }
+      __syncthreads();
+      at = __shfl_sync(full, at, 0);
+      if (displaced) G.disp[s_at + at + __popc(b & ((1u << lane) - 1u))] = k;
+    }
     const int d0 = __shfl_sync(full, d, 0);
-    if (__all_sync(full, d < 0 || d == d0)) {
+    if (d0 < 0) {
+    } else if (__all_sync(full, d < 0 || d == d0)) {
       unsigned long long hi = d < 0 ? 0ull : kk, lo = d < 0 ? ~0ull : kk;
 #pragma unroll
       for (int o = 16; o > 0; o >>= 1) {
@@ -590,6 +636,304 @@
       if (kk > __ldcg(G.vmm + 2 * d)) atomicMax(G.vmm + 2 * d, kk);
       if (kk < __ldcg(G.vmm + 2 * d + 1)) atomicMin(G.vmm + 2 * d + 1, kk);
     }
+  }
+}
+
+#ifndef EVG_GUNITS_THREADS
+#define EVG_GUNITS_THREADS 1024
+#endif
+#ifndef EVG_GUNITS_OCC
+#define EVG_GUNITS_OCC 1
+#endif
+constexpr int kUSlots = 1 << 17;
+constexpr int kUWords = kUSlots / 32;
+constexpr int kUUnits = 16384;
+constexpr uint32_t kUBig = 1024;
+constexpr int kUChunks = 2048;
+constexpr int kUEntries = 1 << 16;
+struct GUnitsSmem {
+  uint32_t bits[kUWords];
+  uint32_t wpre[kUWords];
+  uint32_t head[kUUnits + 1];
+  uint32_t chunk[kUChunks];
+  uint32_t edged[kUEntries / 32];
+};
+constexpr size_t kGUnitsBytes = sizeof(GUnitsSmem);
+
+__device__ __forceinline__ WlTask gu_task(const uint4& e, int d, int64_t base) {
+  WlTask x;
+  x.t = e.x; x.d = d; x.s_own = e.z; x.s_ver = e.w;
+  x.base = base;
+  x.li = uint32_t(int64_t(e.x) - base);
+  x.own_complex = e.z != kInactive;
+  return x;
+}
+__device__ __forceinline__ uint32_t gu_uid(const GUnitsSmem& S, uint32_t ls) {
+  const uint32_t w = ls >> 5;
+  return S.wpre[w] + __popc(S.bits[w] & ((1u << (ls & 31u)) - 1u));
+}
+
+template <int NT>
+__device__ __forceinline__ uint32_t gu_scan(uint32_t* a, int n, uint32_t* s_w) {
+  const int tid = threadIdx.x, lane = tid & 31, warp = tid >> 5;
+  const int per = (n + NT - 1) / NT, lo = min(n, tid * per), hi = min(n, lo + per);
+  uint32_t sum = 0;
+  for (int i = lo; i < hi; i++) sum += a[i];
+  uint32_t inc = sum;
+#pragma unroll
+  for (int o = 1; o < 32; o <<= 1) { const uint32_t y = __shfl_up_sync(0xffffffffu, inc, o); if (lane >= o) inc += y; }
+  if (lane == 31) s_w[warp] = inc;
+  __syncthreads();
+  if (warp == 0) {
+    const uint32_t v = lane < NT / 32 ? s_w[lane] : 0u;
+    uint32_t vi = v;
+#pragma unroll
+    for (int o = 1; o < 32; o <<= 1) { const uint32_t y = __shfl_up_sync(0xffffffffu, vi, o); if (lane >= o) vi += y; }
+    s_w[lane] = vi - v;
+    if (lane == 31) s_w[32] = vi;
+  }
+  __syncthreads();
+  uint32_t run = s_w[warp] + inc - sum;
+  const uint32_t total = s_w[32];
+  for (int i = lo; i < hi; i++) { const uint32_t x = a[i]; a[i] = run; run += x; }
+  __syncthreads();
+  return total;
+}
+
+__global__ void __launch_bounds__(EVG_GUNITS_THREADS, EVG_GUNITS_OCC)
+k_gunits(DTasks T, DDistros D, DWork W, DGen G, const int32_t* __restrict__ general_list, int64_t now, int want_best_pair, int hand_back) {
+  constexpr int NT = EVG_GUNITS_THREADS;
+  extern __shared__ __align__(16) unsigned char gu_raw[];
+  GUnitsSmem& S = *reinterpret_cast<GUnitsSmem*>(gu_raw);
+  __shared__ uint32_t s_w[33];
+  __shared__ uint32_t s_nch, s_big, s_at, s_rbase;
+  __shared__ evg_distro_cfg s_cfg;
+  __shared__ unsigned long long s_vmax, s_vmin;
+  if (*W.err) return;
+  const int d = general_list[blockIdx.x];
+  const unsigned int n = G.dcount[d];
+  if (n == 0) return;
+  const int tid = threadIdx.x, lane = tid & 31, warp = tid >> 5;
+  const unsigned full = 0xffffffffu;
+  const uint32_t seg = G.wl_off[d];
+  const int64_t base = D.task_off[d];
+  const uint32_t ub = uint32_t(D.unit_base[d]), nslot = uint32_t(D.unit_base[d + 1] - D.unit_base[d]);
+  const uint32_t ng = uint32_t(D.group_off[d + 1] - D.group_off[d]);
+  auto hand_back_distro = [&]() {
+    if (tid == 0) {
+      const unsigned long long r = atomicAdd(G.punts, (1ull << 32) | (unsigned long long)n);
+      G.prec[r >> 32] = make_uint2(seg, uint32_t(r));
+      atomicAdd(G.ustats + 1, 1u);
+    }
+  };
+  if (hand_back || nslot > uint32_t(kUSlots) || n > uint32_t(kUEntries)) { hand_back_distro(); return; }
+  if (tid == 0) { s_cfg = D.cfg[d]; s_nch = 0u; s_big = 0u; s_vmax = 0ull; s_vmin = ~0ull; }
+  const int nw = int((nslot + 31) >> 5);
+  for (int w = tid; w < nw; w += NT) S.bits[w] = 0u;
+  for (uint32_t w = tid; w < (n + 31) / 32; w += NT) S.edged[w] = 0u;
+  __syncthreads();
+  const bool gv = s_cfg.group_versions != 0;
+  auto mark = [&](uint32_t slot) { const uint32_t ls = slot - ub; atomicOr(&S.bits[ls >> 5], 1u << (ls & 31u)); };
+  auto edged = [&](uint32_t i) { return T.n_edges > 0 && ((S.edged[i >> 5] >> (i & 31u)) & 1u) != 0; };
+  const uint4 e_first = tid < n ? G.wl[seg + tid] : make_uint4(0u, 0u, kInactive, kInactive);
+  uint4 nxt = e_first;
+  for (uint32_t i = tid; i < n; i += NT) {
+    const WlTask x = gu_task(nxt, d, base);
+    if (i + NT < n) nxt = G.wl[seg + i + NT];
+    if (x.own_complex) mark(x.s_own);
+    if (x.s_ver != kInactive) mark(x.s_ver);
+    if (T.n_edges > 0) {
+      const int64_t e0 = T.dep_off[x.t], e1 = T.dep_off[x.t + 1];
+      if (e1 > e0) atomicOr(&S.edged[i >> 5], 1u << (i & 31u));
+      for (int64_t e = e0; e < e1; e++) {
+        const uint32_t sl = edge_slot(T, x, e0, e, ub, ng, gv);
+        G.sedge[e] = sl;
+        if (sl != kInactive) mark(sl);
+      }
+    }
+  }
+  __syncthreads();
+  for (int w = tid; w < nw; w += NT) S.wpre[w] = uint32_t(__popc(S.bits[w]));
+  __syncthreads();
+  const uint32_t nu = gu_scan<NT>(S.wpre, nw, s_w);
+  if (nu > uint32_t(kUUnits)) { hand_back_distro(); return; }
+  for (uint32_t u = tid; u <= nu; u += NT) S.head[u] = 0u;
+  __syncthreads();
+  nxt = e_first;
+  for (uint32_t i = tid; i < n; i += NT) {
+    const uint32_t k = seg + i;
+    const WlTask x = gu_task(nxt, d, base);
+    if (i + NT < n) nxt = G.wl[k + NT];
+    if (x.own_complex) G.pown[k] = atomicAdd(&S.head[gu_uid(S, x.s_own - ub)], 1u);
+    if (x.s_ver != kInactive) G.pver[k] = atomicAdd(&S.head[gu_uid(S, x.s_ver - ub)], 1u);
+    if (edged(i))
+      for (int64_t e = T.dep_off[x.t]; e < T.dep_off[x.t + 1]; e++) {
+        const uint32_t sl = G.sedge[e];
+        if (sl != kInactive) G.pedge[e] = atomicAdd(&S.head[gu_uid(S, sl - ub)], 1u);
+      }
+  }
+  __syncthreads();
+  {
+    uint32_t mx = 0, nch = 0;
+    for (uint32_t u = tid; u < nu; u += NT) {
+      const uint32_t c = S.head[u];
+      mx = max(mx, c);
+      nch += c > kRankOne ? (c + 31u) >> 5 : 0u;
+    }
+    mx = __reduce_max_sync(full, mx);
+    nch = __reduce_add_sync(full, nch);
+    if (lane == 0) { atomicMax(&s_big, mx); atomicAdd(&s_nch, nch); }
+  }
+  __syncthreads();
+  if (s_big > kUBig || s_nch > uint32_t(kUChunks)) { hand_back_distro(); return; }
+  __syncthreads();
+  if (tid == 0) s_nch = 0u;
+  const uint32_t nrun = gu_scan<NT>(S.head, int(nu), s_w);
+  if (tid == 0) { S.head[nu] = nrun; s_rbase = atomicAdd(G.rcount, nrun); }
+  __syncthreads();
+  const uint32_t rbase = s_rbase;
+  uint32_t* run = G.run + rbase;
+  uint32_t* rank = G.rank + rbase;
+  nxt = e_first;
+  for (uint32_t i = tid; i < n; i += NT) {
+    const uint32_t k = seg + i;
+    const WlTask x = gu_task(nxt, d, base);
+    if (i + NT < n) nxt = G.wl[k + NT];
+    wl_pairs(T, G, x, k, [&](const uint32_t* place, uint32_t slot, bool own) {
+      run[S.head[gu_uid(S, slot - ub)] + *place] = k | (own ? kRunOwn : 0u);
+    }, edged(i));
+  }
+  __syncthreads();
+  const int64_t threshold = s_cfg.target_time_ns;
+  const bool incl = s_cfg.includes_dependencies != 0;
+  for (uint32_t u = tid; u < nu; u += NT) {
+    int lo = 0, hi = nw - 1;
+    while (lo < hi) { const int mid = (lo + hi + 1) >> 1; if (S.wpre[mid] <= u) lo = mid; else hi = mid - 1; }
+    const uint32_t ls = uint32_t(lo) * 32u + uint32_t(__fns(S.bits[lo], 0u, int(u - S.wpre[lo]) + 1));
+    const uint32_t slot = ub + ls;
+    const uint32_t h = S.head[u], cnt = S.head[u + 1] - h;
+    UnitAcc a;
+    acc_init(a);
+    uint32_t anchor = kNoAnchor;
+    int64_t g_cnt = 0, g_exp = 0, g_over = 0, g_sover = 0, g_wait = 0, g_mq = 0;
+    for (uint32_t i = 0; i < cnt; i++) {
+      const uint32_t q = run[h + i];
+      const URec r = rec_load(G.pay + (q & kRunEntry));
+      rec_acc(a, now, r);
+      if (q & kRunOwn) {
+        anchor = min(anchor, rec_li(r));
+        if (ls < ng) {
+          const uint32_t fl = (r.lif >> 24) & 0x3Fu;
+          const bool dm = (fl & EVG_TF_DEPS_MET) != 0;
+          const bool counted = !incl || dm;
+          const bool over = counted && r.exp_ns > threshold;
+          g_cnt += counted; g_exp += counted ? r.exp_ns : 0; g_over += over; g_sover += over ? r.exp_ns : 0;
+          g_wait += (r.lif & kRecWaitOver) != 0; g_mq += dm && (fl & EVG_TF_REQ_MASK) == EVG_TF_REQ_MERGE_QUEUE;
+        }
+      }
+    }
+    if (ls < ng) {
+      evg_group_info* g = W.ginfo + D.group_off[d] + ls;
+      g->count = g_cnt; g->expected_duration = g_exp; g->count_duration_over_threshold = g_over;
+      g->duration_over_threshold = g_sover; g->count_wait_over_threshold = g_wait; g->count_dep_filled_merge_queue_tasks = g_mq;
+    }
+    const unsigned long long v = (unsigned long long)unit_value(a, s_cfg, nullptr);
+    G.usum[slot] = make_uint4(uint32_t(v), uint32_t(v >> 32), anchor, cnt);
+    W.unit_mask[slot] = 0ull;
+    W.head[slot] = rbase + h;
+    W.unit_n[slot] = cnt;
+    if (cnt <= kRankOne) {
+      for (uint32_t i = 0; i < cnt; i++) {
+        const URec me = rec_load(G.pay + (run[h + i] & kRunEntry));
+        uint32_t rk = 0;
+        for (uint32_t j = 0; j < cnt; j++)
+          if (j != i) rk += rec_less(rec_load(G.pay + (run[h + j] & kRunEntry)), me) ? 1u : 0u;
+        rank[h + i] = rk;
+      }
+    } else {
+      const uint32_t nch = (cnt + 31u) >> 5, at = atomicAdd(&s_nch, nch);
+      for (uint32_t c = 0; c < nch; c++) S.chunk[at + c] = (u << 5) | c;
+    }
+  }
+  __syncthreads();
+  for (uint32_t c = warp; c < s_nch; c += NT / 32) {
+    const uint32_t ch = S.chunk[c], u = ch >> 5;
+    const uint32_t h = S.head[u], cnt = S.head[u + 1] - h;
+    const uint32_t i = (ch & 31u) * 32u + uint32_t(lane);
+    URec me;
+    me.tgo = 0; me.nd = 0; me.prio = 0; me.exp_ns = 0; me.lif = 0;
+    if (i < cnt) me = rec_load(G.pay + (run[h + i] & kRunEntry));
+    uint32_t rk = 0;
+    for (uint32_t j0 = 0; j0 < cnt; j0 += 32) {
+      URec o;
+      o.tgo = 0; o.nd = 0; o.prio = 0; o.exp_ns = 0; o.lif = 0;
+      if (j0 + lane < cnt) o = rec_load(G.pay + (run[h + j0 + lane] & kRunEntry));
+      const uint32_t m = min(32u, cnt - j0);
+      for (uint32_t q = 0; q < m; q++) {
+        URec y;
+        y.tgo = __shfl_sync(full, o.tgo, q); y.nd = __shfl_sync(full, o.nd, q); y.prio = __shfl_sync(full, o.prio, q);
+        y.exp_ns = __shfl_sync(full, o.exp_ns, q); y.lif = __shfl_sync(full, o.lif, q);
+        rk += (i < cnt && rec_less(y, me)) ? 1u : 0u;
+      }
+    }
+    if (i < cnt) rank[h + i] = rk;
+  }
+  __syncthreads();
+  unsigned long long kmax = 0ull, kmin = ~0ull;
+  nxt = e_first;
+  for (uint32_t i0 = 0; i0 < n; i0 += NT) {
+    const uint32_t i = i0 + tid, k = seg + i;
+    bool displaced = false;
+    if (i < n) {
+      const WlTask x = gu_task(nxt, d, base);
+      if (i + NT < n) nxt = G.wl[k + NT];
+      const uint32_t t = x.t, li = x.li;
+      bool have = false;
+      int64_t bv = 0;
+      uint32_t ba = 0, brk = 0, bslot = kInactive, bn = 1, bkx = 0;
+      if (!x.own_complex) { have = true; bv = G.tv[t]; ba = li; }
+      wl_pairs(T, G, x, k, [&](const uint32_t* place, uint32_t slot, bool) {
+        const uint4 u = G.usum[slot];
+        const uint32_t kx = *place;
+        const uint32_t a = u.z;
+        if (a == kNoAnchor) return;
+        const int64_t v = int64_t((unsigned long long)u.x | ((unsigned long long)u.y << 32));
+        if (!have || v > bv || (v == bv && a < ba)) { have = true; bv = v; ba = a; bslot = slot; bn = u.w; bkx = kx; }
+      }, edged(i));
+      if (bslot != kInactive) {
+        brk = rank[S.head[gu_uid(S, bslot - ub)] + bkx];
+        if (bn <= 64) atomicOr(&W.unit_mask[bslot], 1ull << brk);
+      }
+      G.tv[t] = bv;
+      G.tie[k] = make_uint4(ba, brk, bslot, 0u);
+      if (want_best_pair) W.best_pair[t] = bslot;
+      displaced = !(ba == li && brk == 0);
+      if (displaced) W.has_dep[t] |= 2;
+      atomicAdd(G.e + base + ba, 1u);
+      const unsigned long long kk = ord_i64(bv);
+      kmax = max(kmax, kk); kmin = min(kmin, kk);
+    }
+    const unsigned b = __ballot_sync(full, displaced);
+    if (lane == 0) s_w[warp] = uint32_t(__popc(b));
+    __syncthreads();
+    const uint32_t wc = lane < NT / 32 ? s_w[lane] : 0u;
+    const uint32_t before = __reduce_add_sync(full, lane < warp ? wc : 0u), total = __reduce_add_sync(full, wc);
+    if (tid == 0) s_at = total ? atomicAdd(G.dcnt, total) : 0u;
+    __syncthreads();
+    if (displaced) G.disp[s_at + before + __popc(b & ((1u << lane) - 1u))] = k;
+    __syncthreads();
+  }
+#pragma unroll
+  for (int o = 16; o > 0; o >>= 1) {
+    kmax = max(kmax, __shfl_xor_sync(full, kmax, o));
+    kmin = min(kmin, __shfl_xor_sync(full, kmin, o));
+  }
+  if (lane == 0) { atomicMax(&s_vmax, kmax); atomicMin(&s_vmin, kmin); }
+  __syncthreads();
+  if (tid == 0) {
+    if (s_vmax > __ldcg(G.vmm + 2 * d)) atomicMax(G.vmm + 2 * d, s_vmax);
+    if (s_vmin < __ldcg(G.vmm + 2 * d + 1)) atomicMin(G.vmm + 2 * d + 1, s_vmin);
+    atomicAdd(G.ustats, 1u);
   }
 }
 
@@ -781,11 +1125,11 @@
 }
 
 __global__ void __launch_bounds__(256) k_gplace_disp(DTasks T, DDistros D, DWork W, DGen G) {
-  const unsigned int n = *G.ccount;
-  for (unsigned int k = blockIdx.x * blockDim.x + threadIdx.x; k < n; k += gridDim.x * blockDim.x) {
+  const unsigned int n = *G.dcnt;
+  for (unsigned int j = blockIdx.x * blockDim.x + threadIdx.x; j < n; j += gridDim.x * blockDim.x) {
+  const uint32_t k = G.disp[j];
   const uint4 ent = G.wl[k];
   const uint32_t t = ent.x;
-  if (!(W.has_dep[t] & 2)) continue;
   const int d = int(ent.y);
   const int64_t base = D.task_off[d];
   const uint4 tie = G.tie[k];
diff --git a/evergreen_b200/csrc/evg_sched.cu b/evergreen_b200/csrc/evg_sched.cu
--- a/evergreen_b200/csrc/evg_sched.cu
+++ b/evergreen_b200/csrc/evg_sched.cu
@@ -1138,8 +1138,10 @@
   cudaEvent_t ev_h[kMaxChunks] = {}, ev_c[kMaxChunks] = {};
   int general_complex = 0;
   int64_t Tgc = 0;
+  int gunits = -1;
   DevBuf b_kv, b_vmm, b_klo[2], b_khi[2], b_ix[2], b_e, b_tilesum, b_gmisc;
   DevBuf b_tiledistro, b_tilestart, b_dtileoff, b_tilehist, b_wl, b_pay, b_place, b_eplace, b_run, b_rank, b_blist, b_tie, b_hlist, b_usum, b_upd;
+  DevBuf b_wloff, b_dcount, b_prec, b_disp;
   DevBuf b_qinfo, b_ginfo, b_order, b_tv, b_bd;
   DevBuf b_hflags, b_hgid, b_hexp, b_hstd, b_hstart, b_hostoff, b_acfg, b_gs, b_result, b_status;
   bool bd_valid = false;
@@ -1198,6 +1200,7 @@
   if (rc == EVG_OK && D > 0) rc = check_offsets(dt->group_off, D, -1, who, "group_off");
   if (rc != EVG_OK) return rc;
   std::vector<int64_t> unit_base(size_t(D) + 1, 0), dtile_off(size_t(D) + 1, 0);
+  std::vector<uint32_t> wl_off(size_t(D) + 1, 0);
   std::vector<int32_t> tile_distro, list[kRoutes];
   std::vector<int64_t> tile_start;
   std::vector<uint8_t> route(size_t(D) + 1, 0);
@@ -1246,6 +1249,7 @@
     if (r == kGeneral) {
       if (gb > ga || cf.group_versions || de > 0) {
         general_complex = 1;
+        wl_off[size_t(d)] = uint32_t(Tgc);
         Tgc += n;
         Prec += n + ((cf.group_versions && gb > ga) ? n : 0) + de;
       }
@@ -1297,6 +1301,7 @@
   UP(s, c->b_tiledistro, tile_distro.data(), NT, int32_t);
   UP(s, c->b_tilestart, tile_start.data(), NT, int64_t);
   UP(s, c->b_dtileoff, dtile_off.data(), D + 1, int64_t);
+  if (general_complex) UP(s, c->b_wloff, wl_off.data(), D + 1, uint32_t);
   UP(s, c->b_route, route.data(), D + 1, uint8_t);
   for (int r = 0; r < kRoutes; r++) UP(s, c->routes[r].b, list[r].data(), int64_t(list[r].size()), int32_t);
   std::vector<int32_t> lpt[kRoutes];
@@ -1344,6 +1349,8 @@
     }
     CK(c->b_vmm.ensure(sizeof(uint64_t) * 2 * size_t(D + 1)));
     CK(c->b_gmisc.ensure(64));
+    CK(cudaMemsetAsync(c->b_gmisc.p, 0, 64, s));
+    CK(c->b_dcount.ensure(sizeof(uint32_t) * size_t(D + 1)));
     CK(c->b_tilesum.ensure(sizeof(uint32_t) * size_t(NT + 1)));
     CK(c->b_tilehist.ensure(sizeof(uint32_t) * 256 * size_t(NT + 1)));
     if (general_complex) {
@@ -1358,6 +1365,8 @@
       CK(c->b_blist.ensure(sizeof(uint2) * size_t(Prec / kRankOne + 1)));
       CK(c->b_hlist.ensure(sizeof(uint2) * size_t(Prec + 1)));
       CK(c->b_usum.ensure(sizeof(uint4) * size_t(U + 1)));
+      CK(c->b_prec.ensure(sizeof(uint2) * (list[kGeneral].size() + 1)));
+      CK(c->b_disp.ensure(sizeof(uint32_t) * size_t(Tgc + 1)));
     }
   }
   CK(c->b_punt.ensure(sizeof(int32_t) * size_t(D + 1)));
@@ -1369,6 +1378,8 @@
   c->T = T; c->E = E; c->G = G; c->U = U; c->NT = NT; c->Dn = D;
   c->t_pad = (T + 3) & ~int64_t(3);
   c->Tgc = Tgc;
+  const char* units_env = getenv("EVG_GENERAL_UNITS");
+  c->gunits = units_env ? (atoi(units_env) != 0 ? 1 : 0) : -1;
   c->max_groups = 0;
   for (int32_t d = 0; d < D; d++) c->max_groups = std::max(c->max_groups, dt->group_off[d + 1] - dt->group_off[d]);
   c->any_complex = any_complex;
@@ -1476,11 +1487,17 @@
   g.pver = c->b_place.as<uint32_t>() + (c->Tgc + 1);
   g.pedge = c->b_eplace.as<uint32_t>();
   g.sedge = c->b_eplace.as<uint32_t>() + (c->E + 1);
-  g.ccount = c->b_gmisc.as<unsigned int>();
+  g.wl_off = c->b_wloff.as<uint32_t>();
+  g.dcount = c->b_dcount.as<unsigned int>();
+  g.prec = c->b_prec.as<uint2>();
+  g.disp = c->b_disp.as<uint32_t>();
+  g.dcnt = c->b_gmisc.as<unsigned int>();
   g.maxpass = c->b_gmisc.as<int32_t>() + 1;
   g.rcount = c->b_gmisc.as<unsigned int>() + 2;
   g.hcount = c->b_gmisc.as<unsigned int>() + 3;
   g.bcount = c->b_gmisc.as<unsigned int>() + 4;
+  g.punts = c->b_gmisc.as<unsigned long long>() + 4;
+  g.ustats = c->b_gmisc.as<unsigned int>() + 12;
   g.blist = c->b_blist.as<uint2>();
   g.rank = c->b_rank.as<uint32_t>();
   g.hlist = c->b_hlist.as<uint2>();
@@ -1500,6 +1517,13 @@
     }                                                                        \
   } while (0)
 #define LAUNCH(c, kernel, grid, block, ...) LAUNCH_ON(c, (c)->stream, kernel, grid, block, __VA_ARGS__)
+#define LAUNCH_DYN_ON(c, st, kernel, grid, block, smem, ...)                 \
+  do {                                                                       \
+    if ((grid) > 0) {                                                        \
+      kernel<<<(grid), (block), (smem), (st)>>>(__VA_ARGS__);                \
+      (c)->launches++;                                                       \
+    }                                                                        \
+  } while (0)
 
 int run_alloc_range(evg_ctx* c, int64_t now, int32_t d0, int32_t d1) {
   DHosts h;
@@ -1589,6 +1613,8 @@
   if (c->timed) { CK(cudaEventRecord(c->ev_gt1, st)); c->general_timed = true; }
   const unsigned wl_grid = unsigned(std::min<int64_t>(std::max<int64_t>(1, (c->Tgc + 255) / 256), int64_t(c->num_sms) * 16));
   if (gc) {
+    const int hand_back = c->gunits == 0 || (c->gunits < 0 && gcount < c->num_sms) ? 1 : 0;
+    LAUNCH_DYN_ON(c, st, k_gunits, unsigned(gcount), EVG_GUNITS_THREADS, kGUnitsBytes, dt, dd, w, g, gl, now, c->bd_valid ? 1 : 0, hand_back);
     LAUNCH_ON(c, st, k_glink, wl_grid, 256, dt, dd, w, g, now);
     LAUNCH_ON(c, st, k_galloc, wl_grid, 256, dt, dd, w, g);
     LAUNCH_ON(c, st, k_gfill, wl_grid, 256, dt, dd, w, g);
@@ -1736,6 +1762,7 @@
   CK(cudaGetDeviceProperties(&prop, device));
   if (prop.major != 9 || prop.minor != 0)
     return fail(EVG_ERR_CUDA, "device %d is sm_%d%d; this library is built for sm_90a only", device, prop.major, prop.minor);
+  CK(cudaFuncSetAttribute(k_gunits, cudaFuncAttributeMaxDynamicSharedMemorySize, int(kGUnitsBytes)));
   evg_ctx* c = new evg_ctx();
   c->device = device;
   c->num_sms = prop.multiProcessorCount;
@@ -1968,6 +1995,19 @@
   return EVG_OK;
 }
 int64_t evg_last_launch_count(evg_ctx* c) { return c ? c->launches : 0; }
+
+int evg_general_units(evg_ctx* c, int64_t* kept, int64_t* handed_back) {
+  if (!c || !kept || !handed_back) return fail(EVG_ERR_INVALID, "evg_general_units: null argument");
+  LOCK(c);
+  *kept = *handed_back = 0;
+  if (c->tick.kind == Tick::kNone || c->routes[kGeneral].h.empty()) return EVG_OK;
+  CK(cudaSetDevice(c->device));
+  uint32_t st[2] = {0u, 0u};
+  CK(cudaMemcpyAsync(st, c->b_gmisc.as<uint32_t>() + 12, sizeof(st), cudaMemcpyDeviceToHost, c->stream));
+  CK(cudaStreamSynchronize(c->stream));
+  *kept = st[0]; *handed_back = st[1];
+  return EVG_OK;
+}
 
 int evg_last_timing_ms(evg_ctx* c, float* total_ms, float* sort_ms) {
   if (!c || !c->timed) return fail(EVG_ERR_STATE, "no timed run");
diff --git a/evergreen_b200/scheduler.py b/evergreen_b200/scheduler.py
--- a/evergreen_b200/scheduler.py
+++ b/evergreen_b200/scheduler.py
@@ -180,6 +180,11 @@
 
     def last_launch_count(self) -> int:
         return int(self.lib.evg_last_launch_count(self.ctx))
+
+    def general_units(self):
+        kept, back = C.c_int64(0), C.c_int64(0)
+        L.check(self.lib.evg_general_units(self.ctx, C.byref(kept), C.byref(back)))
+        return int(kept.value), int(back.value)
 
     def last_timing_ms(self) -> Tuple[float, float]:
         a, b = C.c_float(), C.c_float()
diff --git a/include/evg_sched.h b/include/evg_sched.h
--- a/include/evg_sched.h
+++ b/include/evg_sched.h
@@ -230,6 +230,7 @@
 void* evg_device_result_ptr(evg_ctx* ctx);
 int evg_bind_result_buffer(evg_ctx* ctx, void* device_ptr, int64_t capacity);
 int64_t evg_last_launch_count(evg_ctx* ctx);
+int evg_general_units(evg_ctx* ctx, int64_t* kept, int64_t* handed_back);
 int evg_last_timing_ms(evg_ctx* ctx, float* total_ms, float* sort_ms);
 
 int evg_kernel_timing_ms(evg_ctx* ctx, float* out_ms, int32_t n);
```

Result: faster. 5.004 billion, median of 6 (+10.1%).
